# zhouxuguang/GNXRayTracer

Measured on AMD Instinct MI355X. Metric: Mrays/sec + wall-clock to 1024spp, dragon Cornell 1920×1080, higher is better.
Workload: dtype f32; 1 GPU; cfg3: Cornell + synthetic 100000-tri mesh (stand-in for absent dragon.3d), Glass+Metal, PathIntegrator maxDepth 8 rr 1 spatial, Halton(1024), 1920x1080; passes_in_flight=4, sub_passes=56, spp_rendered=1024, gather=n/a, world_size=1, backend=none, devices_visible=1

## Files before the change

### __graft_entry__.py

```python
import os
import shutil
import subprocess
import sys

ROOT = os.path.dirname(os.path.abspath(__file__))
CSRC = os.path.join(ROOT, "gnxraytracer_amd", "csrc")
LIB = os.path.join(ROOT, "gnxraytracer_amd", "libgnxr.so")
SOURCES = ["inst_whitted_tex.hip", "inst_whitted.hip", "inst_vol.hip", "inst_shade_query.hip", "inst_aov.hip", "api.hip", "scene_compile.cpp", "scene_builder.cpp"]
HIPCC_FLAGS = ["--offload-arch=gfx950", "-O3", "-std=c++17", "-fPIC", "-ffp-contract=off", "-fno-slp-vectorize", "-fno-unroll-loops", "-Wall",
               "-Wno-unused-variable", "-Wno-unused-function"]


def _newer(target, deps):
    if not os.path.exists(target):
        return False
    t = os.path.getmtime(target)
    return all(os.path.getmtime(d) <= t for d in deps)


def source_id():
    import hashlib
    h = hashlib.sha1()
    for f in sorted(os.listdir(CSRC)):
        if f.endswith((".h", ".hip", ".cpp")):
            h.update(f.encode()); h.update(open(os.path.join(CSRC, f), "rb").read())
    h.update(" ".join(HIPCC_FLAGS).encode())
    return h.hexdigest()[:12]


LIB_ID = LIB + ".source_id"


def library_source_id():
    try:
        return open(LIB_ID).read().strip()
    except OSError:
        return None


def build_lib(force=False):
    hipcc = shutil.which("hipcc") or "/opt/rocm/bin/hipcc"
    deps = [os.path.join(CSRC, f) for f in os.listdir(CSRC)] + [os.path.join(ROOT, "include", "gnxr.h")]
    if not force and _newer(LIB, deps) and library_source_id() == source_id():
        return LIB
    objdir = os.path.join(ROOT, "build")
    os.makedirs(objdir, exist_ok=True)
    objs = [os.path.join(objdir, os.path.splitext(s)[0] + ".o") for s in SOURCES]
    procs = [subprocess.Popen([hipcc] + HIPCC_FLAGS + ["-c", os.path.join(CSRC, s), "-o", o], cwd=CSRC) for s, o in zip(SOURCES, objs)]
    failed = [s for s, p in zip(SOURCES, procs) if p.wait() != 0]
    if failed:
        raise RuntimeError("hipcc failed for " + ", ".join(failed))
    sid = source_id()
    subprocess.check_call([hipcc, "--offload-arch=gfx950", "-shared", "-fPIC"] + objs + ["-o", LIB, "-lpthread"], cwd=CSRC)
    with open(LIB_ID, "w") as f:
        f.write(sid + "\n")
    return LIB


CLI = os.path.join(ROOT, "gnxraytracer_amd", "gnxr_cli")


def build_cli():
    src = os.path.join(ROOT, "tools", "gnxr_cli.c")
    if _newer(CLI, [src, LIB, os.path.join(ROOT, "include", "gnxr.h")]):
        return CLI
    subprocess.check_call(["gcc", "-std=c11", "-O2", "-Wall", src, "-o", CLI, "-L" + os.path.dirname(LIB), "-lgnxr", "-Wl,-rpath,$ORIGIN"])
    return CLI


def build_oracle():
    subprocess.check_call(["make", "-C", os.path.join(ROOT, "oracle"), "libgnx_oracle.so"])
    if os.path.isdir("/root/reference"):
        subprocess.check_call(["make", "-C", os.path.join(ROOT, "oracle"), "-j8", "ref"], stdout=subprocess.DEVNULL)


def build():
    build_lib()
    build_cli()
    build_oracle()
    sys.path.insert(0, ROOT)
    import gnxraytracer_amd as gx
    gx.lib()


def smoke():
    sys.path.insert(0, ROOT)
    sys.path.insert(0, os.path.join(ROOT, "tests"))
    import numpy as np

    import gnxraytracer_amd as gx
    import oracle_lib as ol
    import scenes

    if library_source_id() is not None and library_source_id() != source_id():
        raise RuntimeError("gnxraytracer_amd/libgnxr.so was built from other sources than gnxraytracer_amd/csrc (%s vs %s): run build()" % (library_source_id(), source_id()))
    gx.init(0)
    b = scenes.cornell()
    integ = gx.PathIntegrator(8, 1.0, "spatial")
    scene = gx.Scene(b)
    img, st = integ.Render(scene, 64, 64, 16)
    oimg, ost = ol.OracleScene(b).render(integ, 64, 64, 16)
    rmse = float(np.sqrt(np.mean((img[..., :3] - oimg[..., :3]) ** 2)))
    print(f"smoke: 64x64x16spp Cornell  rays gpu={st['rays_closest']}+{st['rays_any']} oracle={ost['rays_closest']}+{ost['rays_any']} rmse={rmse:.3e}")
    assert rmse < 1e-3, rmse
    assert abs(st["rays_closest"] - ost["rays_closest"]) <= 1e-3 * ost["rays_closest"]


if __name__ == "__main__":
    build()
    if len(sys.argv) > 1 and sys.argv[1] == "smoke":
        smoke()
```

### gnxraytracer_amd/csrc/api.hip

```cpp
#include <hip/hip_runtime.h>

#include <chrono>
#include <cstdio>
#include <cstdlib>
#include <memory>
#include <mutex>
#include <string>
#include <thread>
#include <vector>

#include "host_scene.h"
#include "kernels.hip.h"
#include "trace4_kernel.hip.h"
#include "hlbvh_build.hip.h"
#include "refit_kernel.hip.h"
#include "material_kernel.hip.h"
#include "rebuild_kernel.hip.h"
#include "li_kernel.hip.h"
#include "views_kernel.hip.h"
#include "shade_query_kernel.hip.h"
#include "aov_kernel.hip.h"
#include "kernel_instances.h"

using namespace gnxr;

#define X(M, L, S, T) extern template GX_WHITTED_SIGNATURE(M, L, S, T)
GX_WHITTED_INSTANCES(X)
#undef X
#define X(M, L, ST, T) extern template GX_VOL_SIGNATURE(M, L, ST, T)
GX_VOL_INSTANCES(X)
#undef X
extern template GX_BSDF_QUERY_SIGNATURE(LM_ALL)
extern template GX_LIGHT_SAMPLE_QUERY_SIGNATURE(LT_ALL)
extern template GX_LIGHT_LE_QUERY_SIGNATURE(LT_ALL)
extern template GX_TRACE_CLOSEST_CODE_SIGNATURE(32)
extern template GX_TRACE_CLOSEST_CODE_SIGNATURE(64)
#define X(M) extern template GX_AOV_RESOLVE_SIGNATURE(M)
GX_AOV_INSTANCES(X)
#undef X

#include "api_common.hip.h"
#include "api_scene.hip.h"
#include "api_hlbvh.hip.h"
#include "api_probes.hip.h"
#include "api_device_call.hip.h"
#include "api_render.hip.h"

extern "C" {

int gnxr_init(int device_id) {
    int n = 0;
    hipError_t e = hipGetDeviceCount(&n);
    if (e != hipSuccess || n <= 0) { set_error("no HIP device available; libgnxr has no CPU fallback"); return GNXR_ERR_NO_DEVICE; }
    if (device_id < 0 || device_id >= n) { set_error("device %d out of range (%d visible)", device_id, n); return GNXR_ERR_INVALID; }
    HIP_TRY(hipSetDevice(device_id));
    g_device = -1;
    g_devices.assign(1, device_id);
    g_peer_ok.assign(1, 1);
    return ensure_device();
}
int gnxr_init_devices(int32_t n_devices, const int32_t *device_ids) {
    if (n_devices <= 0 || n_devices > 64 || !device_ids) { set_error("bad device list"); return GNXR_ERR_INVALID; }
    int n = 0;
    hipError_t e = hipGetDeviceCount(&n);
    if (e != hipSuccess || n <= 0) { set_error("no HIP device available; libgnxr has no CPU fallback"); return GNXR_ERR_NO_DEVICE; }
    for (int i = 0; i < n_devices; ++i)
        if (device_ids[i] < 0 || device_ids[i] >= n) { set_error("device %d out of range (%d visible)", device_ids[i], n); return GNXR_ERR_INVALID; }
    int rc = gnxr_init(device_ids[0]);
    if (rc) return rc;
    g_devices.assign(device_ids, device_ids + n_devices);
    g_peer_ok.assign(n_devices, 1);
    for (int i = 1; i < n_devices; ++i) {
        if (device_ids[i] == device_ids[0]) continue;
        int can01 = 0, can10 = 0;
        bool ok = hipDeviceCanAccessPeer(&can01, device_ids[0], device_ids[i]) == hipSuccess && can01 &&
                  hipDeviceCanAccessPeer(&can10, device_ids[i], device_ids[0]) == hipSuccess && can10;
        if (ok) {
            hipError_t e0 = hipSetDevice(device_ids[0]) == hipSuccess ? hipDeviceEnablePeerAccess(device_ids[i], 0) : hipErrorInvalidDevice;
            hipError_t e1 = hipSetDevice(device_ids[i]) == hipSuccess ? hipDeviceEnablePeerAccess(device_ids[0], 0) : hipErrorInvalidDevice;
            ok = (e0 == hipSuccess || e0 == hipErrorPeerAccessAlreadyEnabled) && (e1 == hipSuccess || e1 == hipErrorPeerAccessAlreadyEnabled);
        }
        g_peer_ok[i] = ok ? 1 : 0;
        if (getenv("GNXR_VERBOSE")) fprintf(stderr, "[gnxr] device %d <-> %d: %s\n", device_ids[0], device_ids[i], ok ? "peer access" : "no peer access: rows are staged through the host");
    }
    (void)hipGetLastError();
    if (getenv("GNXR_NO_PEER")) for (int i = 1; i < n_devices; ++i) g_peer_ok[i] = 0;
    HIP_TRY(hipSetDevice(device_ids[0]));
    return GNXR_OK;
}
void gnxr_shutdown(void) { g_device = -1; g_devices.clear(); g_peer_ok.clear(); }
int gnxr_set_profiling(int flags) { g_profiling = flags; return GNXR_OK; }
#ifdef GX_SHADE_STATS
int gnxr_debug_shade_stats(unsigned long long *out16, int reset) {
    if (hipMemcpyFromSymbol(out16, HIP_SYMBOL(g_shade_stats), 16 * sizeof(unsigned long long)) != hipSuccess) return GNXR_ERR_INVALID;
    if (reset) { unsigned long long z[16] = {0}; (void)hipMemcpyToSymbol(HIP_SYMBOL(g_shade_stats), z, sizeof(z)); }
    return GNXR_OK;
}
#endif
#ifdef GX_TRACE_STATS
int gnxr_debug_trace_stats(unsigned long long *out16, int reset) {
    if (hipMemcpyFromSymbol(out16, HIP_SYMBOL(g_trace_stats), 24 * sizeof(unsigned long long)) != hipSuccess) return GNXR_ERR_INVALID;
    if (reset) { unsigned long long z[24] = {0}; (void)hipMemcpyToSymbol(HIP_SYMBOL(g_trace_stats), z, sizeof(z)); }
    return GNXR_OK;
}
#endif
#ifdef GX_TAIL_STAMP
int gnxr_debug_tail_stamp(unsigned long long *out12, int reset) {
    if (hipMemcpyFromSymbol(out12, HIP_SYMBOL(g_tail), 12 * sizeof(unsigned long long)) != hipSuccess) return GNXR_ERR_INVALID;
    if (reset) { unsigned long long z[12] = {~0ull, 0ull, ~0ull, 0ull}; (void)hipMemcpyToSymbol(HIP_SYMBOL(g_tail), z, sizeof(z)); }
    return GNXR_OK;
}
#endif

static int upload_scene(gnxr_scene *s, size_t) {
    const CompiledScene &cs = s->cs;
    int rc;
    if (cs.bvh_max_depth + 1 > 64) { set_error("BVH depth %d exceeds the 64-entry traversal stack (BVHAccel.cpp:661)", cs.bvh_max_depth); return GNXR_ERR_UNSUPPORTED; }
    s->set_traversal(std::any_of(cs.nodes.begin(), cs.nodes.end(), [](const DNode &n) { return (n.meta & 0xffffu) > 127; }));
#define UP(field) if ((rc = s->field.upload(cs.field)) != GNXR_OK) return rc;
    UP(nodes) UP(nodes4) UP(tris) UP(leaf_boxes) UP(tri_class) UP(lights) UP(perms) UP(primes) UP(prime_sums) UP(prime_magic)
    UP(dmedia) UP(grid_density) UP(tri_media) UP(spheres) UP(textures) UP(tex_texels) UP(ewa_lut) UP(tri_uv) UP(tri_n) UP(tri_s)
    UP(aov_albedo)
    UP(env_texels4) UP(env_cond_func) UP(env_cond_cdf) UP(env_cond_int) UP(env_marg_func) UP(env_marg_cdf) UP(env_marg_guide) UP(env_cond_guide)
#undef UP
    {
        const size_t worst = 2 * cs.desc_materials.size();
        if ((rc = s->material_authored.alloc(worst)) || (rc = s->materials.alloc(1 + worst)) || (rc = s->materials_single.alloc(1 + worst))) return rc;
        if ((rc = s->material_authored.upload(cs.material_authored)) != GNXR_OK) return rc;
        const DTexTables rec = s->tex_tables(s->tri_uv.p, s->tri_n.p, s->tri_s.p);
        for (int k = 0; k < 2; ++k) {
            const std::vector<DMaterial> &src = k == 0 ? cs.materials : cs.materials_single;
            std::vector<DMaterial> up(src.size() + 1);
            memset(&up[0], 0, sizeof(DMaterial));
            memcpy(&up[0], &rec, sizeof(rec));
            std::copy(src.begin(), src.end(), up.begin() + 1);
            if ((rc = (k == 0 ? s->materials : s->materials_single).upload(up)) != GNXR_OK) return rc;
        }
    }
    if ((rc = s->infinite.upload(cs.infinite_lights)) != GNXR_OK) return rc;
    if ((rc = s->counters.alloc(1)) != GNXR_OK) return rc;
    if (hipHostMalloc((void **)&s->h_counters, sizeof(Counters)) != hipSuccess) { set_error("hipHostMalloc failed"); return GNXR_ERR_OOM; }
    if (hipHostMalloc((void **)&s->h_ring, sizeof(Counters) * gnxr_scene::kRing) != hipSuccess) { set_error("hipHostMalloc failed"); return GNXR_ERR_OOM; }
    for (hipEvent_t &e : s->ring_ev) HIP_TRY(hipEventCreateWithFlags(&e, hipEventDisableTiming));
    for (hipStream_t &a : s->aux_stream) HIP_TRY(hipStreamCreateWithFlags(&a, hipStreamNonBlocking));
    HIP_TRY(hipEventCreateWithFlags(&s->ev_fork, hipEventDisableTiming));
    for (hipEvent_t &e : s->ev_join) HIP_TRY(hipEventCreateWithFlags(&e, hipEventDisableTiming));
    return GNXR_OK;
}

int gnxr_scene_create(const gnxr_scene_desc *desc, gnxr_scene **out) {
    if (!desc || !out) { set_error("null argument"); return GNXR_ERR_INVALID; }
    int rc = ensure_device();
    if (rc) return rc;
    gnxr_scene *s = new (std::nothrow) gnxr_scene(g_device);
    if (!s) return GNXR_ERR_OOM;
    if (!compile_scene(desc, &s->cs, device_hlbvh_build)) { delete s; return GNXR_ERR_INVALID; }
    for (size_t i = 1; i < g_devices.size(); ++i) s->replicas.push_back(std::make_unique<gnxr_scene>(g_devices[i], s->host));
    if ((rc = s->each_copy(upload_scene)) != GNXR_OK) { delete s; return rc; }
    const CompiledScene &cs = s->cs;
    if (getenv("GNXR_VERBOSE"))
        fprintf(stderr, "[gnxr] scene: %zu tris, %zu nodes (depth %d), %zu 4-wide nodes (stack %d), wide=%d, %zu device(s)\n", cs.tris.size(), cs.nodes.size(), cs.bvh_max_depth,
                cs.nodes4.size(), cs.stack4_need, (int)s->wide_ok, s->n_copies());
    *out = s;
    return GNXR_OK;
}
void gnxr_scene_destroy(gnxr_scene *s) { delete s; }

int gnxr_scene_info(const gnxr_scene *s, int32_t *n_nodes, int32_t *max_depth, int32_t *n_vox) {
    if (!s) return GNXR_ERR_INVALID;
    if (n_nodes) *n_nodes = (int32_t)s->cs.nodes.size();
    if (max_depth) *max_depth = s->cs.bvh_max_depth;
    if (n_vox) *n_vox = s->grid_strategy >= 0 ? s->grid.nvox[0] * s->grid.nvox[1] * s->grid.nvox[2] : 0;
    return GNXR_OK;
}

int gnxr_render_device(gnxr_scene *s, const gnxr_render_params *pin, void *d_rgba_out, void *hip_stream, gnxr_stats *stats) {
    return render_sharded(s, pin, d_rgba_out, hip_stream, stats);
}

int gnxr_render_reserve(gnxr_scene *s, const gnxr_render_params *pin) {
    if (!s || !pin) { set_error("null argument"); return GNXR_ERR_INVALID; }
    int dummy = 0;
    return render_sharded(s, pin, &dummy, nullptr, nullptr, true);
// ... 261 lines not shown
```

### gnxraytracer_amd/csrc/api_common.hip.h

```cpp
#pragma once

namespace { int hip_status(hipError_t e); }
#define HIP_TRY(expr)                                                                                   \
    do {                                                                                                \
        hipError_t e_ = (expr);                                                                         \
        if (e_ != hipSuccess) {                                                                         \
            set_error("%s failed: %s (%s:%d)", #expr, hipGetErrorString(e_), __FILE__, __LINE__);       \
            return hip_status(e_);                                                                      \
        }                                                                                               \
    } while (0)

namespace {

int hip_status(hipError_t e) {
    if (e == hipErrorOutOfMemory) return GNXR_ERR_OOM;
    if (e == hipErrorNoDevice || e == hipErrorInvalidDevice || e == hipErrorInsufficientDriver || e == hipErrorNotInitialized) return GNXR_ERR_NO_DEVICE;
    return GNXR_ERR_RUNTIME;
}

int g_device = -1;
std::vector<int> g_devices;
std::vector<char> g_peer_ok;
int g_num_cus = 256;
int g_profiling = 0;
int g_grid_bpc = 8;
int g_trace_blocks_per_cu = 5;

struct KernelTimer {
    std::vector<hipEvent_t> pool;
    struct Span { int kind; hipEvent_t a, b; };
    std::vector<Span> open;
    size_t used = 0;
    double seconds[3] = {0, 0, 0};
    unsigned launches[3] = {0, 0, 0};
    hipEvent_t get() {
        if (used == pool.size()) { hipEvent_t e; if (hipEventCreate(&e) != hipSuccess) return nullptr; pool.push_back(e); }
        return pool[used++];
    }
    void begin(int kind, hipStream_t st) { Span s{kind, get(), get()}; if (s.a && s.b) { (void)hipEventRecord(s.a, st); open.push_back(s); } }
    void end(hipStream_t st) { if (!open.empty()) (void)hipEventRecord(open.back().b, st); }
    void collect() {
        for (auto &s : open) { float ms = 0; if (hipEventElapsedTime(&ms, s.a, s.b) == hipSuccess) { seconds[s.kind] += ms * 1e-3; launches[s.kind]++; } }
        open.clear();
        used = 0;
    }
    ~KernelTimer() { for (auto e : pool) (void)hipEventDestroy(e); }
};

struct Knobs {
    static int env_int(const char *name, int unset) { const char *e = getenv(name); return e ? atoi(e) : unset; }
    static bool env_set(const char *name) { return getenv(name) != nullptr; }
#define GX_ONCE(type, expr) do { static const type v = (expr); return v; } while (0)
    static int trace_blocks_per_cu() { const int v = env_int("GNXR_TRACE_BLOCKS_PER_CU", 0); return v >= 1 && v <= 8 ? v : 0; }
    static int grid_blocks_per_cu() { const int v = env_int("GNXR_GRID_BLOCKS_PER_CU", 0); return v >= 1 && v <= 4096 ? v : 0; }
    static int trace_lds_levels() { GX_ONCE(int, env_set("GNXR_TRACE_LDS_LEVELS") ? std::max(2, env_int("GNXR_TRACE_LDS_LEVELS", 0)) : 64); }
    static int trace_chunk() { GX_ONCE(int, env_set("GNXR_TRACE_CHUNK") ? std::max(64, env_int("GNXR_TRACE_CHUNK", 0) / 64 * 64) : kTraceChunk); }
    static bool leaf_box_table() { GX_ONCE(bool, env_set("GNXR_LEAF_BOX_TABLE")); }
    static int regions() { GX_ONCE(int, env_int("GNXR_REGIONS", 0)); }
    static bool pipeline() { GX_ONCE(bool, env_int("GNXR_PIPELINE", 1) != 0); }
    static int pipe_cut() { GX_ONCE(int, env_int("GNXR_PIPE_CUT", -1)); }
    static int loop_lag() { GX_ONCE(int, env_int("GNXR_LOOP_LAG", -1)); }
    static int shade_blocks_per_cu() { GX_ONCE(int, env_set("GNXR_SHADE_BLOCKS_PER_CU") ? std::max(1, env_int("GNXR_SHADE_BLOCKS_PER_CU", 0)) : 32); }
    static int shade_lds_dims() { GX_ONCE(int, env_set("GNXR_SHADE_LDS_DIMS") ? std::max(0, std::min(128, env_int("GNXR_SHADE_LDS_DIMS", 0))) : 64); }
    static bool shade_lds_tables() { GX_ONCE(bool, env_int("GNXR_SHADE_LDS_TABLES", 1) != 0); }
    static int shade_streams() { GX_ONCE(int, env_int("GNXR_SHADE_STREAMS", -1)); }
    static bool vol_pack() { GX_ONCE(bool, env_int("GNXR_VOL_PACK", 1) != 0); }
#undef GX_ONCE
    static int volmedia_step_cap() { return env_set("GNXR_VOLMEDIA_STEP_CAP") ? std::max(0, env_int("GNXR_VOLMEDIA_STEP_CAP", 0)) : 64; }
    static bool no_escape_queue() { return env_set("GNXR_NO_ESCAPE_QUEUE"); }
    static bool host_light_grid() { return env_set("GNXR_HOST_LIGHT_GRID"); }
    static bool binary_bvh() { return env_set("GNXR_BINARY_BVH"); }
};

int ensure_device() {
    if (g_device >= 0) { HIP_TRY(hipSetDevice(g_device)); return GNXR_OK; }
    int n = 0;
    hipError_t e = hipGetDeviceCount(&n);
    if (e != hipSuccess || n <= 0) {
        set_error("no HIP device available (%s); libgnxr has no CPU fallback", e != hipSuccess ? hipGetErrorString(e) : "0 devices");
        return GNXR_ERR_NO_DEVICE;
    }
    int dev = 0;
    HIP_TRY(hipGetDevice(&dev));
    hipDeviceProp_t prop;
    HIP_TRY(hipGetDeviceProperties(&prop, dev));
    g_num_cus = prop.multiProcessorCount > 0 ? prop.multiProcessorCount : 256;
    g_device = dev;
    if (const int v = Knobs::trace_blocks_per_cu()) g_trace_blocks_per_cu = v;
    if (const int v = Knobs::grid_blocks_per_cu()) g_grid_bpc = v;
    return GNXR_OK;
}

template <typename T>
struct DevBuf {
    T *p = nullptr;
    size_t n = 0;
    ~DevBuf() { release(); }
    void release() { if (p) { (void)hipFree(p); p = nullptr; n = 0; } }
    int alloc(size_t count) {
        if (count <= n && p) return GNXR_OK;
        release();
        if (count == 0) count = 1;
        HIP_TRY(hipMalloc((void **)&p, count * sizeof(T)));
        n = count;
        return GNXR_OK;
    }
    int upload(const T *src, size_t count) {
        int rc = alloc(count);
        if (rc) return rc;
        if (count) HIP_TRY(hipMemcpy(p, src, count * sizeof(T), hipMemcpyHostToDevice));
        return GNXR_OK;
    }
    template <typename V> int upload(const V &v) { return upload(v.data(), v.size()); }
};

int grid_for(long long n, int blocks_per_cu = 0) {
    if (blocks_per_cu <= 0) blocks_per_cu = g_grid_bpc;
    long long need = (n + kBlock - 1) / kBlock;
    long long cap = (long long)g_num_cus * blocks_per_cu;
    return (int)std::max<long long>(1, std::min(need, cap));
}

}
```

### gnxraytracer_amd/csrc/api_render.hip.h

```cpp
#pragma once

struct TraceLaunch {
    int entries;
    int lds_entries;
    bool spill_needed;
    size_t lds;
    int n_top;
    int blocks;
};
static TraceLaunch trace_launch(const gnxr_scene *s, bool wide, bool spheres, long long total) {
    TraceLaunch t;
    t.entries = wide ? s->cs.stack4_need + 1 : s->cs.bvh_max_depth + 2;
    const int per_cu = g_trace_blocks_per_cu;
    const size_t fixed_b = wide ? (size_t)(kRayRecDwords + (spheres ? 1 : 0)) * kRqStride * sizeof(int) + (size_t)kTopCache * 128 + 128 : 0;
    t.lds_entries = std::min(std::min(t.entries, Knobs::trace_lds_levels()), std::max(2, (int)(((160 * 1024) / per_cu - 1024 - fixed_b) / (kBlock * sizeof(int)))));
    t.spill_needed = t.entries > t.lds_entries;
    t.lds = (size_t)t.lds_entries * kBlock * sizeof(int) + fixed_b;
    t.n_top = (int)std::min<size_t>(kTopCache, s->cs.root4 >= 0 ? s->cs.nodes4.size() : 0);
    t.blocks = (int)std::min<long long>((long long)g_num_cus * per_cu, (total + kBlock - 1) / kBlock);
    return t;
}

static int count_local_rows(const gnxr_render_params *p) {
    int rows = 0;
    for (int y = 0; y < p->height; ++y)
        if ((y / p->shard_rows) % p->shard_count == p->shard_index) ++rows;
    return rows;
}

struct RaySource {
    const gnxr_ray *rays;
    const gnxr_li_sample *samples;
    float *L;
    long long n;
};

struct ViewSource {
    const gnxr_camera *cameras;
    const int32_t *media;
    int n_views;
};

struct RenderPlan {
    gnxr_render_params p;
    bool direct, volpath, whitted;
    int wmode;
    int n_records, max_light_samples;
    bool textured_scene;
    int class_mask;
    bool area_only, area_env_only;
    bool escape_queue;
    bool caller_rays;
    int n_views;
    int local_rows, npix;
    long long unit, unit_begin, unit_end;
    int spill_entries;
    int k, in_flight;
    size_t half, cap, nrec;

    bool path_int() const { return !whitted && !volpath; }
    int nsamples() const { return p.spp_end - p.spp_begin; }
    int size_passes(size_t slots_held, bool have_mem, size_t free_b);
};

static const long long kSubPassPaths = 64ll << 20;
static const unsigned long long kSlotBytesEstimate = 238;
static const double kStateFreeFraction = 0.45;
static const unsigned long long kStateCapBytes = 150ull * 1000 * 1000 * 1000;

static int plan_render(const CompiledScene &cs, const gnxr_render_params *pin, const RaySource *src, const ViewSource *views, RenderPlan *out) {
    RenderPlan &pl = *out;
    gnxr_render_params &p = pl.p;
    p = *pin;
    if (p.shard_count <= 0) p.shard_count = 1;
    if (p.shard_rows <= 0) p.shard_rows = 1;
    if (p.spp_end <= 0) p.spp_end = p.spp;
    if (!image_and_samples_ok(p) || p.shard_index < 0 || p.shard_index >= p.shard_count || p.max_depth < 0 || p.max_depth > 250) return invalid_render_params();
    if (p.integrator != GNXR_INTEGRATOR_PATH && p.integrator != GNXR_INTEGRATOR_VOLPATH && p.integrator != GNXR_INTEGRATOR_WHITTED &&
        p.integrator != GNXR_INTEGRATOR_DIRECT) {
        set_error("unknown integrator %d", p.integrator);
        return GNXR_ERR_UNSUPPORTED;
    }
    pl.direct = p.integrator == GNXR_INTEGRATOR_DIRECT;
    if (pl.direct && p.direct_strategy != GNXR_DIRECT_SAMPLE_ALL && p.direct_strategy != GNXR_DIRECT_SAMPLE_ONE) {
        set_error("unknown direct-lighting strategy %d", p.direct_strategy);
        return GNXR_ERR_INVALID;
    }
    pl.volpath = p.integrator == GNXR_INTEGRATOR_VOLPATH;
    pl.whitted = p.integrator == GNXR_INTEGRATOR_WHITTED || pl.direct;
    pl.wmode = !pl.direct ? WM_WHITTED : (p.direct_strategy == GNXR_DIRECT_SAMPLE_ONE ? WM_DIRECT_ONE : WM_DIRECT_ALL);
    pl.n_records = (int)cs.desc_lights.size();
    pl.max_light_samples = 1;
    if (pl.wmode == WM_DIRECT_ONE) pl.n_records = 1;
    if (pl.wmode == WM_DIRECT_ALL) {
        pl.n_records = 0;
        for (const gnxr_light &l : cs.desc_lights) { pl.n_records += std::max(1, l.n_samples); pl.max_light_samples = std::max(pl.max_light_samples, l.n_samples); }
        pl.n_records = std::max(1, pl.n_records);
    }
    if (pl.whitted && (pl.n_records > 256 || p.max_depth > 32)) {
        set_error("Whitted / DirectLighting on the device: at most 256 light samples per vertex (every light is sampled at every vertex), depth 32");
        return GNXR_ERR_UNSUPPORTED;
    }
    pl.class_mask = 0;
    for (const DMaterial &m : cs.materials) pl.class_mask |= 1 << m.shade_class;
    pl.textured_scene = (pl.class_mask & 8) != 0;
    if (src && pl.textured_scene && (pl.whitted || pl.volpath)) {
        set_error("Li for caller rays: Whitted, DirectLighting and VolPath need camera ray differentials on scenes with image textures");
        return GNXR_ERR_UNSUPPORTED;
    }
    if (views && pl.textured_scene && pl.volpath) {
        set_error("views: VolPath on a scene with image textures recomputes the camera's ray differentials inside its shade kernels; render its views one by one");
        return GNXR_ERR_UNSUPPORTED;
    }
    pl.area_only = pl.area_env_only = true;
    for (const gnxr_light &l : cs.desc_lights) {
        if (l.type != GNXR_LIGHT_AREA_TRI) pl.area_only = false;
        if (l.type != GNXR_LIGHT_AREA_TRI && l.type != GNXR_LIGHT_INFINITE) pl.area_env_only = false;
    }
    pl.escape_queue = pl.path_int() && !pl.textured_scene && !cs.infinite_lights.empty() && !Knobs::no_escape_queue();
    pl.caller_rays = src != nullptr;
    pl.n_views = views ? views->n_views : 0;
    pl.local_rows = count_local_rows(&p);
    pl.npix = views ? views->n_views * p.width * p.height : pl.local_rows * p.width;
    pl.unit = src ? 1 : pl.npix;
    pl.unit_begin = src ? 0 : p.spp_begin;
    pl.unit_end = src ? src->n : p.spp_end;
    pl.spill_entries = std::max(cs.stack4_need + 1, cs.bvh_max_depth + 2);
    pl.k = pl.in_flight = 0;
    pl.half = pl.cap = pl.nrec = 0;
    return GNXR_OK;
}

int RenderPlan::size_passes(size_t slots_held, bool have_mem, size_t free_b) {
    const long long n_units = unit_end - unit_begin;
    k = p.samples_per_pass;
    if (k <= 0) {
        long long target = 32ll << 20;
        if (have_mem) target = std::max<long long>(target, std::min<long long>(256ll << 20, (long long)(free_b / 4 / 230)));
        if (volpath) target = std::min<long long>(target, 64ll << 20);
        if (whitted) target = (4ll << 20) / std::max(1, n_records / 4);
        if (path_int()) target = kSubPassPaths;
        k = (int)std::max<long long>(1, std::min<long long>(n_units, target / unit));
    }
    k = (int)std::min<long long>(k, n_units);
    half = (size_t)unit * k;
    in_flight = 1;
    if (path_int() && Knobs::pipeline()) {
        const int n_subs = (int)std::min<long long>(kMaxRegions, (n_units + k - 1) / k);
        in_flight = p.passes_in_flight > 0 ? p.passes_in_flight : (Knobs::regions() > 0 ? Knobs::regions() : 4);
        in_flight = std::max(1, std::min(std::min(in_flight, kMaxRegions), n_subs));
        for (; in_flight > 1; --in_flight) {
            const unsigned long long want = (unsigned long long)in_flight * half, held = (unsigned long long)slots_held;
            const bool idx_ok = want < (1ull << 31) && want * 3ull < (1ull << 32);
            bool mem_ok = true;
            if (want > held && have_mem) mem_ok = (want - held) * kSlotBytesEstimate < (unsigned long long)(kStateFreeFraction * (double)free_b);
            if (want * kSlotBytesEstimate > kStateCapBytes) mem_ok = false;
            if (idx_ok && mem_ok) break;
        }
    }
    cap = (size_t)in_flight * half;
    nrec = whitted ? (size_t)std::max(1, n_records) : 1;
    const unsigned long long recs = nrec;
    if (cap >= (1ull << 31) || (unsigned long long)cap * recs >= (1ull << 31) || (unsigned long long)cap * (1ull + 2ull * recs) >= (1ull << 32)) {
        set_error("pass too large: %zu paths x %llu NEE records per vertex overflow the 32-bit work indices; lower samples_per_pass", cap, recs);
        return GNXR_ERR_INVALID;
    }
    return GNXR_OK;
}

int RenderState::reserve(const RenderPlan &pl) {
    const size_t cap = pl.cap, nrec = pl.nrec;
    int rc;
#define AL(f) if ((rc = f.alloc(cap)) != GNXR_OK) return rc;
    for (int i = 0; i < kRecGroups; ++i) {
        const size_t per_slot = i < 2 ? 1 : (i < 4 ? nrec : (pl.direct ? nrec : 1));
        if ((rc = rec[i].alloc(cap * per_slot * kRS)) != GNXR_OK) return rc;
    }
    if ((rc = mis_Y.alloc(cap * (pl.direct ? nrec : 1))) != GNXR_OK) return rc;
    AL(L) AL(hit) AL(queue_a) AL(queue_b) AL(queue_nee) AL(queue_c0) AL(queue_c1) AL(queue_c2) AL(queue_c3) AL(pflags) AL(pclass) AL(nee_vis)
    if (pl.whitted) {
        const size_t nl = (size_t)std::max(1, pl.n_records), md = (size_t)std::max(1, pl.p.max_depth);
        if ((rc = wh_rec.alloc(cap * nl)) ||
            (rc = wh_o.alloc(cap * md)) || (rc = wh_d.alloc(cap * md)) || (rc = wh_L.alloc(cap * md)) || (rc = wh_w.alloc(cap * md)) ||
            (rc = wh_pdf.alloc(cap * md)) || (rc = vol_vs.alloc(cap)))
            return rc;
        if (pl.textured_scene && ((rc = wh_rxo.alloc(cap * (md + 1))) || (rc = wh_rxd.alloc(cap * (md + 1))) || (rc = wh_ryo.alloc(cap * (md + 1))) || (rc = wh_ryd.alloc(cap * (md + 1)))))
            return rc;
    }
    if (pl.volpath) {
        AL(vol_n1) AL(vol_f) AL(vol_Li) AL(vol_Tr) AL(vol_Ld) AL(vol_mres) AL(vol_vs) AL(vol_state)
        AL(vol_Lout) AL(vol_alt_state) AL(vol_orig) AL(vol_alt_orig) AL(vol_newslot)
        for (int i = 0; i < kVolPackF4; ++i) AL(vol_alt[i])
        for (int i = 0; i < kRecGroups; ++i) if ((rc = vol_alt_rec[i].alloc(cap * kRS)) != GNXR_OK) return rc;
    }
#undef AL
    if ((rc = trace_spill.alloc((size_t)g_num_cus * g_trace_blocks_per_cu * kBlock * (size_t)pl.spill_entries)) != GNXR_OK) return rc;
    if (!pl.caller_rays && (rc = accum.alloc(pl.npix)) != GNXR_OK) return rc;
    const size_t max_tiles = (cap + kCompactTile - 1) / kCompactTile;
    if (tile_desc.n < kCompactMaxOut * max_tiles || !tile_desc.p) {
        if ((rc = tile_desc.alloc(kCompactMaxOut * max_tiles)) != GNXR_OK) return rc;
        HIP_TRY(hipMemset(tile_desc.p, 0, tile_desc.n * sizeof(unsigned long long)));
        HIP_TRY(hipDeviceSynchronize());
        compact_seq = 0;
    }
    if ((rc = compact_ticket.alloc(2)) != GNXR_OK) return rc;
    if (pl.n_views > 0 && (rc = view_cams.alloc((size_t)pl.n_views)) != GNXR_OK) return rc;
    return GNXR_OK;
}

unsigned long long RenderState::state_bytes(const RenderPlan &pl) {
    const unsigned long long per_slot = (2ull * kRecGroups + 2) * sizeof(float4) + 8ull * sizeof(int) + 2 + sizeof(unsigned int);
    const unsigned long long tiles = ((unsigned long long)pl.cap + kCompactTile - 1) / kCompactTile;
    return (unsigned long long)pl.cap * per_slot + tiles * kCompactMaxOut * sizeof(unsigned long long) +
           (pl.volpath ? (unsigned long long)pl.cap * (6ull * sizeof(float4) + sizeof(int4) + 1) : 0ull);
}

PathArrays RenderState::path_arrays() {
    PathArrays pa;
    float4 *rec_primary[kRecGroups];
    record_ptrs(rec, rec_primary);
    pa.bind_records(rec_primary);
    pa.mis_Y = mis_Y.p;
    pa.L = L.p; pa.hit = hit.p; pa.pflags = pflags.p; pa.pclass = pclass.p; pa.nee_vis = nee_vis.p;
    return pa;
}
VolArrays RenderState::vol_arrays() {
    VolArrays va;
    float4 *rec_primary[kRecGroups];
    record_ptrs(rec, rec_primary);
    va.bind_records(rec_primary);
    va.mis_Y = mis_Y.p;
    va.vs = vol_vs.p; va.n1 = vol_n1.p; va.f = vol_f.p;
    va.Li = vol_Li.p; va.Tr = vol_Tr.p; va.Ld = vol_Ld.p; va.mres = vol_mres.p; va.state = vol_state.p;
    va.orig = vol_orig.p; va.Lout = vol_Lout.p;
    return va;
}
WhittedArrays RenderState::whitted_arrays(const RenderPlan &pl, int n_lights) {
    WhittedArrays wa;
    wa.ws = vol_vs.p; wa.fr_o = wh_o.p; wa.fr_d = wh_d.p; wa.fr_L = wh_L.p; wa.fr_w = wh_w.p; wa.fr_pdf = wh_pdf.p;
    wa.fr_rxo = wh_rxo.p; wa.fr_rxd = wh_rxd.p; wa.fr_ryo = wh_ryo.p; wa.fr_ryd = wh_ryd.p;
    wa.cap = (int)pl.cap; wa.n_lights = n_lights; wa.n_records = pl.n_records;
    wa.start_dim = pl.wmode == WM_DIRECT_ALL ? 5 + 2 * (pl.p.max_depth * n_lights * 2) : 5;
    return wa;
}
VolPackSet RenderState::pack_set(bool alt) {
    VolPackSet ps;
    if (!alt) {
        float4 *a[kVolPackF4] = {L.p, reinterpret_cast<float4 *>(vol_vs.p), vol_n1.p, vol_f.p, vol_Li.p, vol_Tr.p, vol_Ld.p, mis_Y.p, vol_mres.p};
        for (int i = 0; i < kVolPackF4; ++i) ps.f4[i] = a[i];
        record_ptrs(rec, ps.rec);
        ps.state = vol_state.p; ps.orig = vol_orig.p;
    } else {
        for (int i = 0; i < kVolPackF4; ++i) ps.f4[i] = vol_alt[i].p;
        record_ptrs(vol_alt_rec, ps.rec);
        ps.state = vol_alt_state.p; ps.orig = vol_alt_orig.p;
    }
    return ps;
}

struct RenderRun {
    gnxr_scene *s;
    RenderState &st;
    hipStream_t stream;
    const RenderPlan &pl;
    const RaySource *src;
    const ViewSource *views;
    DScene sc;
    DRender r;
    PathArrays pa;
    VolArrays va;
    WhittedArrays wa;
    DMediaTables mt;
    Counters *dctr;
    KernelTimer timer;
    const bool timing = (g_profiling & 1) != 0, count_wide = (g_profiling & 4) != 0, counting = (g_profiling & 2) != 0 && !count_wide;
    bool spheres;
    bool list_media = false;
    int n_lights, n_scene_media;
    unsigned long long rays_closest = 0, rays_any = 0, rays_mis = 0, media_segments = 0;
    unsigned long long new_paths = 0;
    unsigned int launches = 0, passes = 0, loop_iterations = 0;

    RenderRun(gnxr_scene *scene, hipStream_t stream_, const RenderPlan &plan, const RaySource *src_, const ViewSource *views_, const DScene &sc_, const DRender &r_)
        : s(scene), st(scene->st), stream(stream_), pl(plan), src(src_), views(views_), sc(sc_), r(r_), pa(st.path_arrays()), va(st.vol_arrays()),
          wa(st.whitted_arrays(plan, (int)scene->cs.desc_lights.size())), mt(scene->media_tables()), dctr(scene->counters.p), spheres(scene->cs.n_spheres > 0),
          n_lights((int)scene->cs.desc_lights.size()), n_scene_media((int)scene->cs.media.size()) {}

    void launch_trace(TraceWork w, int n_sh, int n_mis, bool count_rays = true);
    void compact(int mode, const int *qin, int nin, const unsigned char *keys, int nout, int nscatter, unsigned int *totals, int *o0, int *o1, int *o2, int *o3 = nullptr, int split = 0,
                 const unsigned *n_dev = nullptr);
    int shade_stage(const int *q_in, int n, int *q_out, const unsigned *n_dev);
    void raygen(const PathArrays &at, long long u0, int kk, unsigned char *medium_keys);
    void resolve(const PathArrays &at, long long u0, int kk);
    void bind_set(const VolPackSet &ps);
};

void RenderRun::launch_trace(TraceWork w, int n_sh, int n_mis, bool count_rays) {
    long long total = (long long)w.n_closest + w.n_nee;
    if (total <= 0) return;
    w.order = nullptr;
    (void)hipMemsetAsync(&dctr->cursor, 0, sizeof(unsigned int), stream);
    const bool wide = s->wide_ok && !counting;
    const TraceLaunch tl = trace_launch(s, wide, spheres, total);
    if (timing) timer.begin(0, stream);
    const int chunk = Knobs::trace_chunk();
#define GX_TRACE(C, W, S) hipLaunchKernelGGL((k_trace<C, W, S>), dim3(tl.blocks), dim3(kBlock), tl.lds, stream, sc, pa, w, &dctr->cursor, dctr, tl.lds_entries, st.trace_spill.p, chunk)
#define GX_TRACE4(C, S, P) hipLaunchKernelGGL((k_trace4<C, S, P>), dim3(tl.blocks), dim3(kBlock), tl.lds, stream, sc, pa, w, &dctr->cursor, dctr, tl.lds_entries, st.trace_spill.p, chunk, tl.n_top)
#define GX_TRACE4_CS(C, S) do { if (tl.spill_needed) GX_TRACE4(C, S, true); else GX_TRACE4(C, S, false); } while (0)
    if (wide) {
        if (spheres) { if (count_wide) GX_TRACE4_CS(true, true); else GX_TRACE4_CS(false, true); }
        else { if (count_wide) GX_TRACE4_CS(true, false); else GX_TRACE4_CS(false, false); }
    } else {
        const bool cnt = counting || count_wide;
        if (spheres) { if (cnt) GX_TRACE(true, false, true); else GX_TRACE(false, false, true); }
        else { if (cnt) GX_TRACE(true, false, false); else GX_TRACE(false, false, false); }
    }
#undef GX_TRACE4_CS
#undef GX_TRACE4
#undef GX_TRACE
    if (timing) timer.end(stream);
    if (count_rays) {
        rays_closest += (unsigned long long)w.n_closest + (unsigned long long)n_mis;
        rays_any += (unsigned long long)n_sh;
        rays_mis += (unsigned long long)n_mis;
    }
    ++launches;
}

void RenderRun::compact(int mode, const int *qin, int nin, const unsigned char *keys, int nout, int nscatter, unsigned int *totals, int *o0, int *o1, int *o2, int *o3, int split,
                        const unsigned *n_dev) {
    const int tiles = (nin + kCompactTile - 1) / kCompactTile;
    const int g = std::max(1, std::min(tiles, g_num_cus * kCompactBlocksPerCu));
    if (st.compact_seq >= (1u << 30) - 1u) {
        (void)hipMemsetAsync(st.tile_desc.p, 0, st.tile_desc.n * sizeof(unsigned long long), stream);
        st.compact_seq = 0;
    }
    const unsigned seq = ++st.compact_seq;
    const CompactScratch cs{st.tile_desc.p, tiles, st.compact_ticket.p + (seq & 1u), st.compact_ticket.p + ((seq + 1u) & 1u), seq};
    const bool hitclass = mode == COMPACT_HITCLASS;
    const int *hit = hitclass ? (const int *)st.hit.p : nullptr;
    const unsigned char *cls = hitclass ? (const unsigned char *)s->tri_class.p : nullptr;
#define GX_COMPACT(M, N, NS) hipLaunchKernelGGL((k_compact<M, N, NS>), dim3(g), dim3(kCompactBlock), 0, stream, qin, nin, keys, cs, totals, o0, o1, o2, o3, hit, cls, split, n_dev, dctr)
    if (mode == COMPACT_FLAGS) {
        if (nout == 5) { if (nscatter == 3) GX_COMPACT(COMPACT_FLAGS, 5, 3); else GX_COMPACT(COMPACT_FLAGS, 5, 2); }
        else { if (nscatter == 3) GX_COMPACT(COMPACT_FLAGS, 4, 3); else GX_COMPACT(COMPACT_FLAGS, 4, 2); }
    } else if (hitclass) { if (nout == 4) GX_COMPACT(COMPACT_HITCLASS, 4, 4); else GX_COMPACT(COMPACT_HITCLASS, 3, 3); }
    else if (nout == 4) GX_COMPACT(COMPACT_CLASS, 4, 4);
    else GX_COMPACT(COMPACT_CLASS, 3, 3);
#undef GX_COMPACT
    launches += 1;
}
static int compact_stalled(const Counters &c) {
    if (!c.compact_stall) return GNXR_OK;
    set_error("queue compaction: a tile waited for its predecessors beyond the poll limit (k_compact); the render was abandoned");
    return GNXR_ERR_RUNTIME;
}

int RenderRun::shade_stage(const int *q_in, int n, int *q_out, const unsigned *n_dev) {
    if (timing) timer.begin(2, stream);
    const int class_mask = pl.class_mask;
    const bool escape_queue = pl.escape_queue;
    const int n_classes = ((class_mask & 8) || escape_queue) ? 4 : 3;
    compact(COMPACT_HITCLASS, q_in, n, st.pclass.p, n_classes, n_classes, &dctr->q_class[0], st.queue_c0.p, st.queue_c1.p, st.queue_c2.p, st.queue_c3.p, 0, n_dev);
    int *qc[4] = {st.queue_c0.p, st.queue_c1.p, st.queue_c2.p, st.queue_c3.p};
    dim3 g(grid_for(n, Knobs::shade_blocks_per_cu())), b(kBlock);
    const int sdims = std::min<int>(Knobs::shade_lds_dims(), (int)s->cs.prime_sums.size() - 1);
    const int snperm = sdims > 0 ? s->cs.prime_sums[sdims] : 0;
    const bool shade_lds_tabs = Knobs::shade_lds_tables();
    const int lmats = (shade_lds_tabs && s->cs.materials.size() <= 12) ? (int)s->cs.materials.size() : 0;
    const int llights = (shade_lds_tabs && n_lights > 0 && n_lights <= 16) ? n_lights : 0;
    const size_t slds = (sdims > 0 ? ((((size_t)snperm * 2 + 15) & ~(size_t)15) + (size_t)sdims * 32) : 0) + (size_t)lmats * sizeof(DMaterial) + (size_t)llights * sizeof(DLight);
    const int shade_streams = Knobs::shade_streams();
    const int n_class_kernels = 1 + ((class_mask & 2) ? 1 : 0) + ((class_mask & 4) ? 1 : 0) + (((class_mask & 8) || escape_queue) ? 1 : 0);
    const bool fork = (shade_streams < 0 ? n_class_kernels >= 3 : (shade_streams != 0 && n_class_kernels >= 2)) && s->aux_stream[0] && s->aux_stream[1];
    hipStream_t cst[4] = {stream, stream, stream, stream};
    if (fork) {
        HIP_TRY(hipEventRecord(s->ev_fork, stream));
        HIP_TRY(hipStreamWaitEvent(s->aux_stream[0], s->ev_fork, 0));
        HIP_TRY(hipStreamWaitEvent(s->aux_stream[1], s->ev_fork, 0));
        cst[1] = s->aux_stream[0]; cst[2] = s->aux_stream[1]; cst[3] = s->aux_stream[1];
    }
    const bool area_only = pl.area_only, area_env_only = pl.area_env_only;
#define GX_SHADE_K(K, C) hipLaunchKernelGGL(K, g, b, slds, cst[C], sc, r, pa, (const int *)qc[C], (const unsigned int *)&dctr->q_class[C], sdims, snperm, lmats, llights)
#define GX_SHADE(LMV, LTV, C) do { if (spheres) GX_SHADE_K((k_shade<LMV, LTV, true>), C); else GX_SHADE_K((k_shade<LMV, LTV, false>), C); } while (0)
#define GX_SHADE_TEX(LTV) do { if (spheres) GX_SHADE_K((k_shade<LM_ALL, LTV, true, true>), 3); else GX_SHADE_K((k_shade<LM_ALL, LTV, false, true>), 3); } while (0)
    if (area_only) {
        GX_SHADE(LM_DIFFUSE, LT_AREA, 0);
        if (class_mask & 2) GX_SHADE(LM_GLOSSY, LT_AREA, 1);
        if (class_mask & 4) GX_SHADE(LM_ALL, LT_AREA, 2);
        if (class_mask & 8) GX_SHADE_TEX(LT_AREA);
    } else if (area_env_only && !spheres && !(class_mask & 8)) {
#define GX_SHADE_AE(LMV, C) GX_SHADE_K((k_shade<LMV, LT_AREA | LT_ENV, false>), C)
        GX_SHADE_AE(LM_DIFFUSE, 0);
        if (class_mask & 2) GX_SHADE_AE(LM_GLOSSY, 1);
        if (class_mask & 4) GX_SHADE_AE(LM_ALL, 2);
#undef GX_SHADE_AE
    } else {
        GX_SHADE(LM_DIFFUSE, LT_ALL, 0);
        if (class_mask & 2) GX_SHADE(LM_GLOSSY, LT_ALL, 1);
        if (class_mask & 4) GX_SHADE(LM_ALL, LT_ALL, 2);
        if (class_mask & 8) GX_SHADE_TEX(LT_ALL);
    }
#undef GX_SHADE_TEX
#undef GX_SHADE
#undef GX_SHADE_K
    if (escape_queue) {
        if (area_env_only) hipLaunchKernelGGL((k_shade_escape<LT_AREA | LT_ENV>), g, b, 0, cst[3], sc, pa, (const int *)qc[3], (const unsigned int *)&dctr->q_class[3]);
        else hipLaunchKernelGGL((k_shade_escape<LT_ALL>), g, b, 0, cst[3], sc, pa, (const int *)qc[3], (const unsigned int *)&dctr->q_class[3]);
        ++launches;
    }
    if (fork) {
        HIP_TRY(hipEventRecord(s->ev_join[0], s->aux_stream[0]));
        HIP_TRY(hipEventRecord(s->ev_join[1], s->aux_stream[1]));
        HIP_TRY(hipStreamWaitEvent(stream, s->ev_join[0], 0));
        HIP_TRY(hipStreamWaitEvent(stream, s->ev_join[1], 0));
    }
    launches += 1 + ((class_mask & 2) ? 1 : 0) + ((class_mask & 4) ? 1 : 0) + ((class_mask & 8) ? 1 : 0);
    compact(COMPACT_FLAGS, q_in, n, st.pflags.p, 4, 2, &dctr->q_next, q_out, st.queue_nee.p, nullptr, nullptr, 0, n_dev);
    if (timing) timer.end(stream);
    return GNXR_OK;
}

void RenderRun::raygen(const PathArrays &at, long long u0, int kk, unsigned char *medium_keys) {
    const int n_new = (int)(pl.unit * kk);
    if (views) hipLaunchKernelGGL(k_raygen_views, dim3(grid_for(n_new)), dim3(kBlock), 0, stream, sc, r, (const DCamera *)st.view_cams.p, at, n_new, (int)u0, medium_keys);
    else if (!src) hipLaunchKernelGGL(k_raygen, dim3(grid_for(n_new)), dim3(kBlock), 0, stream, sc, r, at, n_new, (int)u0);
    else hipLaunchKernelGGL(k_raygen_rays, dim3(grid_for(n_new)), dim3(kBlock), 0, stream, sc, r, at, reinterpret_cast<const float4 *>(src->rays + u0),
                            reinterpret_cast<const int4 *>(src->samples + u0), n_new, n_scene_media, medium_keys, dctr, u0);
}
void RenderRun::resolve(const PathArrays &at, long long u0, int kk) {
    if (!src) hipLaunchKernelGGL(k_resolve, dim3(grid_for(r.npix)), dim3(kBlock), 0, stream, at, st.accum.p, r.npix, kk);
    else hipLaunchKernelGGL(k_store_li, dim3(grid_for(kk)), dim3(kBlock), 0, stream, (const float4 *)at.L, reinterpret_cast<const int4 *>(src->samples + u0), r,
                            n_scene_media, kk, reinterpret_cast<float4 *>(src->L) + u0);
}
void RenderRun::bind_set(const VolPackSet &ps) {
    pa.bind_records(ps.rec); va.bind_records(ps.rec);
    pa.L = ps.f4[0]; va.vs = reinterpret_cast<int4 *>(ps.f4[1]); va.n1 = ps.f4[2]; va.f = ps.f4[3]; va.Li = ps.f4[4]; va.Tr = ps.f4[5]; va.Ld = ps.f4[6]; pa.mis_Y = va.mis_Y = ps.f4[7]; va.mres = ps.f4[8];
    va.state = ps.state; va.orig = ps.orig;
}

#define GX_CHECK_LAUNCHES(where)                                                                                    \
    do {                                                                                                            \
        const hipError_t le_ = hipGetLastError();                                                                   \
        if (le_ != hipSuccess) { set_error("HIP runtime error in " where ": %s", hipGetErrorString(le_)); return hip_status(le_); } \
    } while (0)

static int run_path_loop(RenderRun &run) {
    gnxr_scene *s = run.s;
    RenderState &st = run.st;
    const RenderPlan &pl = run.pl;
    hipStream_t stream = run.stream;
    Counters *dctr = run.dctr;
    const size_t half = pl.half;
    struct Sub { long long u0; int kk; };
    std::vector<Sub> subs;
    for (long long u0 = pl.unit_begin; u0 < pl.unit_end; u0 += pl.k) subs.push_back(Sub{u0, (int)std::min<long long>(pl.k, pl.unit_end - u0)});
    const int R = pl.in_flight;
    struct Region { int sub = -1, started = -1; long long paths = 0; } reg[kMaxRegions];
    const int lag = std::max(1, std::min(gnxr_scene::kRing - 2, Knobs::loop_lag() >= 0 ? Knobs::loop_lag() : 2));
    const int stagger = Knobs::pipe_cut() >= 0 ? Knobs::pipe_cut() : std::max(1, (pl.p.max_depth + 2 + lag + R - 1) / R);
    int *qbuf[2] = {st.queue_a.p, st.queue_b.p};
    int in_idx = 0;
    const unsigned *cnt_ptr = &dctr->n_queue;
    size_t next_sub = 0, done_subs = 0;
    int iter = 0, last_start = -(1 << 20), newest_seen = -1;
    int ring_iter[gnxr_scene::kRing];
    for (int &v : ring_iter) v = -1;
    Counters seen;
    memset(&seen, 0, sizeof(seen));
    long long guard = 0;
    while (done_subs < subs.size()) {
        {
            int oldest_needed = iter - 1 - lag;
            for (int j = newest_seen + 1; j <= oldest_needed; ++j) {
                const int slot = j % gnxr_scene::kRing;
                if (j >= 0 && ring_iter[slot] == j) HIP_TRY(hipEventSynchronize(s->ring_ev[slot]));
            }
            for (int j = iter - 1; j > newest_seen; --j) {
                const int slot = ((j % gnxr_scene::kRing) + gnxr_scene::kRing) % gnxr_scene::kRing;
                if (j < 0 || ring_iter[slot] != j) continue;
                const hipError_t q = hipEventQuery(s->ring_ev[slot]);
                if (q == hipSuccess) { seen = s->h_ring[slot]; newest_seen = j; if (int rc = compact_stalled(seen)) return rc; break; }
                if (q != hipErrorNotReady) { set_error("HIP runtime error in the path loop: hipEventQuery: %s", hipGetErrorString(q)); return hip_status(q); }
                (void)hipGetLastError();
            }
        }
        for (bool progress = true; progress;) {
            progress = false;
            for (int rg = 0; rg < R; ++rg) {
                Region &g = reg[rg];
                if (g.sub >= 0 && (run.src || g.sub == (int)done_subs) && newest_seen > g.started && seen.region_alive[rg] == 0) {
                    run.resolve(run.pa.at((size_t)rg * half), subs[g.sub].u0, subs[g.sub].kk);
                    ++run.launches; ++run.passes; ++done_subs;
                    g.sub = -1;
                    progress = true;
                }
            }
        }
        if (done_subs == subs.size()) break;
        bool any_active = false;
        long long n_upper = 0;
        for (int rg = 0; rg < R; ++rg) {
            const Region &g = reg[rg];
            if (g.sub < 0) continue;
            any_active = true;
            n_upper += newest_seen > g.started ? std::min<long long>(g.paths, seen.region_alive[rg]) : g.paths;
        }
        const int out_idx = 1 - in_idx;
        if (any_active) {
            if (int rc = run.shade_stage(qbuf[in_idx], (int)n_upper, qbuf[out_idx], cnt_ptr)) return rc;
            hipLaunchKernelGGL(k_loop_tail, dim3(1), dim3(64), 0, stream, (const int *)qbuf[out_idx], dctr, R, (int)half, (unsigned)iter);
            ++run.launches;
            const int slot = iter % gnxr_scene::kRing;
            HIP_TRY(hipMemcpyAsync(&s->h_ring[slot], dctr, sizeof(Counters), hipMemcpyDeviceToHost, stream));
            HIP_TRY(hipEventRecord(s->ring_ev[slot], stream));
            ring_iter[slot] = iter;
        }
        int trace_idx = out_idx;
        long long n_trace_upper = n_upper;
        int free_rg = -1;
        for (int rg = 0; rg < R && free_rg < 0; ++rg) if (reg[rg].sub < 0) free_rg = rg;
        const bool start = next_sub < subs.size() && free_rg >= 0 && (!any_active || iter - last_start >= stagger);
        if (start) {
            const Sub &nw = subs[next_sub];
            const int n_new = (int)(pl.unit * nw.kk);
            const size_t base = (size_t)free_rg * half;
            run.raygen(run.pa.at(base), nw.u0, nw.kk, nullptr);
            hipLaunchKernelGGL(k_queue_merge, dim3(grid_for(n_upper + n_new)), dim3(kBlock), 0, stream, (const int *)qbuf[out_idx], dctr, any_active ? 0 : 1, free_rg, (int)base, n_new, qbuf[in_idx]);
            run.launches += 2;
            trace_idx = in_idx; n_trace_upper = n_upper + n_new;
            run.new_paths += (unsigned long long)n_new;
            reg[free_rg].sub = (int)next_sub; reg[free_rg].started = iter; reg[free_rg].paths = n_new;
            last_start = iter;
            ++next_sub;
        }
        if (any_active || start) {
            TraceWork tw{qbuf[trace_idx], (int)n_trace_upper, st.queue_nee.p, any_active ? (int)n_upper : 0, nullptr, reinterpret_cast<unsigned char *>(st.nee_vis.p), cnt_ptr,
                         any_active ? (const unsigned *)&dctr->q_nee : nullptr};
            run.launch_trace(tw, 0, 0, false);
            if (any_active) {
                if (run.timing) run.timer.begin(1, stream);
                hipLaunchKernelGGL(k_nee_combine, dim3(grid_for(n_upper)), dim3(kBlock), 0, stream, run.pa, (const int *)st.queue_nee.p, (int)n_upper, reinterpret_cast<const unsigned char *>(st.nee_vis.p),
                                   (const unsigned *)&dctr->q_nee);
                if (run.timing) run.timer.end(stream);
                ++run.launches;
            }
            in_idx = trace_idx;
        }
        GX_CHECK_LAUNCHES("the path loop");
        ++iter; ++run.loop_iterations;
        if (++guard > (1ll << 24)) { set_error("path loop did not terminate"); return GNXR_ERR_INVALID; }
    }
    return GNXR_OK;
}

static int run_whitted_pass(RenderRun &run, long long u0, int kk) {
    RenderState &st = run.st;
    const RenderPlan &pl = run.pl;
    hipStream_t stream = run.stream;
    Counters *dctr = run.dctr;
    const DScene &sc = run.sc;
    const DRender &r = run.r;
    const PathArrays &pa = run.pa;
    const WhittedArrays &wa = run.wa;
    const int n_paths = (int)(pl.unit * kk), n_records = pl.n_records;
    const bool textured = pl.textured_scene;
    hipLaunchKernelGGL(k_whitted_init, dim3(grid_for(n_paths)), dim3(kBlock), 0, stream, pa, wa, n_paths);
    ++run.launches;
    if (textured) {
        if (run.views) hipLaunchKernelGGL(k_whitted_init_diff_views, dim3(grid_for(n_paths)), dim3(kBlock), 0, stream, sc, r, (const DCamera *)st.view_cams.p, pa, wa, n_paths);
// ... 338 lines not shown
```

### gnxraytracer_amd/csrc/compact_kernel.hip.h

```cpp
#pragma once
#include "device_math.h"

namespace gnxr {

constexpr int kCompactBlock = 512;
enum CompactMode { COMPACT_FLAGS = 0, COMPACT_CLASS = 1, COMPACT_HITCLASS = 2 };

template <int MODE>
GX_DEV bool compact_pred(unsigned key, int o) { return MODE == COMPACT_FLAGS ? ((key >> o) & 1u) != 0 : key == (unsigned)o; }

constexpr int kCompactChunks = 32;
constexpr int kCompactTile = kCompactBlock * kCompactChunks;
constexpr int kCompactWaves = kCompactBlock / 64;
constexpr int kCompactSpan = 64 * kCompactChunks;
constexpr int kCompactBlocksPerCu = 2;
constexpr int kCompactGather = 8;
constexpr unsigned kCompactPollCap = 1u << 21;
constexpr int kCompactMaxOut = 5;
static_assert(kCompactChunks <= 32 && kCompactChunks % kCompactGather == 0, "predicate masks are 32-bit");
static_assert(kCompactMaxOut <= kCompactWaves, "one wave per predicate looks back");

enum : unsigned { COMPACT_DESC_COUNT = 1u, COMPACT_DESC_PREFIX = 2u };
GX_DEV unsigned long long compact_desc(unsigned tag, unsigned value) { return ((unsigned long long)tag << 32) | value; }

struct CompactScratch {
    unsigned long long *desc;
    int stride;
    unsigned *ticket;
    unsigned *ticket_next;
    unsigned seq;
};

template <int MODE, int NOUT, int NSCATTER>
__global__ void __launch_bounds__(kCompactBlock) k_compact(const int *__restrict__ q_in, int n, const unsigned char *__restrict__ keys, CompactScratch cs,
                                                           unsigned int *totals, int *out0, int *out1, int *out2, int *out3, const int *__restrict__ hit,
                                                           const unsigned char *__restrict__ tri_class, int split, const unsigned *n_dev, Counters *ctr) {
    __shared__ unsigned int wtot[NOUT][kCompactWaves];
    __shared__ unsigned int s_excl[NOUT];
    __shared__ unsigned int s_ticket;
    __shared__ int s_stop;
    const int tid = threadIdx.x, lane = tid & 63, wave = tid >> 6;
    int *outs[4] = {out0, out1, out2, out3};
    if (n_dev) n = (int)min(*n_dev, (unsigned)n);
    const int tilesUsed = (n + kCompactTile - 1) / kCompactTile;
    if (blockIdx.x == 0 && tid == 0) *cs.ticket_next = 0u;
    if (tilesUsed == 0) {
        if (blockIdx.x == 0 && tid < NOUT) totals[tid] = 0u;
        return;
    }
    if (tid == 0) s_stop = 0;
    const unsigned tag_count = (cs.seq << 2) | COMPACT_DESC_COUNT, tag_prefix = (cs.seq << 2) | COMPACT_DESC_PREFIX;
    for (;;) {
        __syncthreads();
        if (tid == 0) s_ticket = atomicAdd(cs.ticket, 1u);
        __syncthreads();
        const unsigned tile = s_ticket;
        if (tile >= (unsigned)tilesUsed) break;
        const long long base = (long long)tile * kCompactTile + wave * kCompactSpan + lane;
        const int *q = q_in ? q_in + base : nullptr;
        const int left = (int)min((long long)n - base, (long long)kCompactSpan);
        int path[kCompactChunks];
#pragma unroll
        for (int c = 0; c < kCompactChunks; ++c) path[c] = c * 64 < left ? (q ? q[c * 64] : (int)base + c * 64) : -1;
        unsigned m[NSCATTER];
#pragma unroll
        for (int o = 0; o < NSCATTER; ++o) m[o] = 0u;
        unsigned acc[NOUT];
#pragma unroll
        for (int o = 0; o < NOUT; ++o) acc[o] = 0u;
#pragma unroll
        for (int c0 = 0; c0 < kCompactChunks; c0 += kCompactGather) {
            unsigned key[kCompactGather];
            if (MODE == COMPACT_HITCLASS) {
                int h[kCompactGather];
#pragma unroll
                for (int j = 0; j < kCompactGather; ++j) h[j] = path[c0 + j] >= 0 ? hit[path[c0 + j]] : -1;
#pragma unroll
                for (int j = 0; j < kCompactGather; ++j) key[j] = path[c0 + j] < 0 ? 0xffu : (h[j] >= 0 ? (unsigned)tri_class[h[j]] : (unsigned)keys[path[c0 + j]]);
            } else {
#pragma unroll
                for (int j = 0; j < kCompactGather; ++j) key[j] = path[c0 + j] >= 0 ? (unsigned)keys[path[c0 + j]] : 0xffu;
            }
#pragma unroll
            for (int j = 0; j < kCompactGather; ++j) {
                const int c = c0 + j;
                const bool valid = path[c] >= 0;
#pragma unroll
                for (int o = 0; o < NOUT; ++o) {
                    const bool pr = valid && ((MODE == COMPACT_FLAGS && o == 4) ? ((key[j] & 1u) != 0 && path[c] < split) : compact_pred<MODE>(key[j], o));
                    if (o < NSCATTER) m[o < NSCATTER ? o : 0] |= (pr ? 1u : 0u) << c;
                    acc[o] += (unsigned)__popcll(__ballot(pr));
                }
            }
        }
#pragma unroll
        for (int o = 0; o < NSCATTER; ++o) m[o] = (unsigned)__shfl((int)m[o], lane);
#pragma unroll
        for (int o = 0; o < NOUT; ++o) if (lane == 0) wtot[o][wave] = acc[o];
        __syncthreads();
        if (wave < NOUT) {
            const int o = wave;
            unsigned agg = 0;
            for (int w = 0; w < kCompactWaves; ++w) agg += wtot[o][w];
            unsigned long long *d = cs.desc + (size_t)o * cs.stride;
            if (lane == 0) __hip_atomic_store(&d[tile], compact_desc(tile == 0 ? tag_prefix : tag_count, agg), __ATOMIC_RELAXED, __HIP_MEMORY_SCOPE_AGENT);
            unsigned excl = 0, polls = 0;
            bool stalled = false;
            long long j = (long long)tile - 1;
            while (j >= 0) {
                const long long idx = j - lane;
                const unsigned long long w = idx >= 0 ? __hip_atomic_load(&d[idx], __ATOMIC_RELAXED, __HIP_MEMORY_SCOPE_AGENT) : compact_desc(tag_prefix, 0u);
                const unsigned tag = (unsigned)(w >> 32);
                const unsigned long long has_prefix = __ballot(tag == tag_prefix), not_ready = __ballot(tag != tag_prefix && tag != tag_count);
                const int first = has_prefix ? __ffsll((long long)has_prefix) - 1 : 63;
                const unsigned long long needed = first >= 63 ? ~0ull : ((2ull << first) - 1ull);
                if (not_ready & needed) {
                    if (++polls > kCompactPollCap) { stalled = true; break; }
                    __builtin_amdgcn_s_sleep(2);
                    continue;
                }
                unsigned sum = lane <= first ? (unsigned)w : 0u;
#pragma unroll
                for (int off = 32; off > 0; off >>= 1) sum += __shfl_xor(sum, off);
                excl += sum;
                if (has_prefix) break;
                j -= 64;
            }
            if (lane == 0) {
                if (stalled) {
                    s_stop = 1;
                    atomicOr(&ctr->compact_stall, 1u);
                    __hip_atomic_store(cs.ticket, 0x80000000u, __ATOMIC_RELAXED, __HIP_MEMORY_SCOPE_AGENT);
                } else {
                    s_excl[o] = excl;
                    if (tile > 0) __hip_atomic_store(&d[tile], compact_desc(tag_prefix, excl + agg), __ATOMIC_RELAXED, __HIP_MEMORY_SCOPE_AGENT);
                    if (tile == (unsigned)tilesUsed - 1u) totals[o] = excl + agg;
                }
            }
        }
        __syncthreads();
        if (s_stop) return;
        unsigned run[NSCATTER];
#pragma unroll
        for (int o = 0; o < NSCATTER; ++o) {
            run[o] = s_excl[o];
            for (int w = 0; w < wave; ++w) run[o] += wtot[o][w];
        }
#pragma unroll
        for (int c = 0; c < kCompactChunks; ++c) {
#pragma unroll
            for (int o = 0; o < NSCATTER; ++o) {
                const bool pr = ((m[o] >> c) & 1u) != 0;
                const unsigned long long b = __ballot(pr);
                const unsigned rank = __builtin_amdgcn_mbcnt_hi((unsigned)(b >> 32), __builtin_amdgcn_mbcnt_lo((unsigned)b, 0u));
                if (pr) outs[o][run[o] + rank] = path[c];
                run[o] += (unsigned)__popcll(b);
            }
        }
    }
}

}
```

### gnxraytracer_amd/csrc/device_bsdf.h

```cpp
#pragma once
#include "device_sampler.h"

namespace gnxr {

GX_DEV float cos_theta(V3 w) { return w.z; }
GX_DEV float cos2_theta(V3 w) { return w.z * w.z; }
GX_DEV float abs_cos_theta(V3 w) { return fabsf(w.z); }
GX_DEV float sin2_theta(V3 w) { return fmaxf(0.f, 1.f - cos2_theta(w)); }
GX_DEV float sin_theta(V3 w) { return gx_sqrt(sin2_theta(w)); }
GX_DEV float tan_theta(V3 w) { return sin_theta(w) / cos_theta(w); }
GX_DEV float tan2_theta(V3 w) { return sin2_theta(w) / cos2_theta(w); }
GX_DEV float cos_phi(V3 w) { float s = sin_theta(w); return (s == 0) ? 1 : clampf(w.x / s, -1, 1); }
GX_DEV float sin_phi(V3 w) { float s = sin_theta(w); return (s == 0) ? 0 : clampf(w.y / s, -1, 1); }
GX_DEV float cos2_phi(V3 w) { return cos_phi(w) * cos_phi(w); }
GX_DEV float sin2_phi(V3 w) { return sin_phi(w) * sin_phi(w); }
GX_DEV bool same_hemisphere(V3 w, V3 wp) { return w.z * wp.z > 0; }
GX_DEV V3 reflect(V3 wo, V3 n) { return -wo + 2 * dot(wo, n) * n; }
GX_DEV bool refract(V3 wi, V3 n, float eta, V3 *wt) {
    float cosThetaI = dot(n, wi);
    float sin2ThetaI = fmaxf(0.f, 1 - cosThetaI * cosThetaI);
    float sin2ThetaT = eta * eta * sin2ThetaI;
    if (sin2ThetaT >= 1) return false;
    float cosThetaT = gx_sqrt(1 - sin2ThetaT);
    *wt = eta * -wi + (eta * cosThetaI - cosThetaT) * n;
    return true;
}

GX_DEV float fr_dielectric(float cosThetaI, float etaI, float etaT) {
    cosThetaI = clampf(cosThetaI, -1, 1);
    bool entering = cosThetaI > 0.f;
    if (!entering) { float t = etaI; etaI = etaT; etaT = t; cosThetaI = fabsf(cosThetaI); }
    float sinThetaI = gx_sqrt(fmaxf(0.f, 1 - cosThetaI * cosThetaI));
    float sinThetaT = etaI / etaT * sinThetaI;
    if (sinThetaT >= 1) return 1;
    float cosThetaT = gx_sqrt(fmaxf(0.f, 1 - sinThetaT * sinThetaT));
    float Rparl = ((etaT * cosThetaI) - (etaI * cosThetaT)) / ((etaT * cosThetaI) + (etaI * cosThetaT));
    float Rperp = ((etaI * cosThetaI) - (etaT * cosThetaT)) / ((etaI * cosThetaI) + (etaT * cosThetaT));
    return (Rparl * Rparl + Rperp * Rperp) / 2;
}
GX_DEV Spec fr_conductor(float cosThetaI, Spec etat, Spec k) {
    cosThetaI = clampf(cosThetaI, -1, 1);
    Spec etai(1.f);
    Spec eta = etat / etai;
    Spec etak = k / etai;
    float cosThetaI2 = cosThetaI * cosThetaI;
    float sinThetaI2 = (float)(1. - (double)cosThetaI2);
    Spec eta2 = eta * eta;
    Spec etak2 = etak * etak;
    Spec t0 = eta2 - etak2 - Spec(sinThetaI2);
    Spec a2plusb2 = ssqrt(t0 * t0 + 4 * eta2 * etak2);
    Spec t1 = a2plusb2 + Spec(cosThetaI2);
    Spec a = ssqrt(0.5f * (a2plusb2 + t0));
    Spec t2 = 2.f * cosThetaI * a;
    Spec Rs = (t1 - t2) / (t1 + t2);
    Spec t3 = cosThetaI2 * a2plusb2 + Spec(sinThetaI2 * sinThetaI2);
    Spec t4 = t2 * sinThetaI2;
    Spec Rp = Rs * (t3 - t4) / (t3 + t4);
    return 0.5f * (Rp + Rs);
}
GX_DEV float schlick_weight(float cosTheta) { float m = clampf(1 - cosTheta, 0, 1); return (m * m) * (m * m) * m; }
GX_DEV float fr_schlick(float R0, float cosTheta) { return lerpf(schlick_weight(cosTheta), R0, 1); }
GX_DEV Spec fr_schlick_spec(Spec R0, float cosTheta) { return slerp(schlick_weight(cosTheta), R0, Spec(1.f)); }
GX_DEV float gtr1(float cosTheta, float alpha) {
    float alpha2 = alpha * alpha;
    return (alpha2 - 1) / (GX_PI * gx_log(alpha2) * (1 + (alpha2 - 1) * cosTheta * cosTheta));
}
GX_DEV float smith_g_ggx(float cosTheta, float alpha) {
    float alpha2 = alpha * alpha;
    float cosTheta2 = cosTheta * cosTheta;
    return (float)(1 / ((double)cosTheta + sqrt((double)(alpha2 + cosTheta2 - alpha2 * cosTheta2))));
}

#define GX_HAS_LOBE(K) ((LM >> (K)) & 1u)
#define GX_HAS_FRESNEL(K) ((LM >> (16 + (K))) & 1u)
constexpr uint32_t lobe_bit(int k) { return 1u << k; }
constexpr uint32_t fresnel_bit(int k) { return 1u << (16 + k); }
constexpr uint32_t LM_DIFFUSE = lobe_bit(LOBE_LAMBERT) | lobe_bit(LOBE_OREN);
constexpr uint32_t LM_GLOSSY = LM_DIFFUSE | lobe_bit(LOBE_SPEC_REFL) | lobe_bit(LOBE_SPEC_TRANS) | lobe_bit(LOBE_FRESNEL_SPEC) | lobe_bit(LOBE_MICRO_REFL) |
                               lobe_bit(LOBE_MICRO_TRANS) | fresnel_bit(FRESNEL_NOOP) | fresnel_bit(FRESNEL_DIELECTRIC) | fresnel_bit(FRESNEL_CONDUCTOR);
constexpr uint32_t LM_ALL = 0xffffffffu;

template <uint32_t LM>
GX_DEV Spec fresnel_eval(const DLobe &l, float cosI) {
    if (GX_HAS_FRESNEL(FRESNEL_DIELECTRIC) && l.fresnel == FRESNEL_DIELECTRIC) return Spec(fr_dielectric(cosI, l.f_etaI, l.f_etaT));
    if (GX_HAS_FRESNEL(FRESNEL_CONDUCTOR) && l.fresnel == FRESNEL_CONDUCTOR) return fr_conductor(fabsf(cosI), spec3(l.f_cEtaT), spec3(l.f_cK));
    if (GX_HAS_FRESNEL(FRESNEL_DISNEY) && l.fresnel == FRESNEL_DISNEY)
        return slerp(l.f_metallic, Spec(fr_dielectric(cosI, 1, l.f_eta)), fr_schlick_spec(spec3(l.f_R0), cosI));
    return Spec(1.f);
}

GX_DEV float tr_D(float ax, float ay, V3 wh) {
    float tan2Theta = tan2_theta(wh);
    if (isinf(tan2Theta)) return 0.f;
    const float cos4Theta = cos2_theta(wh) * cos2_theta(wh);
    float e = (cos2_phi(wh) / (ax * ax) + sin2_phi(wh) / (ay * ay)) * tan2Theta;
    return 1 / (GX_PI * ax * ay * cos4Theta * (1 + e) * (1 + e));
}
GX_DEV float tr_lambda(float ax, float ay, V3 w) {
    float absTanTheta = fabsf(tan_theta(w));
    if (isinf(absTanTheta)) return 0.f;
    float alpha = gx_sqrt(cos2_phi(w) * ax * ax + sin2_phi(w) * ay * ay);
    float alpha2Tan2Theta = (alpha * absTanTheta) * (alpha * absTanTheta);
    return (-1 + gx_sqrt(1.f + alpha2Tan2Theta)) / 2;
}
GX_DEV float tr_G1(float ax, float ay, V3 w) { return 1 / (1 + tr_lambda(ax, ay, w)); }
GX_DEV float tr_G(const DLobe &l, V3 wo, V3 wi) {
    if (l.disney_g) return tr_G1(l.alphax, l.alphay, wo) * tr_G1(l.alphax, l.alphay, wi);
    return 1 / (1 + tr_lambda(l.alphax, l.alphay, wo) + tr_lambda(l.alphax, l.alphay, wi));
}
GX_DEV float tr_pdf(float ax, float ay, V3 wo, V3 wh) {
    return tr_D(ax, ay, wh) * tr_G1(ax, ay, wo) * absdot(wo, wh) / abs_cos_theta(wo);
}
GX_DEV void tr_sample11(float cosTheta, float U1, float U2, float *slope_x, float *slope_y) {
    if (cosTheta > .9999) {
        float r = (float)sqrt((double)(U1 / (1 - U1)));
        float phi = (float)(6.28318530718 * (double)U2);
        const double sphi = gx_sin_d((double)phi), cphi = gx_cos_d((double)phi);
        *slope_x = (float)((double)r * cphi);
        *slope_y = (float)((double)r * sphi);
        return;
    }
    float sinTheta = gx_sqrt(fmaxf(0.f, 1.f - cosTheta * cosTheta));
    float tanTheta = sinTheta / cosTheta;
    float a = 1 / tanTheta;
    float G1 = 2 / (1 + gx_sqrt(1.f + 1.f / (a * a)));
    float A = 2 * U1 / G1 - 1;
    float tmp = 1.f / (A * A - 1.f);
    if (tmp > 1e10f) tmp = 1e10f;
    float B = tanTheta;
    float D = gx_sqrt(fmaxf(B * B * tmp * tmp - (A * A - B * B) * tmp, 0.f));
    float slope_x_1 = B * tmp - D;
    float slope_x_2 = B * tmp + D;
    *slope_x = (A < 0 || slope_x_2 > 1.f / tanTheta) ? slope_x_1 : slope_x_2;
    float S;
    if (U2 > 0.5f) { S = 1.f; U2 = 2.f * (U2 - .5f); }
    else { S = -1.f; U2 = 2.f * (.5f - U2); }
    float z = (U2 * (U2 * (U2 * 0.27385f - 0.73369f) + 0.46341f)) / (U2 * (U2 * (U2 * 0.093073f + 0.309420f) - 1.000000f) + 0.597999f);
    *slope_y = S * z * gx_sqrt(1.f + *slope_x * *slope_x);
}
GX_DEV V3 tr_sample_wh(float ax, float ay, V3 wo, float u0, float u1) {
    bool flip = wo.z < 0;
    V3 wi = flip ? -wo : wo;
    V3 wiStretched = normalize(V3(ax * wi.x, ay * wi.y, wi.z));
    float slope_x, slope_y;
    tr_sample11(cos_theta(wiStretched), u0, u1, &slope_x, &slope_y);
    float tmp = cos_phi(wiStretched) * slope_x - sin_phi(wiStretched) * slope_y;
    slope_y = sin_phi(wiStretched) * slope_x + cos_phi(wiStretched) * slope_y;
    slope_x = tmp;
    slope_x = ax * slope_x;
    slope_y = ay * slope_y;
    V3 wh = normalize(V3(-slope_x, -slope_y, 1.f));
    if (flip) wh = -wh;
    return wh;
}

template <uint32_t LM>
GX_DEV Spec lobe_f(const DLobe &l, V3 wo, V3 wi) {
    switch (l.kind) {
    case LOBE_LAMBERT: if (GX_HAS_LOBE(LOBE_LAMBERT)) return spec3(l.R) * GX_INV_PI; break;
    case LOBE_LAMBERT_TRANS: if (GX_HAS_LOBE(LOBE_LAMBERT_TRANS)) return spec3(l.T) * GX_INV_PI; break;
    case LOBE_OREN: if (GX_HAS_LOBE(LOBE_OREN)) {
        float sinThetaI = sin_theta(wi), sinThetaO = sin_theta(wo);
        float maxCos = 0;
        if (sinThetaI > 1e-4 && sinThetaO > 1e-4) {
            float sinPhiI = sin_phi(wi), cosPhiI = cos_phi(wi);
            float sinPhiO = sin_phi(wo), cosPhiO = cos_phi(wo);
            float dCos = cosPhiI * cosPhiO + sinPhiI * sinPhiO;
            maxCos = fmaxf(0.f, dCos);
        }
        const bool iBig = abs_cos_theta(wi) > abs_cos_theta(wo);
        const float sinAlpha = iBig ? sinThetaO : sinThetaI;
        const float tanBeta = (iBig ? sinThetaI : sinThetaO) / (iBig ? abs_cos_theta(wi) : abs_cos_theta(wo));
        return spec3(l.R) * GX_INV_PI * (l.A + l.B * maxCos * sinAlpha * tanBeta);
    }
    break;
    case LOBE_MICRO_REFL: case LOBE_MICRO_TRANS: if (GX_HAS_LOBE(LOBE_MICRO_REFL) || GX_HAS_LOBE(LOBE_MICRO_TRANS)) {
        const bool refl = l.kind == LOBE_MICRO_REFL;
        float cosThetaO, cosThetaI, eta = 1, cosArg;
        V3 wh;
        if (refl) {
            cosThetaO = abs_cos_theta(wo); cosThetaI = abs_cos_theta(wi);
            wh = wi + wo;
            if (cosThetaI == 0 || cosThetaO == 0) return Spec(0.f);
            if (wh.x == 0 && wh.y == 0 && wh.z == 0) return Spec(0.f);
            wh = normalize(wh);
            cosArg = dot(wi, faceforward(wh, V3(0, 0, 1)));
        } else {
            if (same_hemisphere(wo, wi)) return Spec(0.f);
            cosThetaO = cos_theta(wo); cosThetaI = cos_theta(wi);
            if (cosThetaI == 0 || cosThetaO == 0) return Spec(0.f);
            { const bool up = cos_theta(wo) > 0; eta = (up ? l.etaB : l.etaA) / (up ? l.etaA : l.etaB); }
            wh = normalize(wo + wi * eta);
            if (wh.z < 0) wh = -wh;
            if (dot(wo, wh) * dot(wi, wh) > 0) return Spec(0.f);
            cosArg = dot(wo, wh);
        }
        const Spec F = fresnel_eval<LM>(l, cosArg);
        const float D = tr_D(l.alphax, l.alphay, wh), G = tr_G(l, wo, wi);
        if (refl) return spec3(l.R) * D * G * F / (4 * cosThetaI * cosThetaO);
        float sqrtDenom = dot(wo, wh) + eta * dot(wi, wh);
        float factor = (1 / eta);
        return (Spec(1.f) - F) * spec3(l.T) *
               fabsf(D * G * eta * eta * absdot(wi, wh) * absdot(wo, wh) * factor * factor / (cosThetaI * cosThetaO * sqrtDenom * sqrtDenom));
    }
    break;
    case LOBE_DISNEY_DIFFUSE: if (GX_HAS_LOBE(LOBE_DISNEY_DIFFUSE)) {
        float Fo = schlick_weight(abs_cos_theta(wo)), Fi = schlick_weight(abs_cos_theta(wi));
        return spec3(l.R) * GX_INV_PI * (1 - Fo / 2) * (1 - Fi / 2);
    }
    break;
    case LOBE_DISNEY_FAKESS: if (GX_HAS_LOBE(LOBE_DISNEY_FAKESS)) {
        V3 wh = wi + wo;
        if (wh.x == 0 && wh.y == 0 && wh.z == 0) return Spec(0.f);
        wh = normalize(wh);
        float cosThetaD = dot(wi, wh);
        float Fss90 = cosThetaD * cosThetaD * l.roughness;
        float Fo = schlick_weight(abs_cos_theta(wo)), Fi = schlick_weight(abs_cos_theta(wi));
        float Fss = lerpf(Fo, 1.0f, Fss90) * lerpf(Fi, 1.0f, Fss90);
        float ss = 1.25f * (Fss * (1 / (abs_cos_theta(wo) + abs_cos_theta(wi)) - .5f) + .5f);
        return spec3(l.R) * GX_INV_PI * ss;
    }
    break;
    case LOBE_DISNEY_RETRO: if (GX_HAS_LOBE(LOBE_DISNEY_RETRO)) {
        V3 wh = wi + wo;
        if (wh.x == 0 && wh.y == 0 && wh.z == 0) return Spec(0.f);
        wh = normalize(wh);
        float cosThetaD = dot(wi, wh);
        float Fo = schlick_weight(abs_cos_theta(wo)), Fi = schlick_weight(abs_cos_theta(wi));
        float Rr = 2 * l.roughness * cosThetaD * cosThetaD;
        return spec3(l.R) * GX_INV_PI * Rr * (Fo + Fi + Fo * Fi * (Rr - 1));
    }
    break;
    case LOBE_DISNEY_SHEEN: if (GX_HAS_LOBE(LOBE_DISNEY_SHEEN)) {
        V3 wh = wi + wo;
        if (wh.x == 0 && wh.y == 0 && wh.z == 0) return Spec(0.f);
        wh = normalize(wh);
        return spec3(l.R) * schlick_weight(dot(wi, wh));
    }
    break;
    case LOBE_DISNEY_CLEARCOAT: if (GX_HAS_LOBE(LOBE_DISNEY_CLEARCOAT)) {
        V3 wh = wi + wo;
        if (wh.x == 0 && wh.y == 0 && wh.z == 0) return Spec(0.f);
        wh = normalize(wh);
        float Dr = gtr1(abs_cos_theta(wh), l.gloss);
        float Fr = fr_schlick(.04f, dot(wo, wh));
        float Gr = smith_g_ggx(abs_cos_theta(wo), .25f) * smith_g_ggx(abs_cos_theta(wi), .25f);
        return Spec(l.weight * Gr * Fr * Dr / 4);
    }
    break;
    default: break;
    }
    return Spec(0.f);
}

template <uint32_t LM>
GX_DEV float lobe_pdf(const DLobe &l, V3 wo, V3 wi) {
    switch (l.kind) {
    case LOBE_SPEC_REFL: case LOBE_SPEC_TRANS: case LOBE_FRESNEL_SPEC: return 0.f;
    case LOBE_LAMBERT_TRANS: if (GX_HAS_LOBE(LOBE_LAMBERT_TRANS)) return !same_hemisphere(wo, wi) ? abs_cos_theta(wi) * GX_INV_PI : 0.f; break;
    case LOBE_MICRO_REFL: case LOBE_MICRO_TRANS: if (GX_HAS_LOBE(LOBE_MICRO_REFL) || GX_HAS_LOBE(LOBE_MICRO_TRANS)) {
        const bool refl = l.kind == LOBE_MICRO_REFL;
        V3 wh;
        float scale;
        if (refl) {
            if (!same_hemisphere(wo, wi)) return 0.f;
            wh = normalize(wo + wi);
            scale = 4 * dot(wo, wh);
        } else {
            if (same_hemisphere(wo, wi)) return 0.f;
            const bool up = cos_theta(wo) > 0;
            float eta = (up ? l.etaB : l.etaA) / (up ? l.etaA : l.etaB);
            wh = normalize(wo + wi * eta);
            if (dot(wo, wh) * dot(wi, wh) > 0) return 0.f;
            float sqrtDenom = dot(wo, wh) + eta * dot(wi, wh);
            scale = fabsf((eta * eta * dot(wi, wh)) / (sqrtDenom * sqrtDenom));
        }
        const float p = tr_pdf(l.alphax, l.alphay, wo, wh);
        return refl ? p / scale : p * scale;
    }
    break;
    case LOBE_DISNEY_CLEARCOAT: if (GX_HAS_LOBE(LOBE_DISNEY_CLEARCOAT)) {
        if (!same_hemisphere(wo, wi)) return 0.f;
        V3 wh = wi + wo;
        if (wh.x == 0 && wh.y == 0 && wh.z == 0) return 0.f;
        wh = normalize(wh);
        float Dr = gtr1(abs_cos_theta(wh), l.gloss);
        return Dr * abs_cos_theta(wh) / (4 * dot(wo, wh));
    }
    break;
    default: break;
    }
    return same_hemisphere(wo, wi) ? abs_cos_theta(wi) * GX_INV_PI : 0.f;
}

template <uint32_t LM>
GX_DEV Spec lobe_sample(const DLobe &l, V3 wo, V3 *wi, float u0, float u1, float *pdf, int *sampledType, bool need_f = true) {
    switch (l.kind) {
    case LOBE_SPEC_REFL: if (GX_HAS_LOBE(LOBE_SPEC_REFL)) {
        *wi = V3(-wo.x, -wo.y, wo.z);
        *pdf = 1;
        return fresnel_eval<LM>(l, cos_theta(*wi)) * spec3(l.R) / abs_cos_theta(*wi);
    }
    break;
    case LOBE_SPEC_TRANS: if (GX_HAS_LOBE(LOBE_SPEC_TRANS)) {
        bool entering = cos_theta(wo) > 0;
        float etaI = entering ? l.etaA : l.etaB, etaT = entering ? l.etaB : l.etaA;
        if (!refract(wo, faceforward(V3(0, 0, 1), wo), etaI / etaT, wi)) return Spec(0.f);
        *pdf = 1;
        Spec ft = spec3(l.T) * (Spec(1.f) - fresnel_eval<LM>(l, cos_theta(*wi)));
        ft = ft * ((etaI * etaI) / (etaT * etaT));
        return ft / abs_cos_theta(*wi);
    }
    break;
    case LOBE_FRESNEL_SPEC: if (GX_HAS_LOBE(LOBE_FRESNEL_SPEC)) {
        float F = fr_dielectric(cos_theta(wo), l.etaA, l.etaB);
        if (u0 < F) {
            *wi = V3(-wo.x, -wo.y, wo.z);
            *sampledType = BSDF_SPECULAR | BSDF_REFLECTION;
            *pdf = F;
            return F * spec3(l.R) / abs_cos_theta(*wi);
        } else {
            bool entering = cos_theta(wo) > 0;
            float etaI = entering ? l.etaA : l.etaB, etaT = entering ? l.etaB : l.etaA;
            if (!refract(wo, faceforward(V3(0, 0, 1), wo), etaI / etaT, wi)) return Spec(0.f);
            Spec ft = spec3(l.T) * (1 - F);
            ft = ft * ((etaI * etaI) / (etaT * etaT));
            *sampledType = BSDF_SPECULAR | BSDF_TRANSMISSION;
            *pdf = 1 - F;
            return ft / abs_cos_theta(*wi);
        }
    }
    break;
    case LOBE_MICRO_REFL: case LOBE_MICRO_TRANS: if (GX_HAS_LOBE(LOBE_MICRO_REFL) || GX_HAS_LOBE(LOBE_MICRO_TRANS)) {
        if (wo.z == 0) return Spec(0.f);
        V3 wh = tr_sample_wh(l.alphax, l.alphay, wo, u0, u1);
        if (dot(wo, wh) < 0) return Spec(0.f);
        if (l.kind == LOBE_MICRO_REFL) {
            *wi = reflect(wo, wh);
            if (!same_hemisphere(wo, *wi)) return Spec(0.f);
            *pdf = tr_pdf(l.alphax, l.alphay, wo, wh) / (4 * dot(wo, wh));
        } else {
            const bool up = cos_theta(wo) > 0;
            float eta = (up ? l.etaA : l.etaB) / (up ? l.etaB : l.etaA);
            if (!refract(wo, wh, eta, wi)) return Spec(0.f);
            *pdf = lobe_pdf<LM>(l, wo, *wi);
        }
        return need_f ? lobe_f<LM>(l, wo, *wi) : Spec(0.f);
    }
    break;
    case LOBE_LAMBERT_TRANS: if (GX_HAS_LOBE(LOBE_LAMBERT_TRANS)) {
        *wi = cosine_sample_hemisphere(u0, u1);
        if (wo.z > 0) wi->z *= -1;
        *pdf = lobe_pdf<LM>(l, wo, *wi);
        return need_f ? lobe_f<LM>(l, wo, *wi) : Spec(0.f);
    }
    break;
    case LOBE_DISNEY_CLEARCOAT: if (GX_HAS_LOBE(LOBE_DISNEY_CLEARCOAT)) {
        if (wo.z == 0) return Spec(0.f);
        float alpha2 = l.gloss * l.gloss;
        float cosTheta = gx_sqrt(fmaxf(0.f, (1 - gx_pow(alpha2, 1 - u0)) / (1 - alpha2)));
        float sinTheta = gx_sqrt(fmaxf(0.f, 1 - cosTheta * cosTheta));
        float phi = 2 * GX_PI * u1;
        float sinPhi, cosPhi;
        gx_sincos(phi, &sinPhi, &cosPhi);
        V3 wh(sinTheta * cosPhi, sinTheta * sinPhi, cosTheta);
        if (!same_hemisphere(wo, wh)) wh = -wh;
        *wi = reflect(wo, wh);
        if (!same_hemisphere(wo, *wi)) return Spec(0.f);
        *pdf = lobe_pdf<LM>(l, wo, *wi);
        return need_f ? lobe_f<LM>(l, wo, *wi) : Spec(0.f);
    }
    break;
    default: break;
    }
    *wi = cosine_sample_hemisphere(u0, u1);
    if (wo.z < 0) wi->z *= -1;
    *pdf = lobe_pdf<LM>(l, wo, *wi);
    return need_f ? lobe_f<LM>(l, wo, *wi) : Spec(0.f);
}

template <uint32_t LM>
struct Bsdf {
    const DMaterial *mat;
    V3 ns, ng, ss, ts;
    GX_DEV V3 to_local(V3 v) const { return V3(dot(v, ss), dot(v, ts), dot(v, ns)); }
    GX_DEV V3 to_world(V3 v) const {
        return V3(ss.x * v.x + ts.x * v.y + ns.x * v.z, ss.y * v.x + ts.y * v.y + ns.y * v.z, ss.z * v.x + ts.z * v.y + ns.z * v.z);
    }
    GX_DEV static bool matches(int type, int flags) { return (type & flags) == type; }
    GX_DEV int num_components(int flags) const {
        int n = 0;
        for (int i = 0; i < mat->n_lobes; ++i) if (matches(mat->lobes[i].type, flags)) ++n;
        return n;
    }
    static constexpr bool kSingle = (LM == LM_DIFFUSE);
    static constexpr int kSingleType = BSDF_REFLECTION | BSDF_DIFFUSE;
    GX_DEV Spec f(V3 woW, V3 wiW, int flags) const {
        V3 wi = to_local(wiW), wo = to_local(woW);
        if (wo.z == 0) return Spec(0.f);
        bool refl = dot(wiW, ng) * dot(woW, ng) > 0;
        if (kSingle) return (mat->n_lobes > 0 && refl && matches(kSingleType, flags)) ? lobe_f<LM>(mat->lobes[0], wo, wi) : Spec(0.f);
        return sum_f(wo, wi, flags, refl);
    }
    GX_DEV Spec sum_f(V3 wo, V3 wi, int flags, bool refl) const {
        Spec f(0.f);
        const int n = mat->n_lobes;
        int i = 0;
        while (true) {
            while (i < n) {
                const int t = mat->lobes[i].type;
                if (matches(t, flags) && ((refl && (t & BSDF_REFLECTION)) || (!refl && (t & BSDF_TRANSMISSION)))) break;
                ++i;
            }
            if (i >= n) break;
            f = f + lobe_f<LM>(mat->lobes[i], wo, wi);
            ++i;
        }
        return f;
    }
    GX_DEV float pdf(V3 woW, V3 wiW, int flags) const {
        if (mat->n_lobes == 0) return 0.f;
        V3 wo = to_local(woW), wi = to_local(wiW);
        if (wo.z == 0) return 0.f;
        if (kSingle) return matches(kSingleType, flags) ? 0.f + lobe_pdf<LM>(mat->lobes[0], wo, wi) : 0.f;
        float p = 0.f;
        int matching = 0;
        for (int i = 0; i < mat->n_lobes; ++i) {
            const DLobe &l = mat->lobes[i];
            if (matches(l.type, flags)) { ++matching; p += lobe_pdf<LM>(l, wo, wi); }
        }
        return matching > 0 ? p / matching : 0.f;
    }
    GX_DEV Spec sample_f(V3 woW, V3 *wiW, float u0, float u1, float *pdf, int flags, int *sampledType) const {
        if (kSingle) {
            *sampledType = 0;
            if (mat->n_lobes == 0 || !matches(kSingleType, flags)) { *pdf = 0; return Spec(0.f); }
            const DLobe &bx = mat->lobes[0];
            const float ur0 = fminf(u0 * 1 - 0, GX_ONE_MINUS_EPS);
            V3 wi, wo = to_local(woW);
            *pdf = 0;
            if (wo.z == 0) return Spec(0.f);
            *sampledType = kSingleType;
            (void)lobe_sample<LM>(bx, wo, &wi, ur0, u1, pdf, sampledType, false);
            if (*pdf == 0) { *sampledType = 0; return Spec(0.f); }
            *wiW = to_world(wi);
            const bool refl = dot(*wiW, ng) * dot(woW, ng) > 0;
            return refl ? lobe_f<LM>(bx, wo, wi) : Spec(0.f);
        }
        int matching = num_components(flags);
        *sampledType = 0;
        if (matching == 0) { *pdf = 0; return Spec(0.f); }
        int comp = min((int)floorf(u0 * matching), matching - 1);
        int which = -1, count = comp;
        for (int i = 0; i < mat->n_lobes; ++i)
            if (matches(mat->lobes[i].type, flags) && count-- == 0) { which = i; break; }
        const DLobe &bx = mat->lobes[which];
        float ur0 = fminf(u0 * matching - comp, GX_ONE_MINUS_EPS);
        V3 wi, wo = to_local(woW);
        *pdf = 0;
        if (wo.z == 0) return Spec(0.f);
        *sampledType = bx.type;
        Spec f = lobe_sample<LM>(bx, wo, &wi, ur0, u1, pdf, sampledType, (bx.type & BSDF_SPECULAR) != 0);
        if (*pdf == 0) { *sampledType = 0; return Spec(0.f); }
        *wiW = to_world(wi);
        if (!(bx.type & BSDF_SPECULAR) && matching > 1) {
            const int n = mat->n_lobes;
            int i = 0;
            while (true) {
                while (i < n && !(i != which && matches(mat->lobes[i].type, flags))) ++i;
                if (i >= n) break;
                *pdf += lobe_pdf<LM>(mat->lobes[i], wo, wi);
                ++i;
            }
        }
        if (matching > 1) *pdf /= matching;
        if (!(bx.type & BSDF_SPECULAR)) {
            bool refl = dot(*wiW, ng) * dot(woW, ng) > 0;
            f = sum_f(wo, wi, flags, refl);
        }
        return f;
    }
};

}
```

### gnxraytracer_amd/csrc/gnxr_device_types.h

```cpp
#pragma once
#include <stdint.h>

namespace gnxr {

struct DNode {
    float lo[3];
    float hi0;
    float hi1, hi2;
    int32_t offset;
    uint32_t meta;
};
static_assert(sizeof(DNode) == 32, "DNode must be 32 bytes");

struct DNode4 {
    float lox[4], loy[4], loz[4], hix[4], hiy[4], hiz[4];
    int32_t child[4];
    uint32_t order_lo, order_hi;
    int32_t axes;
    int32_t _pad;
};
static_assert(sizeof(DNode4) == 128, "DNode4 must be 128 bytes");
constexpr int32_t kNode4Empty = 0x7ffffffe;
constexpr int kTopNodesMax = 1024;
constexpr int32_t kRefDone = 0x7fffffff;

struct DTri {
    float p0[3]; int32_t prim;
    float p1[3]; int32_t material;
    float p2[3]; int32_t light;
};
static_assert(sizeof(DTri) == 48, "DTri must be 48 bytes");

struct DSphere {
    float c[3]; float r;
    int32_t material, med_in, med_out, prim;
};
static_assert(sizeof(DSphere) == 32, "DSphere must be 32 bytes");

enum LobeKind : int32_t {
    LOBE_LAMBERT = 0, LOBE_OREN, LOBE_SPEC_REFL, LOBE_SPEC_TRANS, LOBE_FRESNEL_SPEC, LOBE_MICRO_REFL, LOBE_MICRO_TRANS,
    LOBE_LAMBERT_TRANS, LOBE_DISNEY_DIFFUSE, LOBE_DISNEY_FAKESS, LOBE_DISNEY_RETRO, LOBE_DISNEY_SHEEN, LOBE_DISNEY_CLEARCOAT
};
enum FresnelKind : int32_t { FRESNEL_NOOP = 0, FRESNEL_DIELECTRIC, FRESNEL_CONDUCTOR, FRESNEL_DISNEY };
enum : int32_t {
    BSDF_REFLECTION = 1, BSDF_TRANSMISSION = 2, BSDF_DIFFUSE = 4, BSDF_GLOSSY = 8, BSDF_SPECULAR = 16, BSDF_ALL = 31
};

struct DLobe {
    int32_t kind, type, fresnel, disney_g;
    float R[3]; float A;
    float T[3]; float B;
    float etaA, etaB, alphax, alphay;
    float f_etaI, f_etaT, f_metallic, f_eta;
    float f_cEtaT[3]; float roughness;
    float f_cK[3]; float weight;
    float f_R0[3]; float gloss;
};
static_assert(sizeof(DLobe) == 128, "DLobe must be 128 bytes");

struct DMaterial {
    int32_t n_lobes;
    int32_t has_bump;
    int32_t n_nonspecular;
    float eta;
    int32_t shade_class;
    int32_t kd_tex, ks_tex;
    int32_t has_attr;
    DLobe lobes[8];
};

struct DTexture {
    int32_t n_levels, w0, h0, wrap;
    int32_t trilinear; float max_aniso;
    float su, sv, du, dv;
    int32_t level_offset[16];
    int32_t _pad[2];
};
struct DLight {
    int32_t type;
    int32_t tri_leaf;
    int32_t two_sided;
    int32_t env;
    float le[3]; float area;
    float p0[3]; float inv_area;
    float p1[3]; float radius;
    float p2[3]; int32_t n_samples;
    float n[3]; float _pad2;
    float center[3]; float _pad3;
};

struct DHalton {
    int32_t base_scale[2], base_exp[2];
    int32_t stride, mult_inv[2];
    int32_t base32_max;
};

struct DCamera {
    float r2c[16];
    float c2w[16];
    float lens_radius, focal_distance;
    int32_t medium;
    int32_t ortho;
};

constexpr int kEnvGuideMarg = 1024, kEnvGuideCond = 512;
struct DEnv {
    int32_t w, h;
    int32_t dw, dh;
    float l2w[16], w2l[16];
    float world_center[3]; float world_radius;
    float marg_func_int;
};

struct DMedium {
    int32_t type;
    int32_t nx, ny, nz;
    float sigma_a[3]; float g;
    float sigma_s[3]; float sigma_t;
    float w2m[16];
    float inv_max_density;
    int32_t density_offset;
    int32_t _pad[2];
};

struct DLightGrid {
    int32_t nvox[3];
    int32_t n_lights;
    int32_t stride;
    int32_t spatial;
    float lo[3], hi[3];
};

}
```

### gnxraytracer_amd/csrc/host_scene.h

```cpp
#pragma once
#include <string>
#include <vector>

#include "../../include/gnxr.h"
#include "gnxr_device_types.h"
#include "host_math.h"

namespace gnxr {

void set_error(const char *fmt, ...);
const char *get_error();

struct Builder {
    std::vector<float> vertices;
    std::vector<int32_t> indices, tri_material, tri_light, tri_med_in, tri_med_out;
    std::vector<gnxr_material> materials;
    std::vector<gnxr_light> lights;
    std::vector<gnxr_medium> media;
    std::vector<gnxr_sphere> spheres;
    std::vector<float> grid_density;
    std::vector<gnxr_texture> textures;
    std::vector<float> texels;
    std::vector<float> tri_uv;
    std::vector<float> tri_n;
    std::vector<float> tri_s;
    std::vector<float> env_rgb;
    int env_w = 0, env_h = 0;
    gnxr_camera camera;
    int camera_medium = -1;
    int bvh_split_method = 0;
    Builder();
    int add_mesh(const float *verts, int nv, const int32_t *idx, int nt, const Xf &o2w, int material, int med_in, int med_out);
    void fill_desc(gnxr_scene_desc *d) const;
};

bool read_model_3d(const char *path, std::vector<float> *verts, std::vector<int32_t> *idx);
bool write_synthetic_3d(const char *path, int target_tris, uint32_t seed);
bool read_rgbe(const char *path, std::vector<float> *rgb, int *w, int *h);

struct CompiledScene {
    std::vector<DNode> nodes;
    std::vector<DNode4> nodes4;
    int32_t root4 = 0;
    int stack4_need = 1;
    std::vector<DTri> tris;
    std::vector<float> leaf_boxes;
    int leaf1_from_verts = 0;
    std::vector<uint8_t> tri_class;
    std::vector<int32_t> leaf_of_prim;
    int bvh_max_depth = 0;
    Box3 world_bound;
    int n_vertices = 0;
    std::vector<int32_t> corner_vertex;
    std::vector<int32_t> node_parent;
    std::vector<int32_t> node4_src;
    std::vector<DMaterial> materials;
    std::vector<DMaterial> materials_single;
    std::vector<DTexture> textures;
    std::vector<float> tex_texels;
    std::vector<float> ewa_lut;
    std::vector<float> tri_uv;
    std::vector<float> tri_n;
    std::vector<float> tri_s;
    std::vector<float> aov_albedo;
    std::vector<int32_t> material_authored;
    std::vector<gnxr_material> desc_materials;
    std::vector<int32_t> tri_material;
    std::vector<uint8_t> tri_own_attr;
    std::vector<int32_t> sphere_material;
    std::vector<int32_t> mat_map;
    std::vector<DLight> lights;
    std::vector<int32_t> infinite_lights;
    std::vector<uint16_t> perms;
    std::vector<int32_t> primes, prime_sums;
    std::vector<uint32_t> prime_magic;
    bool has_env = false;
    DEnv env;
    std::vector<float> env_texels;
    std::vector<float> env_texels4;
    float env_power_lookup[3] = {0, 0, 0};
    std::vector<float> env_cond_func, env_cond_cdf, env_cond_int;
    std::vector<float> env_marg_func, env_marg_cdf;
    std::vector<uint16_t> env_marg_guide, env_cond_guide;
    std::vector<gnxr_medium> media;
    std::vector<DMedium> dmedia;
    std::vector<float> grid_density;
    std::vector<DSphere> spheres;
    int n_spheres = 0;
    std::vector<int32_t> tri_media;
    gnxr_camera camera;
    int camera_medium = -1;
    std::vector<gnxr_light> desc_lights;
};

struct HlbvhNode { float b[6]; int32_t child[2]; int32_t axis, first, n; };
typedef bool (*HlbvhBuildFn)(const float *prim_bounds6, const float *centroids3, int n, const float lo[3], const float hi[3],
                             std::vector<HlbvhNode> *nodes, int *root, uint32_t *prims_sorted);
bool compile_scene(const gnxr_scene_desc *d, CompiledScene *out, HlbvhBuildFn hlbvh_build = nullptr);
struct MaterialTables {
    std::vector<DMaterial> materials, materials_single;
    std::vector<float> aov_albedo;
    std::vector<int32_t> material_authored, mat_map;
    void move_to(CompiledScene *cs);
};
bool compile_materials(const gnxr_material *mats, int n_materials, int n_textures, const std::vector<int32_t> &sphere_material, const int32_t *tri_material,
                       const uint8_t *tri_own_attr, int n_triangles, const int32_t *visit, MaterialTables *mt);
void triangle_material(const int32_t *mat_map, int32_t authored, uint8_t own_attr, int32_t *material, uint8_t *shade_class);
void refit_world_bound(CompiledScene *cs, const float root6[6]);
bool compile_light(const gnxr_light &l, int index, const Vec3 corners[3], int tri_leaf, const Box3 &world_bound, DLight *out);
DCamera make_camera(const gnxr_camera &c, int W, int H, int medium);
DHalton make_halton(int W, int H);
void build_light_grid(const CompiledScene &cs, int strategy, DLightGrid *grid, std::vector<float> *table, bool layout_only = false);
void light_grid_probes(const CompiledScene &cs, float *ri );

float host_radical_inverse(const CompiledScene &cs, int baseIndex, uint64_t a);

}
```

### gnxraytracer_amd/csrc/kernel_instances.h

```cpp
#pragma once
#include <hip/hip_runtime.h>

#include "host_scene.h"
#include "kernels.hip.h"
#include "vol_kernel.hip.h"
#include "whitted_kernel.hip.h"

#define GX_WH_SPH(X, M, L, T) X(M, L, false, T) X(M, L, true, T)
#define GX_WH_LT(X, M, T) GX_WH_SPH(X, M, LT_AREA, T) GX_WH_SPH(X, M, LT_ALL, T)
#define GX_WHITTED_INSTANCES_TEX(X, T) GX_WH_LT(X, WM_WHITTED, T) GX_WH_LT(X, WM_DIRECT_ONE, T) GX_WH_LT(X, WM_DIRECT_ALL, T)
#define GX_WHITTED_INSTANCES(X) GX_WHITTED_INSTANCES_TEX(X, false) GX_WHITTED_INSTANCES_TEX(X, true)

#define GX_VS_ST(X, M, L, T) X(M, L, VS_MAIN, T) X(M, L, VS_SHADOW, T) X(M, L, VS_MIS, T)
#define GX_VS_LT(X, M, T) GX_VS_ST(X, M, LT_AREA, T) GX_VS_ST(X, M, LT_ALL, T)
#define GX_VOL_INSTANCES(X) GX_VS_LT(X, LM_DIFFUSE, false) GX_VS_LT(X, LM_GLOSSY, false) GX_VS_LT(X, LM_ALL, false) GX_VS_LT(X, LM_ALL, true)

#define GX_WHITTED_SIGNATURE(M, L, S, T) \
    __global__ void gnxr::k_whitted_step<M, L, S, T>(gnxr::DScene, gnxr::DRender, gnxr::PathArrays, gnxr::WhittedArrays, const int *, int, unsigned long long *);
#define GX_VOL_SIGNATURE(M, L, ST, T) \
    __global__ void gnxr::k_vol_step<M, L, ST, T>(gnxr::DScene, gnxr::DMediaTables, gnxr::DRender, gnxr::PathArrays, gnxr::VolArrays, const int *, const unsigned int *, int, int);
```

### gnxraytracer_amd/csrc/kernels.hip.h

```cpp
#pragma once
#include "device_bsdf.h"
#include "device_lights.h"
#include "device_texture.h"

namespace gnxr {

constexpr int kBlock = 256;

constexpr int kRS = 2;
constexpr int kRSm = 2 * kRS;
constexpr int kRecGroups = 5;
struct PathArrays {
    float4 *ray_o;
    float4 *ray_d;
    float4 *beta;
    uint2 *meta;
    float4 *L;
    int *hit;
    unsigned char *pflags;
    unsigned char *pclass;
    float4 *sh_o;
    float4 *sh_d;
    float4 *sh_X;
    float4 *nbeta;
// ... 194 lines not shown
        V3 o, d;
        float tMax;
        int dim;
        camera_ray(r.cam, sc.st, px, py, index, &o, &d, &tMax, &dim);
        pa.ray_o[(size_t)slot * kRS] = make_float4(o.x, o.y, o.z, tMax);
        pa.ray_d[(size_t)slot * kRS] = make_float4(d.x, d.y, d.z, __int_as_float(r.cam.medium));
        pa.beta[(size_t)slot * kRS] = make_float4(1.f, 1.f, 1.f, 1.f);
        pa.L[slot] = make_float4(0.f, 0.f, 0.f, 0.f);
        pa.store_meta(slot, index, (uint32_t)dim);
    }
}

template <uint32_t LM, int LT>
GX_DEV int estimate_direct_record(const DScene &sc, const Bsdf<LM> &bsdf, const SurfacePoint &sp, V3 woN, int lightNum, float ul0, float ul1, float us0,
                                  float us1, const PathArrays &pa, size_t rec, float xw) {
    const int bsdfFlags = BSDF_ALL & ~BSDF_SPECULAR;
    int nflags = 0;
    V3 so, sd, mo, wi2;
    Spec X(0.f), Y(0.f);
    int expect = -1;
    LightSample ls = light_sample<LT>(sc.lt, lightNum, sp.p, ul0, ul1);
    float scatteringPdf = 0;
    if (ls.pdf > 0 && !ls.Li.is_black()) {
        Spec f = bsdf.f(woN, ls.wi, bsdfFlags) * absdot(ls.wi, sp.ns);
        scatteringPdf = bsdf.pdf(woN, ls.wi, bsdfFlags);
        if (!f.is_black()) {
            spawn_ray_to(sp.p, sp.pError, sp.n, ls.p1, ls.p1Error, ls.n1, &so, &sd);
            float weight = light_is_delta<LT>(sc.lt.lights[lightNum]) ? 1.f : power_heuristic(ls.pdf, scatteringPdf);
            X = f * ls.Li * weight / ls.pdf;
            nflags |= 1;
        }
    }
    if (!light_is_delta<LT>(sc.lt.lights[lightNum])) {
        int sampledType;
        Spec f = bsdf.sample_f(woN, &wi2, us0, us1, &scatteringPdf, bsdfFlags, &sampledType);
        f = f * absdot(wi2, sp.ns);
        bool sampledSpecular = (sampledType & BSDF_SPECULAR) != 0;
        if (!f.is_black() && scatteringPdf > 0) {
            float weight = 1;
            bool skip = false;
            if (!sampledSpecular) {
                float lightPdf = light_pdf<LT>(sc.lt, lightNum, sp.p, sp.pError, sp.n, wi2);
                if (lightPdf == 0) skip = true;
                else weight = power_heuristic(scatteringPdf, lightPdf);
            }
            if (!skip) {
                const DLight &lt = sc.lt.lights[lightNum];
                mo = offset_ray_origin(sp.p, sp.pError, sp.n, wi2);
                Spec Li2;
                if (LT == LT_AREA || lt.type == GNXR_LIGHT_AREA_TRI) {
                    V3 lp0(lt.p0[0], lt.p0[1], lt.p0[2]), lp1(lt.p1[0], lt.p1[1], lt.p1[2]), lp2(lt.p2[0], lt.p2[1], lt.p2[2]);
                    V3 ln = normalize(cross(lp0 - lp2, lp1 - lp2));
                    Li2 = area_L(lt, ln, -wi2);
                    expect = lt.tri_leaf;
                } else {
                    Li2 = light_Le<LT>(sc.lt, lightNum, mo, wi2);
                    expect = -1;
                }
                if (!Li2.is_black()) Y = f * Li2 * Spec(1.f) * weight / scatteringPdf;
                nflags |= 2;
            }
        }
    }
    if (nflags) {
        pa.sh_o[(size_t)rec * kRS] = make_float4(so.x, so.y, so.z, 1 - GX_SHADOW_EPS);
        pa.sh_d[(size_t)rec * kRS] = make_float4(sd.x, sd.y, sd.z, __int_as_float(nflags));
        pa.sh_X[(size_t)rec * kRS] = make_float4(X.r, X.g, X.b, xw);
        if (nflags & 2) {
            pa.mis_o[(size_t)rec * kRS] = make_float4(mo.x, mo.y, mo.z, __int_as_float(expect));
            pa.mis_d[(size_t)rec * kRS] = make_float4(wi2.x, wi2.y, wi2.z, 0.f);
            pa.mis_Y[rec] = make_float4(Y.r, Y.g, Y.b, 0.f);
        }
    }
    return nflags;
}
GX_DEV Spec nee_record_Ld(const PathArrays &pa, size_t rec, float *xw) {
    float4 sd4 = pa.sh_d[(size_t)rec * kRS], X4 = pa.sh_X[(size_t)rec * kRS];
    int flags = __float_as_int(sd4.w);
    Spec Ld(0.f);
    if ((flags & 1) && pa.sh_o[(size_t)rec * kRS].w == 1.f) Ld = Ld + Spec(X4.x, X4.y, X4.z);
    if (flags & 2) {
        float4 Y4 = pa.mis_Y[rec];
        Spec Y(Y4.x, Y4.y, Y4.z);
        if (pa.mis_o[(size_t)rec * kRS].w == 1.f && !Y.is_black()) Ld = Ld + Y;
    }
    *xw = X4.w;
    return Ld;
}

template <bool SPH, bool TEX, bool UV = false>
GX_DEV bool shade_hit_rebuild(const DScene &sc, const DMaterial *mats, int leaf, V3 ro, V3 rd, float tMax, V3 *p0, V3 *p1, V3 *p2, TriHit *h, int *triMat, int *triLight,
                              SurfacePoint *sp, V3 *sdpdu, V3 *sdpdv) {
    bool found = leaf != -1;
    if (SPH && leaf < -1) {
        const DSphere &sph = sc.spheres[-2 - leaf];
        *triMat = sph.material;
        float tH;
        found = sphere_test(sph, ro, rd, tMax, &tH);
        if (found) *sp = sphere_surface_point_uv<UV>(sph, ro, rd, tH, *triMat >= 0 ? mats[*triMat].has_bump != 0 : false, sdpdu, sdpdv);
    } else if (found) {
        const float4 *q = reinterpret_cast<const float4 *>(sc.tris + leaf);
        float4 a = q[0], b = q[1], c = q[2];
        *p0 = V3(a.x, a.y, a.z); *p1 = V3(b.x, b.y, b.z); *p2 = V3(c.x, c.y, c.z);
        *triMat = __float_as_int(b.w); *triLight = __float_as_int(c.w);
        tri_hit_recompute(*p0, *p1, *p2, ro, rd, h);
        *sp = surface_point(*p0, *p1, *p2, *h, *triMat >= 0 ? mats[*triMat].has_bump != 0 : false);
        if (TEX) {
            V3 dndu, dndv;
            *sp = surface_point_tables(tex_tables(sc.materials), leaf, *p0, *p1, *p2, *h, *triMat >= 0 ? mats[*triMat].has_bump != 0 : false, &dndu, &dndv);
        }
        found = sp->valid;
    }
    return found;
}
template <bool TEX>
GX_DEV const DMaterial *shade_material(const DScene &sc, const DMaterial *mat, int leaf, V3 p0, V3 p1, V3 p2, const TriHit &h, const SurfacePoint &sp, const RayDiff &rdf,
                                       DMaterial *tm) {
    if (TEX && leaf >= 0 && (mat->kd_tex | mat->ks_tex)) {
        float tu, tv;
        V3 dpdu, dpdv;
        tri_uv_frame(p0, p1, p2, h, tri_uvs(tex_tables(sc.materials), leaf), &tu, &tv, &dpdu, &dpdv);
        textured_material(tex_tables(sc.materials), *mat, tu, tv, compute_differentials(rdf, sp.p, sp.n, dpdu, dpdv), tm);
        mat = tm;
    }
    return mat;
}

#ifndef GX_SHADE_MINWAVES
#define GX_SHADE_MINWAVES 2
#endif
#ifdef GX_SHADE_WAVES
#define GX_SHADE_ATTR __attribute__((amdgpu_waves_per_eu(GX_SHADE_WAVES, GX_SHADE_WAVES)))
#else
#define GX_SHADE_ATTR __attribute__((amdgpu_waves_per_eu(GX_SHADE_MINWAVES)))
#endif
#ifdef GX_SHADE_STATS
static __device__ unsigned long long g_shade_stats[16];
#define GX_STICK(i) do { const unsigned long long t_ = __builtin_amdgcn_s_memtime(); if ((threadIdx.x & 63) == 0) sst_[i] += t_ - stick_; stick_ = t_; } while (0)
#else
#define GX_STICK(i) do {} while (0)
#endif
#ifndef GX_SHADE_W_DIFFUSE
#define GX_SHADE_W_DIFFUSE 3
#endif
#ifndef GX_SHADE_W_GLOSSY
#define GX_SHADE_W_GLOSSY 3
#endif
#ifndef GX_SHADE_W_ALL
#define GX_SHADE_W_ALL GX_SHADE_MINWAVES
#endif
#ifndef GX_SHADE_W_TEX
#define GX_SHADE_W_TEX 3
#endif
template <uint32_t LM> constexpr int shade_min_waves() { return LM == LM_DIFFUSE ? GX_SHADE_W_DIFFUSE : (LM == LM_GLOSSY ? GX_SHADE_W_GLOSSY : GX_SHADE_W_ALL); }
template <uint32_t LM, int LT, bool SPH, bool TEX = false>
__global__ void __launch_bounds__(kBlock, (TEX ? GX_SHADE_W_TEX : shade_min_waves<LM>())) k_shade(DScene sc, DRender r, PathArrays pa, const int *__restrict__ queue, const unsigned int *n_dev, int lds_dims, int lds_nperm, int lds_mats, int lds_lights) {
    extern __shared__ int shade_smem[];
    const int n = (int)*n_dev;
    if (blockIdx.x * blockDim.x >= (unsigned)n) return;
    const LdsSampler lsam = lds_sampler_fill(sc.st, lds_dims, lds_nperm, shade_smem, threadIdx.x, kBlock);
    const DMaterial *mats = sc.materials;
    DLightTables ltab = sc.lt;
    {
        int *dst = shade_smem + (lds_sampler_bytes(lds_nperm, lds_dims) >> 2);
        if (!TEX && lds_mats > 0) {
            const int *src = reinterpret_cast<const int *>(sc.materials);
            const int nd = lds_mats * (int)(sizeof(DMaterial) / 4);
            for (int k = threadIdx.x; k < nd; k += kBlock) dst[k] = src[k];
            mats = reinterpret_cast<const DMaterial *>(dst);
            dst += nd;
        }
        if (lds_lights > 0) {
            const int *src = reinterpret_cast<const int *>(sc.lt.lights);
            const int nd = lds_lights * (int)(sizeof(DLight) / 4);
            for (int k = threadIdx.x; k < nd; k += kBlock) dst[k] = src[k];
            ltab.lights = reinterpret_cast<const DLight *>(dst);
        }
    }
    __syncthreads();
#ifdef GX_SHADE_STATS
    unsigned long long sst_[16] = {0};
    unsigned long long stick_ = __builtin_amdgcn_s_memtime();
#endif
    const int stride_ = (int)(gridDim.x * blockDim.x);
    int i = (int)(blockIdx.x * blockDim.x + threadIdx.x);
    int pathCur_ = i < n ? queue[i] : -1;
    int leafCur_ = pathCur_ >= 0 ? pa.hit[pathCur_] : -1;
    int pathNext_ = (long long)i + stride_ < n ? queue[i + stride_] : -1;
    for (; i < n; i += stride_) {
        bool survive = false, wantNee = false, wantShadow = false, wantMis = false;
        int path = -1;
        GX_STICK(9);
        const int leafNext_ = pathNext_ >= 0 ? pa.hit[pathNext_] : -1;
        const int pathNext2_ = (long long)i + 2ll * stride_ < n ? queue[i + 2 * stride_] : -1;
        {
            path = pathCur_;
            uint2 m = pa.meta[(size_t)path * kRSm];
            uint32_t index = m.x;
            int dim = (int)(m.y & 0xffffu), bounces = (int)((m.y >> 16) & 0xffu);
            bool specularBounce = (m.y >> 31) != 0;
            float4 o4 = pa.ray_o[(size_t)path * kRS], d4 = pa.ray_d[(size_t)path * kRS], b4 = pa.beta[(size_t)path * kRS];
            V3 ro(o4.x, o4.y, o4.z), rd(d4.x, d4.y, d4.z);
            Spec beta(b4.x, b4.y, b4.z);
            float etaScale = b4.w;
            int leaf = leafCur_;
            bool found = leaf != -1;
            V3 p0, p1, p2;
            int triMat = -1, triLight = -1;
            TriHit h;
            SurfacePoint sp;
            sp.valid = false;
            found = shade_hit_rebuild<SPH, TEX>(sc, mats, leaf, ro, rd, o4.w, &p0, &p1, &p2, &h, &triMat, &triLight, &sp, nullptr, nullptr);
            GX_STICK(0);
            if ((bounces == 0 || specularBounce) && (found ? triLight >= 0 : ltab.n_infinite > 0)) {
                const float4 L4 = pa.L[path];
                Spec L(L4.x, L4.y, L4.z);
                if (found) L = L + beta * area_L(ltab.lights[triLight], sp.n, -rd);
                else for (int k = 0; k < ltab.n_infinite; ++k) L = L + beta * light_Le<LT>(ltab, ltab.infinite[k], ro, rd);
                pa.L[path] = make_float4(L.r, L.g, L.b, 0.f);
            }
            GX_STICK(1);
            if (found && bounces < r.max_depth) {
                if (triMat < 0) {
                    V3 o2 = offset_ray_origin(sp.p, sp.pError, sp.n, rd);
                    pa.ray_o[(size_t)path * kRS] = make_float4(o2.x, o2.y, o2.z, GX_INF);
                    survive = true;
                } else {
                    DMaterial tm;
                    RayDiff none;
                    none.has = false;
                    const DMaterial *mat = shade_material<TEX>(sc, mats + triMat, leaf, p0, p1, p2, h, sp, none, &tm);
                    Bsdf<LM> bsdf;
                    bsdf.mat = mat; bsdf.ns = sp.ns; bsdf.ng = sp.n; bsdf.ss = sp.ss; bsdf.ts = sp.ts;
                    SampleStream ss(sc.st, index, dim, lsam);
                    V3 woN = normalize(-rd);
                    if (mat->n_nonspecular > 0 && ltab.n_lights > 0) {
                        float lightPdfSel;
                        int lightNum = light_select(ltab, sp.p, ss.get1d(), &lightPdfSel);
                        GX_STICK(2);
                        if (lightPdfSel != 0) {
                            float ul0, ul1, us0, us1;
                            ss.get2d(&ul0, &ul1);
                            ss.get2d(&us0, &us1);
                            GX_STICK(3);
                            const int bsdfFlags = BSDF_ALL & ~BSDF_SPECULAR;
                            int nflags = 0;
                            V3 so, sd, mo, wi2;
                            Spec X(0.f), Y(0.f);
                            int expect = -1;
                            LightSample ls = light_sample<LT>(ltab, lightNum, sp.p, ul0, ul1);
                            GX_STICK(4);
                            float scatteringPdf = 0;
                            if (ls.pdf > 0 && !ls.Li.is_black()) {
                                Spec f = bsdf.f(woN, ls.wi, bsdfFlags) * absdot(ls.wi, sp.ns);
                                scatteringPdf = bsdf.pdf(woN, ls.wi, bsdfFlags);
                                if (!f.is_black()) {
                                    spawn_ray_to(sp.p, sp.pError, sp.n, ls.p1, ls.p1Error, ls.n1, &so, &sd);
                                    float weight = light_is_delta<LT>(ltab.lights[lightNum]) ? 1.f : power_heuristic(ls.pdf, scatteringPdf);
                                    X = f * ls.Li * weight / ls.pdf;
                                    nflags |= 1;
                                }
                            }
                            GX_STICK(5);
                            if (!light_is_delta<LT>(ltab.lights[lightNum])) {
                                int sampledType;
                                Spec f = bsdf.sample_f(woN, &wi2, us0, us1, &scatteringPdf, bsdfFlags, &sampledType);
                                f = f * absdot(wi2, sp.ns);
                                bool sampledSpecular = (sampledType & BSDF_SPECULAR) != 0;
                                GX_STICK(6);
                                if (!f.is_black() && scatteringPdf > 0) {
                                    float weight = 1;
                                    bool skip = false;
                                    if (!sampledSpecular) {
                                        float lightPdf = light_pdf<LT>(ltab, lightNum, sp.p, sp.pError, sp.n, wi2);
                                        if (lightPdf == 0) skip = true;
                                        else weight = power_heuristic(scatteringPdf, lightPdf);
                                    }
                                    if (!skip) {
                                        const DLight &lt = ltab.lights[lightNum];
                                        mo = offset_ray_origin(sp.p, sp.pError, sp.n, wi2);
                                        Spec Li2;
                                        if (LT == LT_AREA || lt.type == GNXR_LIGHT_AREA_TRI) {
                                            V3 lp0(lt.p0[0], lt.p0[1], lt.p0[2]), lp1(lt.p1[0], lt.p1[1], lt.p1[2]), lp2(lt.p2[0], lt.p2[1], lt.p2[2]);
                                            V3 ln = normalize(cross(lp0 - lp2, lp1 - lp2));
                                            Li2 = area_L(lt, ln, -wi2);
                                            expect = lt.tri_leaf;
                                        } else {
                                            Li2 = light_Le<LT>(ltab, lightNum, mo, wi2);
                                            expect = -1;
                                        }
                                        if (!Li2.is_black()) Y = f * Li2 * Spec(1.f) * weight / scatteringPdf;
                                        nflags |= 2;
                                    }
                                }
                            }
                            GX_STICK(7);
                            if (nflags) {
                                pa.sh_o[(size_t)path * kRS] = make_float4(so.x, so.y, so.z, 1 - GX_SHADOW_EPS);
                                pa.sh_d[(size_t)path * kRS] = make_float4(sd.x, sd.y, sd.z, __int_as_float(nflags));
                                pa.sh_X[(size_t)path * kRS] = make_float4(X.r, X.g, X.b, lightPdfSel);
                                if (nflags & 2) {
                                    pa.mis_o[(size_t)path * kRS] = make_float4(mo.x, mo.y, mo.z, __int_as_float(expect));
                                    pa.mis_d[(size_t)path * kRS] = make_float4(wi2.x, wi2.y, wi2.z, 0.f);
                                    pa.mis_Y[path] = make_float4(Y.r, Y.g, Y.b, 0.f);
                                }
                                pa.nbeta[(size_t)path * kRS] = make_float4(beta.r, beta.g, beta.b, 0.f);
                                const bool betaFinite = __builtin_isfinite(beta.r) && __builtin_isfinite(beta.g) && __builtin_isfinite(beta.b);
// ... 320 lines not shown
```

### gnxraytracer_amd/csrc/material_kernel.hip.h

```cpp
#pragma once
#include <hip/hip_runtime.h>

#include "gnxr_device_types.h"
#include "refit_kernel.hip.h"

namespace gnxr {
namespace matedit {

static __global__ void __launch_bounds__(refit::kB) k_material_tris(DTri *__restrict__ tris, unsigned char *__restrict__ tri_class, int n_tris,
                                                                    const int *__restrict__ tri_material, const unsigned char *__restrict__ own_attr,
                                                                    const int4 *__restrict__ mat_map) {
    for (int li = blockIdx.x * blockDim.x + threadIdx.x; li < n_tris; li += gridDim.x * blockDim.x) {
        const int prim = tris[li].prim;
        if ((unsigned)prim >= (unsigned)n_tris) continue;
        const int authored = tri_material[prim];
        int material = authored, cls = 0;
        if (authored >= 0) {
            const int4 e = mat_map[authored];
            const bool own = own_attr[prim] != 0;
            material = e.x < 0 ? -1 : (own ? e.y : e.x);
            cls = e.x < 0 ? 0 : (own ? 3 : e.z);
        }
        tris[li].material = material;
        tri_class[li] = (unsigned char)cls;
    }
}

static __global__ void __launch_bounds__(refit::kB) k_material_gather(const DTri *__restrict__ tris, const unsigned char *__restrict__ tri_class, int n_tris,
                                                                      const int *__restrict__ authored, int *__restrict__ material_out,
                                                                      unsigned char *__restrict__ class_out) {
    for (int li = blockIdx.x * blockDim.x + threadIdx.x; li < n_tris; li += gridDim.x * blockDim.x) {
        const int prim = tris[li].prim;
        if ((unsigned)prim >= (unsigned)n_tris) continue;
        const int m = tris[li].material;
        material_out[prim] = m >= 0 ? authored[m] : -1;
        class_out[prim] = tri_class[li];
    }
}

}
}
```

### gnxraytracer_amd/csrc/scene_compile.cpp

```cpp
#include <cstdio>
#include <thread>

#include "host_scene.h"

namespace gnxr {

namespace {
struct PrimInfo { int prim; Box3 b; Vec3 c; };
struct BuildNode { Box3 b; int child[2]; int axis, first, n; };

struct BvhBuilder {
    std::vector<PrimInfo> info;
    std::vector<BuildNode> nodes;
    std::vector<int> ordered;
    int method = GNXR_BVH_SAH;

    int build(int start, int end) {
        int me = (int)nodes.size();
        nodes.push_back(BuildNode());
        Box3 bounds;
        for (int i = start; i < end; ++i) bounds.grow(info[i].b);
        int n = end - start;
        auto leaf = [&]() {
            nodes[me].b = bounds; nodes[me].first = (int)ordered.size(); nodes[me].n = n;
// ... 231 lines not shown
            }
        }
        break;
    }
    case GNXR_MAT_MIRROR: {
        RGB R = clamp0(m.kr);
        if (!black(R)) { DLobe l = blank_lobe(LOBE_SPEC_REFL, BSDF_REFLECTION | BSDF_SPECULAR); set_R(l, R); l.fresnel = FRESNEL_NOOP; add(l); }
        break;
    }
    case GNXR_MAT_GLASS: {
        float eta = m.eta[0], urough = m.urough, vrough = m.vrough;
        RGB R = clamp0(m.kr), T = clamp0(m.kt);
        out->eta = eta;
        if (black(R) && black(T)) break;
        bool isSpecular = urough == 0 && vrough == 0;
        if (isSpecular && allowMultipleLobes) {
            DLobe l = blank_lobe(LOBE_FRESNEL_SPEC, BSDF_REFLECTION | BSDF_TRANSMISSION | BSDF_SPECULAR);
            set_R(l, R); set_T(l, T); l.etaA = 1.f; l.etaB = eta;
            add(l);
        } else if (isSpecular) {
            if (!black(R)) {
                DLobe l = blank_lobe(LOBE_SPEC_REFL, BSDF_REFLECTION | BSDF_SPECULAR);
                set_R(l, R); l.fresnel = FRESNEL_DIELECTRIC; l.f_etaI = 1.f; l.f_etaT = eta;
                add(l);
            }
            if (!black(T)) {
                DLobe l = blank_lobe(LOBE_SPEC_TRANS, BSDF_TRANSMISSION | BSDF_SPECULAR);
                set_T(l, T); l.etaA = 1.f; l.etaB = eta; l.fresnel = FRESNEL_DIELECTRIC; l.f_etaI = 1.f; l.f_etaT = eta;
                add(l);
            }
        } else {
            if (m.remap_roughness) { urough = roughness_to_alpha(urough); vrough = roughness_to_alpha(vrough); }
            if (!black(R)) {
                DLobe l = blank_lobe(LOBE_MICRO_REFL, BSDF_REFLECTION | BSDF_GLOSSY);
                set_R(l, R); l.fresnel = FRESNEL_DIELECTRIC; l.f_etaI = 1.f; l.f_etaT = eta; set_alpha(l, urough, vrough);
                add(l);
            }
            if (!black(T)) {
                DLobe l = blank_lobe(LOBE_MICRO_TRANS, BSDF_TRANSMISSION | BSDF_GLOSSY);
                set_T(l, T); l.etaA = 1.f; l.etaB = eta; l.fresnel = FRESNEL_DIELECTRIC; l.f_etaI = 1.f; l.f_etaT = eta;
                set_alpha(l, urough, vrough);
                add(l);
            }
        }
        break;
    }
    case GNXR_MAT_METAL: {
        float ur = m.urough, vr = m.vrough;
        if (m.remap_roughness) { ur = roughness_to_alpha(ur); vr = roughness_to_alpha(vr); }
        DLobe l = blank_lobe(LOBE_MICRO_REFL, BSDF_REFLECTION | BSDF_GLOSSY);
        l.R[0] = l.R[1] = l.R[2] = 1.f;
        l.fresnel = FRESNEL_CONDUCTOR;
        memcpy(l.f_cEtaT, m.eta, 12); memcpy(l.f_cK, m.k, 12);
        set_alpha(l, ur, vr);
        add(l);
        break;
    }
    case GNXR_MAT_PLASTIC: {
        RGB kd = clamp0(m.kd), ks = clamp0(m.ks);
        if (!black(kd) || textured) { DLobe l = blank_lobe(LOBE_LAMBERT, BSDF_REFLECTION | BSDF_DIFFUSE); set_R(l, kd); add(l); }
        if (!black(ks) || textured) {
            DLobe l = blank_lobe(LOBE_MICRO_REFL, BSDF_REFLECTION | BSDF_GLOSSY);
            set_R(l, ks); l.fresnel = FRESNEL_DIELECTRIC; l.f_etaI = 1.5f; l.f_etaT = 1.f;
            float rough = m.urough;
            if (m.remap_roughness) rough = roughness_to_alpha(rough);
            set_alpha(l, rough, rough);
            add(l);
        }
        break;
    }
    case GNXR_MAT_DISNEY: {
        if (m.disney_scatter_distance[0] != 0 || m.disney_scatter_distance[1] != 0 || m.disney_scatter_distance[2] != 0) {
            set_error("Disney scatterDistance != 0 selects the BSSRDF branch, which no reference integrator consumes");
            return false;
        }
        RGB c = clamp0(m.kd);
        float metallicWeight = m.disney_metallic, e = m.eta[0], strans = m.disney_spec_trans;
        float diffuseWeight = (1 - metallicWeight) * (1 - strans);
        float dt = m.disney_diff_trans / 2;
        float rough = m.disney_roughness;
        float lum = 0.212671f * c.c[0] + 0.715160f * c.c[1] + 0.072169f * c.c[2];
        RGB Ctint = lum > 0 ? RGB{{c.c[0] / lum, c.c[1] / lum, c.c[2] / lum}} : RGB{{1, 1, 1}};
        float sheenWeight = m.disney_sheen;
        RGB Csheen = {{0, 0, 0}};
        if (sheenWeight > 0) for (int i = 0; i < 3; ++i) Csheen.c[i] = (1 - m.disney_sheen_tint) * 1.f + m.disney_sheen_tint * Ctint.c[i];
        bool thin = m.disney_thin != 0;
        if (diffuseWeight > 0) {
            if (thin) {
                float flat = m.disney_flatness;
                DLobe l = blank_lobe(LOBE_DISNEY_DIFFUSE, BSDF_REFLECTION | BSDF_DIFFUSE);
                set_R(l, scale_rgb(c, diffuseWeight * (1 - flat) * (1 - dt))); add(l);
                DLobe l2 = blank_lobe(LOBE_DISNEY_FAKESS, BSDF_REFLECTION | BSDF_DIFFUSE);
                set_R(l2, scale_rgb(c, diffuseWeight * flat * (1 - dt))); l2.roughness = rough; add(l2);
            } else {
                DLobe l = blank_lobe(LOBE_DISNEY_DIFFUSE, BSDF_REFLECTION | BSDF_DIFFUSE);
                set_R(l, scale_rgb(c, diffuseWeight)); add(l);
            }
            DLobe lr = blank_lobe(LOBE_DISNEY_RETRO, BSDF_REFLECTION | BSDF_DIFFUSE);
            set_R(lr, scale_rgb(c, diffuseWeight)); lr.roughness = rough; add(lr);
            if (sheenWeight > 0) {
                DLobe ls = blank_lobe(LOBE_DISNEY_SHEEN, BSDF_REFLECTION | BSDF_DIFFUSE);
                set_R(ls, scale_rgb(Csheen, diffuseWeight * sheenWeight)); add(ls);
            }
        }
        float aspect = (float)std::sqrt(1 - m.disney_anisotropic * .9);
        float ax = std::max(.001f, sqrf(rough) / aspect), ay = std::max(.001f, sqrf(rough) * aspect);
        float r0s = sqrf(e - 1) / sqrf(e + 1);
        RGB Cspec0;
        for (int i = 0; i < 3; ++i) {
            float tint = (1 - m.disney_spec_tint) * 1.f + m.disney_spec_tint * Ctint.c[i];
            Cspec0.c[i] = (1 - metallicWeight) * (r0s * tint) + metallicWeight * c.c[i];
        }
        {
            DLobe l = blank_lobe(LOBE_MICRO_REFL, BSDF_REFLECTION | BSDF_GLOSSY);
            l.R[0] = l.R[1] = l.R[2] = 1.f;
            l.fresnel = FRESNEL_DISNEY; memcpy(l.f_R0, Cspec0.c, 12); l.f_metallic = metallicWeight; l.f_eta = e;
            set_alpha(l, ax, ay); l.disney_g = 1;
            add(l);
        }
        if (m.disney_clearcoat > 0) {
            DLobe l = blank_lobe(LOBE_DISNEY_CLEARCOAT, BSDF_REFLECTION | BSDF_GLOSSY);
            l.weight = m.disney_clearcoat;
            l.gloss = lerpf(m.disney_clearcoat_gloss, (float).1, (float).001);
            add(l);
        }
        if (strans > 0) {
            RGB T = {{strans * std::sqrt(c.c[0]), strans * std::sqrt(c.c[1]), strans * std::sqrt(c.c[2])}};
            DLobe l = blank_lobe(LOBE_MICRO_TRANS, BSDF_TRANSMISSION | BSDF_GLOSSY);
            set_T(l, T); l.etaA = 1.f; l.etaB = e; l.fresnel = FRESNEL_DIELECTRIC; l.f_etaI = 1.f; l.f_etaT = e;
            if (thin) {
                float rscaled = (0.65f * e - 0.35f) * rough;
                set_alpha(l, std::max(.001f, sqrf(rscaled) / aspect), std::max(.001f, sqrf(rscaled) * aspect));
                l.disney_g = 0;
            } else { set_alpha(l, ax, ay); l.disney_g = 1; }
            add(l);
        }
        if (thin) { DLobe l = blank_lobe(LOBE_LAMBERT_TRANS, BSDF_TRANSMISSION | BSDF_DIFFUSE); set_T(l, scale_rgb(c, dt)); add(l); }
        break;
    }
    default: set_error("unknown material type %d", m.type); return false;
    }
    for (int i = 0; i < out->n_lobes; ++i) if (!(out->lobes[i].type & BSDF_SPECULAR)) out->n_nonspecular++;
    out->shade_class = 0;
    for (int i = 0; i < out->n_lobes; ++i) {
        int k = out->lobes[i].kind, f = out->lobes[i].fresnel;
        int c = (k == LOBE_LAMBERT || k == LOBE_OREN) ? 0
              : ((k == LOBE_SPEC_REFL || k == LOBE_SPEC_TRANS || k == LOBE_FRESNEL_SPEC || k == LOBE_MICRO_REFL || k == LOBE_MICRO_TRANS) && f != FRESNEL_DISNEY &&
                 !out->lobes[i].disney_g) ? 1 : 2;
        out->shade_class = std::max(out->shade_class, c);
    }
    if (out->shade_class == 0 && out->n_lobes > 1) out->shade_class = 1;
    if (textured) out->shade_class = 3;
    return true;
}

namespace {
struct Pcg32 {
    uint64_t state = 0x853c49e6748fea9bULL, inc = 0xda3e39cb94b95bdbULL;
    uint32_t next() {
        uint64_t old = state;
        state = old * 0x5851f42d4c957f2dULL + inc;
        uint32_t xs = (uint32_t)(((old >> 18u) ^ old) >> 27u), rot = (uint32_t)(old >> 59u);
        return (xs >> rot) | (xs << ((~rot + 1u) & 31));
    }
    uint32_t bounded(uint32_t b) {
        uint32_t threshold = (~b + 1u) % b;
        while (true) { uint32_t r = next(); if (r >= threshold) return r % b; }
    }
};
}

static void build_sampler_tables(CompiledScene *cs) {
    const int N = 1000;
    cs->primes.clear();
    for (int c = 2; (int)cs->primes.size() < N; ++c) {
        bool p = true;
        for (int d = 2; d * d <= c; ++d) if (c % d == 0) { p = false; break; }
        if (p) cs->primes.push_back(c);
    }
    cs->prime_sums.resize(N);
    int sum = 0;
    for (int i = 0; i < N; ++i) { cs->prime_sums[i] = sum; sum += cs->primes[i]; }
    cs->perms.resize(sum);
    Pcg32 rng;
    uint16_t *p = cs->perms.data();
    for (int i = 0; i < N; ++i) {
        int count = cs->primes[i];
        for (int j = 0; j < count; ++j) p[j] = (uint16_t)j;
        for (int j = 0; j < count; ++j) { int other = j + (int)rng.bounded(count - j); std::swap(p[j], p[other]); }
        p += count;
    }
    cs->prime_magic.resize(8 * (size_t)N);
    for (int i = 0; i < N; ++i) {
        uint32_t d = (uint32_t)cs->primes[i];
        int s = 0;
        while ((1ull << s) < d) ++s;
        uint64_t M = ((1ull << 32) * ((1ull << s) - d)) / d + 1;
        uint32_t *rec = &cs->prime_magic[8 * (size_t)i];
        rec[0] = (uint32_t)M;
        rec[1] = (uint32_t)s;
        rec[2] = d;
        rec[3] = (uint32_t)cs->prime_sums[i];
        const float invBase = 1.f / (float)d;
        const float tail = invBase * (float)(int)cs->perms[cs->prime_sums[i]] / (1 - invBase);
        memcpy(&rec[4], &invBase, 4);
        memcpy(&rec[5], &tail, 4);
        rec[6] = (uint32_t)((0x100000000ull + d - 1) / d);
        rec[7] = 0;
    }
}

float host_radical_inverse(const CompiledScene &cs, int baseIndex, uint64_t a) {
    if (baseIndex == 0) {
        uint32_t lo = (uint32_t)a, hi = (uint32_t)(a >> 32);
        auto rev = [](uint32_t n) {
            n = (n << 16) | (n >> 16);
            n = ((n & 0x00ff00ff) << 8) | ((n & 0xff00ff00) >> 8);
            n = ((n & 0x0f0f0f0f) << 4) | ((n & 0xf0f0f0f0) >> 4);
            n = ((n & 0x33333333) << 2) | ((n & 0xcccccccc) >> 2);
            n = ((n & 0x55555555) << 1) | ((n & 0xaaaaaaaa) >> 1);
            return n;
        };
        uint64_t r = ((uint64_t)rev(lo) << 32) | rev(hi);
        return (float)(r * 5.4210108624275222e-20);
    }
    int base = cs.primes[baseIndex];
    const float invBase = 1.f / (float)base;
    uint64_t reversedDigits = 0;
    float invBaseN = 1;
    while (a) {
        uint64_t next = a / base, digit = a - next * base;
        reversedDigits = reversedDigits * base + digit;
        invBaseN *= invBase;
        a = next;
    }
    return std::min(reversedDigits * invBaseN, 0x1.fffffep-1f);
}

DCamera make_camera(const gnxr_camera &c, int W, int H, int medium) {
    DCamera d;
    memset(&d, 0, sizeof(d));
    Xf lookat = look_at(Vec3(c.eye[0], c.eye[1], c.eye[2]), Vec3(c.look[0], c.look[1], c.look[2]), Vec3(c.up[0], c.up[1], c.up[2]));
    Mat4 c2w = lookat.inv;
    float frame = (float)W / (float)H;
    float sxmin, sxmax, symin, symax;
    if (frame > 1.f) { sxmin = -frame; sxmax = frame; symin = -1.f; symax = 1.f; }
    else { sxmin = -1.f; sxmax = 1.f; symin = -1.f / frame; symax = 1.f / frame; }
    if (c.orthographic) {
        const float ScreenScale = 2.0f;
        sxmin *= ScreenScale; sxmax *= ScreenScale; symin *= ScreenScale; symax *= ScreenScale;
    }
    Xf c2s = c.orthographic ? xmul(scale(1, 1, 1 / (10.f - 0.f)), translate(Vec3(0, 0, -0.f))) : perspective(c.fov_deg, 1e-2f, 1000.f);
    Xf s2r = xmul(xmul(scale((float)W, (float)H, 1), scale(1 / (sxmax - sxmin), 1 / (symin - symax), 1)), translate(Vec3(-sxmin, -symax, 0)));
    Xf r2c = xmul(xinverse(c2s), xinverse(s2r));
    memcpy(d.r2c, r2c.m.m, 64);
    memcpy(d.c2w, c2w.m, 64);
    d.lens_radius = c.lens_radius;
    d.focal_distance = c.focal_distance;
    d.medium = medium;
    d.ortho = c.orthographic ? 1 : 0;
    return d;
}

static int64_t mod64(int64_t a, int64_t b) { int64_t r = a - (a / b) * b; return r < 0 ? r + b : r; }
static void ext_gcd(uint64_t a, uint64_t b, int64_t *x, int64_t *y) {
    if (b == 0) { *x = 1; *y = 0; return; }
    int64_t d = a / b, xp, yp;
    ext_gcd(b, a % b, &xp, &yp);
    *x = yp; *y = xp - (d * yp);
}
DHalton make_halton(int W, int H) {
    DHalton h;
    memset(&h, 0, sizeof(h));
    int res[2] = {W, H};
    for (int i = 0; i < 2; ++i) {
        int base = (i == 0) ? 2 : 3, sc = 1, ex = 0;
        while (sc < std::min(res[i], 128)) { sc *= base; ++ex; }
        h.base_scale[i] = sc; h.base_exp[i] = ex;
    }
    h.stride = h.base_scale[0] * h.base_scale[1];
    int64_t x, y;
    ext_gcd(h.base_scale[1], h.base_scale[0], &x, &y); h.mult_inv[0] = (int)mod64(x, h.base_scale[0]);
    ext_gcd(h.base_scale[0], h.base_scale[1], &x, &y); h.mult_inv[1] = (int)mod64(x, h.base_scale[1]);
    return h;
}

static inline float lanczos(float x, float tau = 2) {
    x = std::abs(x);
    if (x < 1e-5f) return 1;
    if (x > 1.f) return 0;
    x *= kPi;
    float s = std::sin(x * tau) / (x * tau);
    float l = std::sin(x) / x;
    return s * l;
}
static inline int modi(int a, int b) { int r = a - (a / b) * b; return r < 0 ? r + b : r; }
static inline int round_up_pow2(int v) { v--; v |= v >> 1; v |= v >> 2; v |= v >> 4; v |= v >> 8; v |= v >> 16; return v + 1; }
struct RW { int first; float w[4]; };
static std::vector<RW> resample_weights(int oldRes, int newRes) {
    std::vector<RW> wt(newRes);
    float filterwidth = 2.f;
    for (int i = 0; i < newRes; ++i) {
        float center = (i + .5f) * oldRes / newRes;
        wt[i].first = (int)std::floor((center - filterwidth) + 0.5f);
        for (int j = 0; j < 4; ++j) { float pos = wt[i].first + j + .5f; wt[i].w[j] = lanczos((pos - center) / filterwidth); }
        float inv = 1 / (wt[i].w[0] + wt[i].w[1] + wt[i].w[2] + wt[i].w[3]);
// ... 178 lines not shown
        for (int u = 0; u < W2; ++u) {
            float up = (u + .5f) / (float)W2;
            float s = up * rx - 0.5f, t = vp * ry - 0.5f;
            int s0 = (int)std::floor(s), t0 = (int)std::floor(t);
            float ds = s - s0, dt = t - t0;
            float rgb[3];
            for (int c = 0; c < 3; ++c)
                rgb[c] = (1 - ds) * (1 - dt) * texel(s0, t0, c) + (1 - ds) * dt * texel(s0, t0 + 1, c) + ds * (1 - dt) * texel(s0 + 1, t0, c) +
                         ds * dt * texel(s0 + 1, t0 + 1, c);
            float y = 0.212671f * rgb[0] + 0.715160f * rgb[1] + 0.072169f * rgb[2];
            img[(size_t)u + (size_t)v * W2] = y;
            img[(size_t)u + (size_t)v * W2] *= sinTheta;
        }
    }
    cs->env_cond_func = img;
    cs->env_cond_cdf.resize((size_t)(W2 + 1) * H2);
    cs->env_cond_int.resize(H2);
    for (int v = 0; v < H2; ++v) dist1d(&img[(size_t)v * W2], W2, &cs->env_cond_cdf[(size_t)v * (W2 + 1)], &cs->env_cond_int[v]);
    cs->env_marg_func = cs->env_cond_int;
    cs->env_marg_cdf.resize(H2 + 1);
    dist1d(cs->env_marg_func.data(), H2, cs->env_marg_cdf.data(), &e.marg_func_int);
    auto upper = [](const float *cdf, int size, float u) { int n = 0, len = size; while (len > 0) { int half = len >> 1; if (cdf[n + half] <= u) { n += half + 1; len -= half + 1; } else len = half; } return n; };
    cs->env_marg_guide.resize(kEnvGuideMarg + 1);
    for (int b = 0; b <= kEnvGuideMarg; ++b) cs->env_marg_guide[b] = b == kEnvGuideMarg ? (uint16_t)(H2 + 1) : (uint16_t)upper(cs->env_marg_cdf.data(), H2 + 1, (float)b / kEnvGuideMarg);
    cs->env_cond_guide.resize((size_t)H2 * (kEnvGuideCond + 1));
    for (int v = 0; v < H2; ++v)
        for (int b = 0; b <= kEnvGuideCond; ++b)
            cs->env_cond_guide[(size_t)v * (kEnvGuideCond + 1) + b] = b == kEnvGuideCond ? (uint16_t)(W2 + 1) : (uint16_t)upper(&cs->env_cond_cdf[(size_t)v * (W2 + 1)], W2 + 1, (float)b / kEnvGuideCond);
    env_bounding_sphere(cs);
    cs->has_env = true;
}

static float inverse_gamma_correct(float value) {
    if (value <= 0.04045f) return value * 1.f / 12.92f;
    return std::pow((value + 0.055f) * 1.f / 1.055f, (float)2.4f);
}
static bool build_textures(const gnxr_scene_desc *d, CompiledScene *cs) {
    cs->textures.clear(); cs->tex_texels.clear(); cs->ewa_lut.clear();
    if (d->n_textures <= 0) return true;
    if (!d->textures || !d->texels) { set_error("textures without texel data"); return false; }
    cs->ewa_lut.resize(128);
    for (int i = 0; i < 128; ++i) {
        float alpha = 2;
        float r2 = float(i) / float(128 - 1);
        cs->ewa_lut[i] = std::exp(-alpha * r2) - std::exp(-alpha);
    }
    for (int ti = 0; ti < d->n_textures; ++ti) {
        const gnxr_texture &t = d->textures[ti];
        if (t.width <= 0 || t.height <= 0 || t.texel_offset < 0 || t.wrap < GNXR_WRAP_REPEAT || t.wrap > GNXR_WRAP_CLAMP) { set_error("texture %d: bad description", ti); return false; }
        const float *src = d->texels + t.texel_offset;
        int rx = t.width, ry = t.height;
        std::vector<float> tex((size_t)rx * ry * 3);
        for (int y = 0; y < ry; ++y)
            for (int x = 0; x < rx; ++x)
                for (int c = 0; c < 3; ++c) {
                    float v = src[((size_t)(ry - 1 - y) * rx + x) * 3 + c];
                    tex[((size_t)y * rx + x) * 3 + c] = t.scale * (t.gamma ? inverse_gamma_correct(v) : v);
                }
        auto wrap = [&](int v, int res) { return t.wrap == GNXR_WRAP_REPEAT ? modi(v, res) : (t.wrap == GNXR_WRAP_CLAMP ? std::min(std::max(v, 0), res - 1) : v); };
        if ((rx & (rx - 1)) || (ry & (ry - 1))) {
            int px = round_up_pow2(rx), py = round_up_pow2(ry);
            std::vector<RW> sw = resample_weights(rx, px);
            std::vector<float> res((size_t)px * py * 3, 0.f);
            for (int tt = 0; tt < ry; ++tt)
                for (int s_ = 0; s_ < px; ++s_)
                    for (int c = 0; c < 3; ++c) {
                        float acc = 0.f;
                        for (int j = 0; j < 4; ++j) {
                            int o = wrap(sw[s_].first + j, rx);
                            if (o >= 0 && o < rx) acc += sw[s_].w[j] * tex[((size_t)tt * rx + o) * 3 + c];
                        }
                        res[((size_t)tt * px + s_) * 3 + c] = acc;
                    }
            std::vector<RW> tw = resample_weights(ry, py);
            std::vector<float> work((size_t)py * 3);
            for (int s_ = 0; s_ < px; ++s_) {
                for (int tt = 0; tt < py; ++tt)
                    for (int c = 0; c < 3; ++c) {
                        float acc = 0.f;
                        for (int j = 0; j < 4; ++j) {
                            int o = wrap(tw[tt].first + j, ry);
                            if (o >= 0 && o < ry) acc += tw[tt].w[j] * res[((size_t)o * px + s_) * 3 + c];
                        }
                        work[(size_t)tt * 3 + c] = acc;
                    }
                for (int tt = 0; tt < py; ++tt)
                    for (int c = 0; c < 3; ++c) res[((size_t)tt * px + s_) * 3 + c] = clampf(work[(size_t)tt * 3 + c], 0.f, INFINITY);
            }
            tex.swap(res);
            rx = px; ry = py;
        }
        DTexture dt;
        memset(&dt, 0, sizeof(dt));
        dt.w0 = rx; dt.h0 = ry; dt.wrap = t.wrap; dt.trilinear = t.trilinear; dt.max_aniso = t.max_aniso;
        dt.su = t.su; dt.sv = t.sv; dt.du = t.du; dt.dv = t.dv;
        int nLevels = 1;
        for (int m = std::max(rx, ry); m > 1; m >>= 1) ++nLevels;
        if (nLevels > 16) { set_error("texture %d: more than 16 MIP levels", ti); return false; }
        dt.n_levels = nLevels;
        std::vector<float> prev = tex, cur;
        int pw = rx, ph = ry;
        auto push_level = [&](const std::vector<float> &lvl, int level, int w, int h) {
            dt.level_offset[level] = (int32_t)(cs->tex_texels.size() / 4);
            for (size_t i = 0; i < (size_t)w * h; ++i) { cs->tex_texels.push_back(lvl[3 * i]); cs->tex_texels.push_back(lvl[3 * i + 1]); cs->tex_texels.push_back(lvl[3 * i + 2]); cs->tex_texels.push_back(0.f); }
        };
        push_level(prev, 0, pw, ph);
        for (int i = 1; i < nLevels; ++i) {
            int sRes = std::max(1, pw / 2), tRes = std::max(1, ph / 2);
            cur.assign((size_t)sRes * tRes * 3, 0.f);
            auto tx = [&](int s_, int t_, int c) -> float {
                if (t.wrap == GNXR_WRAP_BLACK && (s_ < 0 || s_ >= pw || t_ < 0 || t_ >= ph)) return 0.f;
                return prev[((size_t)wrap(t_, ph) * pw + wrap(s_, pw)) * 3 + c];
            };
            for (int tt = 0; tt < tRes; ++tt)
                for (int s_ = 0; s_ < sRes; ++s_)
                    for (int c = 0; c < 3; ++c)
                        cur[((size_t)tt * sRes + s_) * 3 + c] = .25f * (tx(2 * s_, 2 * tt, c) + tx(2 * s_ + 1, 2 * tt, c) + tx(2 * s_, 2 * tt + 1, c) + tx(2 * s_ + 1, 2 * tt + 1, c));
            push_level(cur, i, sRes, tRes);
            prev.swap(cur); pw = sRes; ph = tRes;
        }
        cs->textures.push_back(dt);
    }
    return true;
}

static bool material_textures_ok(const gnxr_material &m, int index, int n_textures) {
    if (m.kd_texture > n_textures || m.ks_texture > n_textures || m.kd_texture < 0 || m.ks_texture < 0) { set_error("material %d: texture reference out of range", index); return false; }
    return true;
}
static bool sphere_material_ok(const gnxr_material *mats, int n_materials, int m, int sphere) {
    if (m >= 0 && m < n_materials && (mats[m].kd_texture || mats[m].ks_texture)) { set_error("sphere %d: image-textured materials are supported on triangles only", sphere); return false; }
    return true;
}

void MaterialTables::move_to(CompiledScene *cs) {
    cs->materials = std::move(materials); cs->materials_single = std::move(materials_single);
    cs->aov_albedo = std::move(aov_albedo); cs->material_authored = std::move(material_authored); cs->mat_map = std::move(mat_map);
}

bool compile_materials(const gnxr_material *mats, int n_materials, int n_textures, const std::vector<int32_t> &sphere_material, const int32_t *tri_material,
                       const uint8_t *tri_own_attr, int n_triangles, const int32_t *visit, MaterialTables *mt) {
    for (int i = 0; i < n_materials; ++i) if (!material_textures_ok(mats[i], i, n_textures)) return false;
    for (size_t i = 0; i < sphere_material.size(); ++i) if (!sphere_material_ok(mats, n_materials, sphere_material[i], (int)i)) return false;
    mt->materials.resize(std::max(1, n_materials));
    memset(mt->materials.data(), 0, sizeof(DMaterial) * mt->materials.size());
    for (int i = 0; i < n_materials; ++i) if (!compile_material(mats[i], &mt->materials[i])) return false;
    mt->materials_single = mt->materials;
    for (int i = 0; i < n_materials; ++i) if (!compile_material(mats[i], &mt->materials_single[i], false)) return false;
    mt->mat_map.assign(4 * (size_t)std::max(1, n_materials), 0);
    for (int i = 0; i < n_materials; ++i) {
        mt->mat_map[4 * (size_t)i] = mats[i].type == GNXR_MAT_NONE ? -1 : i;
        mt->mat_map[4 * (size_t)i + 1] = -1;
        mt->mat_map[4 * (size_t)i + 2] = mt->materials[i].shade_class;
    }
    for (int k = 0; k < n_triangles; ++k) {
        const int prim = visit ? visit[k] : k, m = tri_material[prim];
        if (m < 0 || !tri_own_attr[prim] || mt->mat_map[4 * (size_t)m] < 0 || mt->mat_map[4 * (size_t)m + 1] >= 0) continue;
        mt->mat_map[4 * (size_t)m + 1] = (int32_t)mt->materials.size();
        DMaterial c = mt->materials[m], cs_ = mt->materials_single[m];
        c.shade_class = cs_.shade_class = 3;
        c.has_attr = cs_.has_attr = 1;
        mt->materials.push_back(c);
        mt->materials_single.push_back(cs_);
    }
    mt->aov_albedo.assign((size_t)std::max(1, n_materials) * 4, 0.f);
    for (int i = 0; i < n_materials; ++i) {
        if (!material_albedo(mats[i], &mt->aov_albedo[(size_t)i * 4])) { set_error("unknown material type %d", mats[i].type); return false; }
        memcpy(&mt->aov_albedo[(size_t)i * 4 + 3], &mats[i].kd_texture, 4);
    }
    mt->material_authored.assign(mt->materials.size(), 0);
    for (int i = 0; i < n_materials; ++i) {
        mt->material_authored[i] = i;
        if (mt->mat_map[4 * (size_t)i + 1] >= 0) mt->material_authored[mt->mat_map[4 * (size_t)i + 1]] = i;
    }
    return true;
}

void triangle_material(const int32_t *mat_map, int32_t authored, uint8_t own_attr, int32_t *material, uint8_t *shade_class) {
    *material = authored; *shade_class = 0;
    if (authored < 0) return;
    const int32_t *e = mat_map + 4 * (size_t)authored;
    if (e[0] < 0) { *material = -1; return; }
    *material = own_attr ? e[1] : e[0];
    *shade_class = (uint8_t)(own_attr ? 3 : e[2]);
}

bool compile_scene(const gnxr_scene_desc *d, CompiledScene *cs, HlbvhBuildFn hlbvh_build) {
    if (!d || d->abi_version != GNXR_ABI_VERSION) { set_error("scene description ABI version mismatch"); return false; }
    if (d->n_triangles <= 0 || d->n_vertices <= 0 || !d->vertices || !d->indices || !d->tri_material || !d->tri_light) {
        set_error("scene description has no geometry");
        return false;
    }
    if (d->n_materials < 0 || d->n_lights < 0 || d->n_media < 0 || d->n_spheres < 0 || d->n_textures < 0 || (d->n_materials > 0 && !d->materials) ||
        (d->n_lights > 0 && !d->lights) || (d->n_media > 0 && !d->media) || (d->n_spheres > 0 && !d->spheres) || (d->n_textures > 0 && (!d->textures || !d->texels))) {
        set_error("scene description: a table has a count but no data");
        return false;
    }
    for (int i = 0; i < d->n_materials; ++i) if (!material_textures_ok(d->materials[i], i, d->n_textures)) return false;
    if (!build_textures(d, cs)) return false;
    for (int i = 0; i < d->n_spheres; ++i) if (!sphere_material_ok(d->materials, d->n_materials, d->spheres[i].material, i)) return false;
    for (int i = 0; i < 3 * d->n_triangles; ++i)
        if (d->indices[i] < 0 || d->indices[i] >= d->n_vertices) { set_error("triangle index out of range"); return false; }
    for (int i = 0; i < d->n_triangles; ++i) {
        if (d->tri_material[i] >= d->n_materials) { set_error("material index out of range"); return false; }
        if (d->tri_light[i] >= d->n_lights) { set_error("light index out of range"); return false; }
    }
    auto vert = [&](int i) { return Vec3(d->vertices[3 * i], d->vertices[3 * i + 1], d->vertices[3 * i + 2]); };
    BvhBuilder bb;
    bb.info.resize(d->n_triangles);
    for (int i = 0; i < d->n_triangles; ++i) {
        Box3 b;
        b.grow(vert(d->indices[3 * i])); b.grow(vert(d->indices[3 * i + 1])); b.grow(vert(d->indices[3 * i + 2]));
        bb.info[i].prim = i; bb.info[i].b = b;
        bb.info[i].c = .5f * b.lo + .5f * b.hi;
    }
    bb.nodes.reserve(2 * (size_t)d->n_triangles);
    bb.ordered.reserve(d->n_triangles);
    if (d->bvh_split_method < GNXR_BVH_SAH || d->bvh_split_method > GNXR_BVH_EQUAL_COUNTS) { set_error("unknown BVH split method %d", d->bvh_split_method); return false; }
    bb.method = d->bvh_split_method;
    int root = d->bvh_split_method == GNXR_BVH_HLBVH ? bb.build_hlbvh(hlbvh_build) : bb.build(0, d->n_triangles);
    if (root < 0) return false;
    cs->nodes.clear();
    cs->nodes.reserve(bb.nodes.size());
    cs->bvh_max_depth = 0;
    flatten(bb.nodes, root, cs->nodes, 0, &cs->bvh_max_depth);
    cs->nodes4.clear();
    cs->node4_src.clear();
    cs->stack4_need = 1;
    cs->root4 = collapse(cs->nodes, 0, cs->nodes4, cs->node4_src, 0, &cs->stack4_need);
    if (cs->nodes4.empty()) { cs->nodes4.push_back(DNode4()); cs->node4_src.assign(4, -1); }
    else if (cs->root4 >= 0) {
        const size_t n = cs->nodes4.size();
        std::vector<int32_t> order;
        order.reserve(n);
        std::vector<char> placed(n, 0);
        std::vector<int32_t> frontier{cs->root4};
        for (size_t head = 0; head < frontier.size() && order.size() < (size_t)kTopNodesMax; ++head) {
            const int32_t o = frontier[head];
            order.push_back(o); placed[o] = 1;
            for (int k = 0; k < 4; ++k) if (cs->nodes4[o].child[k] >= 0 && cs->nodes4[o].child[k] != kNode4Empty) frontier.push_back(cs->nodes4[o].child[k]);
        }
        for (size_t o = 0; o < n; ++o) if (!placed[o]) order.push_back((int32_t)o);
        std::vector<int32_t> new_of(n);
        for (size_t i = 0; i < n; ++i) new_of[order[i]] = (int32_t)i;
        std::vector<DNode4> re(n);
        std::vector<int32_t> re_src(4 * n);
        for (size_t i = 0; i < n; ++i) {
            re[i] = cs->nodes4[order[i]];
            for (int k = 0; k < 4; ++k) if (re[i].child[k] >= 0 && re[i].child[k] != kNode4Empty) re[i].child[k] = new_of[re[i].child[k]];
            for (int k = 0; k < 4; ++k) re_src[4 * i + k] = cs->node4_src[4 * (size_t)order[i] + k];
        }
        cs->nodes4.swap(re);
        cs->node4_src.swap(re_src);
        cs->root4 = new_of[cs->root4];
    }
    cs->leaf_boxes.assign((size_t)d->n_triangles * 8, 0.f);
    for (const DNode &n : cs->nodes)
        if ((n.meta & 0xffffu) != 0) {
            float *lb = &cs->leaf_boxes[(size_t)n.offset * 8];
            lb[0] = n.lo[0]; lb[1] = n.lo[1]; lb[2] = n.lo[2]; lb[3] = n.hi0; lb[4] = n.hi1; lb[5] = n.hi2;
        }
    cs->node_parent.assign(cs->nodes.size(), -1);
    for (size_t i = 0; i < cs->nodes.size(); ++i)
        if ((cs->nodes[i].meta & 0xffffu) == 0) { cs->node_parent[i + 1] = (int32_t)i; cs->node_parent[cs->nodes[i].offset] = (int32_t)i; }
    cs->world_bound.lo = Vec3(cs->nodes[0].lo[0], cs->nodes[0].lo[1], cs->nodes[0].lo[2]);
    cs->world_bound.hi = Vec3(cs->nodes[0].hi0, cs->nodes[0].hi1, cs->nodes[0].hi2);
    cs->spheres.assign(std::max(1, d->n_spheres), DSphere());
    cs->sphere_material.assign(d->n_spheres, -1);
    for (int i = 0; i < d->n_spheres; ++i) {
        const gnxr_sphere &sp = d->spheres[i];
        DSphere &ds = cs->spheres[i];
        if (!(sp.radius > 0) || sp.material >= d->n_materials || sp.medium_inside >= d->n_media || sp.medium_outside >= d->n_media) {
            set_error("sphere %d: bad radius / material / medium", i);
            return false;
        }
        memcpy(ds.c, sp.center, 12);
        ds.r = sp.radius;
        ds.material = (sp.material >= 0 && d->materials[sp.material].type == GNXR_MAT_NONE) ? -1 : sp.material;
        cs->sphere_material[i] = sp.material;
        ds.med_in = sp.medium_inside; ds.med_out = sp.medium_outside;
        ds.prim = d->n_triangles + i;
    }
    cs->n_spheres = d->n_spheres;
    grow_by_spheres(cs);
    cs->tris.resize(d->n_triangles);
    cs->leaf_of_prim.assign(d->n_triangles, -1);
    cs->n_vertices = d->n_vertices;
    cs->corner_vertex.resize(3 * (size_t)d->n_triangles);
    for (int li = 0; li < d->n_triangles; ++li) {
        int prim = bb.ordered[li];
        cs->leaf_of_prim[prim] = li;
        for (int c = 0; c < 3; ++c) cs->corner_vertex[3 * (size_t)li + c] = d->indices[3 * prim + c];
        DTri &t = cs->tris[li];
        Vec3 p0 = vert(d->indices[3 * prim]), p1 = vert(d->indices[3 * prim + 1]), p2 = vert(d->indices[3 * prim + 2]);
        t.p0[0] = p0.x; t.p0[1] = p0.y; t.p0[2] = p0.z; t.prim = prim;
        t.p1[0] = p1.x; t.p1[1] = p1.y; t.p1[2] = p1.z; t.material = d->tri_material[prim];
        if (t.material >= 0 && d->materials[t.material].type == GNXR_MAT_NONE) t.material = -1;
        t.p2[0] = p2.x; t.p2[1] = p2.y; t.p2[2] = p2.z; t.light = d->tri_light[prim];
    }
    cs->leaf1_from_verts = 1;
    for (const DNode &n : cs->nodes)
        if ((n.meta & 0xffffu) == 1 && (size_t)n.offset < cs->tris.size()) {
            const DTri &t = cs->tris[n.offset];
            const float hi[3] = {n.hi0, n.hi1, n.hi2};
            for (int a = 0; a < 3; ++a) {
                const float lo_v = std::min(std::min(t.p0[a], t.p1[a]), t.p2[a]), hi_v = std::max(std::max(t.p0[a], t.p1[a]), t.p2[a]);
                if (!(lo_v == n.lo[a]) || !(hi_v == hi[a])) cs->leaf1_from_verts = 0;
            }
        }
    cs->tri_uv.clear();
    cs->tri_n.clear();
    cs->tri_s.clear();
    cs->tri_own_attr.assign(d->n_triangles, 0);
    if (d->tri_uv || d->tri_n || d->tri_s) {
        if (d->tri_uv) cs->tri_uv.assign((size_t)d->n_triangles * 8, 0.f);
        if (d->tri_n) cs->tri_n.assign((size_t)d->n_triangles * 12, 0.f);
        if (d->tri_s) cs->tri_s.assign((size_t)d->n_triangles * 12, 0.f);
        const float def[6] = {0, 0, 1, 0, 1, 1}, zero9[9] = {0, 0, 0, 0, 0, 0, 0, 0, 0};
        for (int li = 0; li < d->n_triangles; ++li) {
            const int prim = cs->tris[li].prim;
            bool custom = false;
            if (d->tri_uv) {
                const float *uv = d->tri_uv + 6 * (size_t)prim;
                memcpy(&cs->tri_uv[(size_t)li * 8], uv, 24);
                custom = custom || memcmp(uv, def, 24) != 0;
            }
            if (d->tri_n) {
                const float *nn = d->tri_n + 9 * (size_t)prim;
                memcpy(&cs->tri_n[(size_t)li * 12], nn, 36);
                const bool hasN = memcmp(nn, zero9, 36) != 0;
                if (hasN && d->tri_light[prim] >= 0) { set_error("triangle %d: per-vertex normals on an emissive triangle are not supported", prim); return false; }
                custom = custom || hasN;
            }
            if (d->tri_s) {
                const float *sv = d->tri_s + 9 * (size_t)prim;
                memcpy(&cs->tri_s[(size_t)li * 12], sv, 36);
                const bool hasS = memcmp(sv, zero9, 36) != 0;
// ... 303 lines not shown
```

Before: 5043 Mrays/s.

## Sort glossy hits into per-material-kind queues with narrow conductor/dielectric shade kernels

```diff
diff --git a/__graft_entry__.py b/__graft_entry__.py
--- a/__graft_entry__.py
+++ b/__graft_entry__.py
@@ -6,7 +6,7 @@
 ROOT = os.path.dirname(os.path.abspath(__file__))
 CSRC = os.path.join(ROOT, "gnxraytracer_amd", "csrc")
 LIB = os.path.join(ROOT, "gnxraytracer_amd", "libgnxr.so")
-SOURCES = ["inst_whitted_tex.hip", "inst_whitted.hip", "inst_vol.hip", "inst_shade_query.hip", "inst_aov.hip", "api.hip", "scene_compile.cpp", "scene_builder.cpp"]
+SOURCES = ["inst_whitted_tex.hip", "inst_whitted.hip", "inst_vol.hip", "inst_shade_query.hip", "inst_shade_kinds.hip", "inst_aov.hip", "api.hip", "scene_compile.cpp", "scene_builder.cpp"]
 HIPCC_FLAGS = ["--offload-arch=gfx950", "-O3", "-std=c++17", "-fPIC", "-ffp-contract=off", "-fno-slp-vectorize", "-fno-unroll-loops", "-Wall",
                "-Wno-unused-variable", "-Wno-unused-function"]
 
diff --git a/gnxraytracer_amd/csrc/api.hip b/gnxraytracer_amd/csrc/api.hip
--- a/gnxraytracer_amd/csrc/api.hip
+++ b/gnxraytracer_amd/csrc/api.hip
@@ -29,6 +29,9 @@
 #undef X
 #define X(M, L, ST, T) extern template GX_VOL_SIGNATURE(M, L, ST, T)
 GX_VOL_INSTANCES(X)
+#undef X
+#define X(M, L) extern template GX_SHADE_KIND_SIGNATURE(M, L)
+GX_SHADE_KIND_INSTANCES(X)
 #undef X
 extern template GX_BSDF_QUERY_SIGNATURE(LM_ALL)
 extern template GX_LIGHT_SAMPLE_QUERY_SIGNATURE(LT_ALL)
diff --git a/gnxraytracer_amd/csrc/api_common.hip.h b/gnxraytracer_amd/csrc/api_common.hip.h
--- a/gnxraytracer_amd/csrc/api_common.hip.h
+++ b/gnxraytracer_amd/csrc/api_common.hip.h
@@ -68,6 +68,8 @@
 #undef GX_ONCE
     static int volmedia_step_cap() { return env_set("GNXR_VOLMEDIA_STEP_CAP") ? std::max(0, env_int("GNXR_VOLMEDIA_STEP_CAP", 0)) : 64; }
     static bool no_escape_queue() { return env_set("GNXR_NO_ESCAPE_QUEUE"); }
+    static bool no_material_queues() { return env_set("GNXR_NO_MATERIAL_QUEUES"); }
+    static bool no_narrow_shade() { return env_set("GNXR_NO_NARROW_SHADE"); }
     static bool host_light_grid() { return env_set("GNXR_HOST_LIGHT_GRID"); }
     static bool binary_bvh() { return env_set("GNXR_BINARY_BVH"); }
 };
diff --git a/gnxraytracer_amd/csrc/api_render.hip.h b/gnxraytracer_amd/csrc/api_render.hip.h
--- a/gnxraytracer_amd/csrc/api_render.hip.h
+++ b/gnxraytracer_amd/csrc/api_render.hip.h
@@ -50,6 +50,8 @@
     int class_mask;
     bool area_only, area_env_only;
     bool escape_queue;
+    int queue_kernel[4];
+    unsigned kind_queue;
     bool caller_rays;
     int n_views;
     int local_rows, npix;
@@ -62,6 +64,31 @@
     int nsamples() const { return p.spp_end - p.spp_begin; }
     int size_passes(size_t slots_held, bool have_mem, size_t free_b);
 };
+
+enum ShadeQueueKernel { SHADE_Q_NONE = 0, SHADE_Q_DIFFUSE, SHADE_Q_GLOSSY, SHADE_Q_CONDUCTOR, SHADE_Q_ROUGH_DIELECTRIC, SHADE_Q_ALL, SHADE_Q_TEX, SHADE_Q_ESCAPE };
+
+static void plan_shade_queues(const CompiledScene &cs, RenderPlan *pl) {
+    int *qk = pl->queue_kernel;
+    qk[0] = SHADE_Q_DIFFUSE;
+    qk[1] = (pl->class_mask & 2) ? SHADE_Q_GLOSSY : SHADE_Q_NONE;
+    qk[2] = (pl->class_mask & 4) ? SHADE_Q_ALL : SHADE_Q_NONE;
+    qk[3] = (pl->class_mask & 8) ? SHADE_Q_TEX : (pl->escape_queue ? SHADE_Q_ESCAPE : SHADE_Q_NONE);
+    pl->kind_queue = 0x01010101u;
+    int kinds = 0, n_kinds = 0;
+    for (const DMaterial &m : cs.materials) if (m.shade_class == 1) kinds |= 1 << material_kind(m);
+    for (int k = 0; k < MATERIAL_KINDS; ++k) n_kinds += (kinds >> k) & 1;
+    const int n_free = 1 + (qk[2] == SHADE_Q_NONE ? 1 : 0) + (qk[3] == SHADE_Q_NONE ? 1 : 0);
+    if (!pl->path_int() || cs.n_spheres > 0 || (kinds & ~1) == 0 || n_kinds > n_free || Knobs::no_material_queues()) return;
+    const bool narrow = !Knobs::no_narrow_shade();
+    pl->kind_queue = 0;
+    for (int k = 0, q = 1; k < MATERIAL_KINDS; ++k) {
+        if (!((kinds >> k) & 1)) { pl->kind_queue |= 1u << (8 * k); continue; }
+        while (q < 3 && qk[q] != SHADE_Q_NONE && !(q == 1 && qk[1] == SHADE_Q_GLOSSY)) ++q;
+        qk[q] = !narrow ? SHADE_Q_GLOSSY : (k == MATERIAL_KIND_CONDUCTOR ? SHADE_Q_CONDUCTOR : (k == MATERIAL_KIND_ROUGH_DIELECTRIC ? SHADE_Q_ROUGH_DIELECTRIC : SHADE_Q_GLOSSY));
+        pl->kind_queue |= (unsigned)q << (8 * k);
+        ++q;
+    }
+}
 
 static const long long kSubPassPaths = 64ll << 20;
 static const unsigned long long kSlotBytesEstimate = 238;
@@ -118,6 +145,7 @@
         if (l.type != GNXR_LIGHT_AREA_TRI && l.type != GNXR_LIGHT_INFINITE) pl.area_env_only = false;
     }
     pl.escape_queue = pl.path_int() && !pl.textured_scene && !cs.infinite_lights.empty() && !Knobs::no_escape_queue();
+    plan_shade_queues(cs, &pl);
     pl.caller_rays = src != nullptr;
     pl.n_views = views ? views->n_views : 0;
     pl.local_rows = count_local_rows(&p);
@@ -288,7 +316,7 @@
 
     void launch_trace(TraceWork w, int n_sh, int n_mis, bool count_rays = true);
     void compact(int mode, const int *qin, int nin, const unsigned char *keys, int nout, int nscatter, unsigned int *totals, int *o0, int *o1, int *o2, int *o3 = nullptr, int split = 0,
-                 const unsigned *n_dev = nullptr);
+                 const unsigned *n_dev = nullptr, unsigned kind_queue = 0x01010101u);
     int shade_stage(const int *q_in, int n, int *q_out, const unsigned *n_dev);
     void raygen(const PathArrays &at, long long u0, int kk, unsigned char *medium_keys);
     void resolve(const PathArrays &at, long long u0, int kk);
@@ -328,7 +356,7 @@
 }
 
 void RenderRun::compact(int mode, const int *qin, int nin, const unsigned char *keys, int nout, int nscatter, unsigned int *totals, int *o0, int *o1, int *o2, int *o3, int split,
-                        const unsigned *n_dev) {
+                        const unsigned *n_dev, unsigned kind_queue) {
     const int tiles = (nin + kCompactTile - 1) / kCompactTile;
     const int g = std::max(1, std::min(tiles, g_num_cus * kCompactBlocksPerCu));
     if (st.compact_seq >= (1u << 30) - 1u) {
@@ -340,7 +368,7 @@
     const bool hitclass = mode == COMPACT_HITCLASS;
     const int *hit = hitclass ? (const int *)st.hit.p : nullptr;
     const unsigned char *cls = hitclass ? (const unsigned char *)s->tri_class.p : nullptr;
-#define GX_COMPACT(M, N, NS) hipLaunchKernelGGL((k_compact<M, N, NS>), dim3(g), dim3(kCompactBlock), 0, stream, qin, nin, keys, cs, totals, o0, o1, o2, o3, hit, cls, split, n_dev, dctr)
+#define GX_COMPACT(M, N, NS) hipLaunchKernelGGL((k_compact<M, N, NS>), dim3(g), dim3(kCompactBlock), 0, stream, qin, nin, keys, cs, totals, o0, o1, o2, o3, hit, cls, kind_queue, split, n_dev, dctr)
     if (mode == COMPACT_FLAGS) {
         if (nout == 5) { if (nscatter == 3) GX_COMPACT(COMPACT_FLAGS, 5, 3); else GX_COMPACT(COMPACT_FLAGS, 5, 2); }
         else { if (nscatter == 3) GX_COMPACT(COMPACT_FLAGS, 4, 3); else GX_COMPACT(COMPACT_FLAGS, 4, 2); }
@@ -358,10 +386,9 @@
 
 int RenderRun::shade_stage(const int *q_in, int n, int *q_out, const unsigned *n_dev) {
     if (timing) timer.begin(2, stream);
-    const int class_mask = pl.class_mask;
-    const bool escape_queue = pl.escape_queue;
-    const int n_classes = ((class_mask & 8) || escape_queue) ? 4 : 3;
-    compact(COMPACT_HITCLASS, q_in, n, st.pclass.p, n_classes, n_classes, &dctr->q_class[0], st.queue_c0.p, st.queue_c1.p, st.queue_c2.p, st.queue_c3.p, 0, n_dev);
+    const int *qk = pl.queue_kernel;
+    const int n_classes = qk[3] != SHADE_Q_NONE ? 4 : 3;
+    compact(COMPACT_HITCLASS, q_in, n, st.pclass.p, n_classes, n_classes, &dctr->q_class[0], st.queue_c0.p, st.queue_c1.p, st.queue_c2.p, st.queue_c3.p, 0, n_dev, pl.kind_queue);
     int *qc[4] = {st.queue_c0.p, st.queue_c1.p, st.queue_c2.p, st.queue_c3.p};
     dim3 g(grid_for(n, Knobs::shade_blocks_per_cu())), b(kBlock);
     const int sdims = std::min<int>(Knobs::shade_lds_dims(), (int)s->cs.prime_sums.size() - 1);
@@ -371,7 +398,8 @@
     const int llights = (shade_lds_tabs && n_lights > 0 && n_lights <= 16) ? n_lights : 0;
     const size_t slds = (sdims > 0 ? ((((size_t)snperm * 2 + 15) & ~(size_t)15) + (size_t)sdims * 32) : 0) + (size_t)lmats * sizeof(DMaterial) + (size_t)llights * sizeof(DLight);
     const int shade_streams = Knobs::shade_streams();
-    const int n_class_kernels = 1 + ((class_mask & 2) ? 1 : 0) + ((class_mask & 4) ? 1 : 0) + (((class_mask & 8) || escape_queue) ? 1 : 0);
+    int n_class_kernels = 0;
+    for (int q = 0; q < 4; ++q) n_class_kernels += qk[q] != SHADE_Q_NONE ? 1 : 0;
     const bool fork = (shade_streams < 0 ? n_class_kernels >= 3 : (shade_streams != 0 && n_class_kernels >= 2)) && s->aux_stream[0] && s->aux_stream[1];
     hipStream_t cst[4] = {stream, stream, stream, stream};
     if (fork) {
@@ -384,38 +412,42 @@
 #define GX_SHADE_K(K, C) hipLaunchKernelGGL(K, g, b, slds, cst[C], sc, r, pa, (const int *)qc[C], (const unsigned int *)&dctr->q_class[C], sdims, snperm, lmats, llights)
 #define GX_SHADE(LMV, LTV, C) do { if (spheres) GX_SHADE_K((k_shade<LMV, LTV, true>), C); else GX_SHADE_K((k_shade<LMV, LTV, false>), C); } while (0)
 #define GX_SHADE_TEX(LTV) do { if (spheres) GX_SHADE_K((k_shade<LM_ALL, LTV, true, true>), 3); else GX_SHADE_K((k_shade<LM_ALL, LTV, false, true>), 3); } while (0)
-    if (area_only) {
-        GX_SHADE(LM_DIFFUSE, LT_AREA, 0);
-        if (class_mask & 2) GX_SHADE(LM_GLOSSY, LT_AREA, 1);
-        if (class_mask & 4) GX_SHADE(LM_ALL, LT_AREA, 2);
-        if (class_mask & 8) GX_SHADE_TEX(LT_AREA);
-    } else if (area_env_only && !spheres && !(class_mask & 8)) {
-#define GX_SHADE_AE(LMV, C) GX_SHADE_K((k_shade<LMV, LT_AREA | LT_ENV, false>), C)
-        GX_SHADE_AE(LM_DIFFUSE, 0);
-        if (class_mask & 2) GX_SHADE_AE(LM_GLOSSY, 1);
-        if (class_mask & 4) GX_SHADE_AE(LM_ALL, 2);
-#undef GX_SHADE_AE
-    } else {
-        GX_SHADE(LM_DIFFUSE, LT_ALL, 0);
-        if (class_mask & 2) GX_SHADE(LM_GLOSSY, LT_ALL, 1);
-        if (class_mask & 4) GX_SHADE(LM_ALL, LT_ALL, 2);
-        if (class_mask & 8) GX_SHADE_TEX(LT_ALL);
-    }
+    const int light_set = area_only ? 0 : ((area_env_only && !spheres && !(pl.class_mask & 8)) ? 1 : 2);
+#define GX_SHADE_LM(LMV, C) do { \
+        if (light_set == 0) GX_SHADE(LMV, LT_AREA, C); \
+        else if (light_set == 1) GX_SHADE_K((k_shade<LMV, LT_AREA | LT_ENV, false>), C); \
+        else GX_SHADE(LMV, LT_ALL, C); } while (0)
+#define GX_SHADE_NARROW(LMV, C) do { \
+        if (light_set == 0) GX_SHADE_K((k_shade<LMV, LT_AREA, false>), C); \
+        else if (light_set == 1) GX_SHADE_K((k_shade<LMV, LT_AREA | LT_ENV, false>), C); \
+        else GX_SHADE_K((k_shade<LMV, LT_ALL, false>), C); } while (0)
+    for (int q = 0; q < 4; ++q) {
+        switch (qk[q]) {
+        case SHADE_Q_DIFFUSE: GX_SHADE_LM(LM_DIFFUSE, q); break;
+        case SHADE_Q_GLOSSY: GX_SHADE_LM(LM_GLOSSY, q); break;
+        case SHADE_Q_CONDUCTOR: GX_SHADE_NARROW(LM_CONDUCTOR, q); break;
+        case SHADE_Q_ROUGH_DIELECTRIC: GX_SHADE_NARROW(LM_ROUGH_DIELECTRIC, q); break;
+        case SHADE_Q_ALL: GX_SHADE_LM(LM_ALL, q); break;
+        case SHADE_Q_TEX: if (light_set == 0) GX_SHADE_TEX(LT_AREA); else GX_SHADE_TEX(LT_ALL); break;
+        case SHADE_Q_ESCAPE:
+            if (area_env_only) hipLaunchKernelGGL((k_shade_escape<LT_AREA | LT_ENV>), g, b, 0, cst[q], sc, pa, (const int *)qc[q], (const unsigned int *)&dctr->q_class[q]);
+            else hipLaunchKernelGGL((k_shade_escape<LT_ALL>), g, b, 0, cst[q], sc, pa, (const int *)qc[q], (const unsigned int *)&dctr->q_class[q]);
+            break;
+        default: continue;
+        }
+        ++launches;
+    }
+#undef GX_SHADE_NARROW
+#undef GX_SHADE_LM
 #undef GX_SHADE_TEX
 #undef GX_SHADE
 #undef GX_SHADE_K
-    if (escape_queue) {
-        if (area_env_only) hipLaunchKernelGGL((k_shade_escape<LT_AREA | LT_ENV>), g, b, 0, cst[3], sc, pa, (const int *)qc[3], (const unsigned int *)&dctr->q_class[3]);
-        else hipLaunchKernelGGL((k_shade_escape<LT_ALL>), g, b, 0, cst[3], sc, pa, (const int *)qc[3], (const unsigned int *)&dctr->q_class[3]);
-        ++launches;
-    }
     if (fork) {
         HIP_TRY(hipEventRecord(s->ev_join[0], s->aux_stream[0]));
         HIP_TRY(hipEventRecord(s->ev_join[1], s->aux_stream[1]));
         HIP_TRY(hipStreamWaitEvent(stream, s->ev_join[0], 0));
         HIP_TRY(hipStreamWaitEvent(stream, s->ev_join[1], 0));
     }
-    launches += 1 + ((class_mask & 2) ? 1 : 0) + ((class_mask & 4) ? 1 : 0) + ((class_mask & 8) ? 1 : 0);
     compact(COMPACT_FLAGS, q_in, n, st.pflags.p, 4, 2, &dctr->q_next, q_out, st.queue_nee.p, nullptr, nullptr, 0, n_dev);
     if (timing) timer.end(stream);
     return GNXR_OK;
diff --git a/gnxraytracer_amd/csrc/compact_kernel.hip.h b/gnxraytracer_amd/csrc/compact_kernel.hip.h
--- a/gnxraytracer_amd/csrc/compact_kernel.hip.h
+++ b/gnxraytracer_amd/csrc/compact_kernel.hip.h
@@ -1,5 +1,6 @@
 #pragma once
 #include "device_math.h"
+#include "gnxr_device_types.h"
 
 namespace gnxr {
 
@@ -8,6 +9,10 @@
 
 template <int MODE>
 GX_DEV bool compact_pred(unsigned key, int o) { return MODE == COMPACT_FLAGS ? ((key >> o) & 1u) != 0 : key == (unsigned)o; }
+GX_DEV unsigned compact_class_queue(unsigned key, unsigned kind_queue) {
+    const unsigned cls = key & (unsigned)kClassKeyClassMask;
+    return cls == 1u ? (kind_queue >> ((key >> kClassKeyKindShift) * 8u)) & 0xffu : cls;
+}
 
 constexpr int kCompactChunks = 32;
 constexpr int kCompactTile = kCompactBlock * kCompactChunks;
@@ -34,7 +39,7 @@
 template <int MODE, int NOUT, int NSCATTER>
 __global__ void __launch_bounds__(kCompactBlock) k_compact(const int *__restrict__ q_in, int n, const unsigned char *__restrict__ keys, CompactScratch cs,
                                                            unsigned int *totals, int *out0, int *out1, int *out2, int *out3, const int *__restrict__ hit,
-                                                           const unsigned char *__restrict__ tri_class, int split, const unsigned *n_dev, Counters *ctr) {
+                                                           const unsigned char *__restrict__ tri_class, unsigned kind_queue, int split, const unsigned *n_dev, Counters *ctr) {
     __shared__ unsigned int wtot[NOUT][kCompactWaves];
     __shared__ unsigned int s_excl[NOUT];
     __shared__ unsigned int s_ticket;
@@ -76,7 +81,7 @@
 #pragma unroll
                 for (int j = 0; j < kCompactGather; ++j) h[j] = path[c0 + j] >= 0 ? hit[path[c0 + j]] : -1;
 #pragma unroll
-                for (int j = 0; j < kCompactGather; ++j) key[j] = path[c0 + j] < 0 ? 0xffu : (h[j] >= 0 ? (unsigned)tri_class[h[j]] : (unsigned)keys[path[c0 + j]]);
+                for (int j = 0; j < kCompactGather; ++j) key[j] = path[c0 + j] < 0 ? 0xffu : (h[j] >= 0 ? compact_class_queue((unsigned)tri_class[h[j]], kind_queue) : (unsigned)keys[path[c0 + j]]);
             } else {
 #pragma unroll
                 for (int j = 0; j < kCompactGather; ++j) key[j] = path[c0 + j] >= 0 ? (unsigned)keys[path[c0 + j]] : 0xffu;
diff --git a/gnxraytracer_amd/csrc/device_bsdf.h b/gnxraytracer_amd/csrc/device_bsdf.h
--- a/gnxraytracer_amd/csrc/device_bsdf.h
+++ b/gnxraytracer_amd/csrc/device_bsdf.h
@@ -79,6 +79,10 @@
 constexpr uint32_t LM_GLOSSY = LM_DIFFUSE | lobe_bit(LOBE_SPEC_REFL) | lobe_bit(LOBE_SPEC_TRANS) | lobe_bit(LOBE_FRESNEL_SPEC) | lobe_bit(LOBE_MICRO_REFL) |
                                lobe_bit(LOBE_MICRO_TRANS) | fresnel_bit(FRESNEL_NOOP) | fresnel_bit(FRESNEL_DIELECTRIC) | fresnel_bit(FRESNEL_CONDUCTOR);
 constexpr uint32_t LM_ALL = 0xffffffffu;
+constexpr uint32_t LM_CONDUCTOR = lobe_bit(LOBE_MICRO_REFL) | fresnel_bit(FRESNEL_CONDUCTOR);
+constexpr uint32_t LM_ROUGH_DIELECTRIC = lobe_bit(LOBE_MICRO_REFL) | lobe_bit(LOBE_MICRO_TRANS) | fresnel_bit(FRESNEL_DIELECTRIC);
+constexpr bool lm_micro_only(uint32_t lm) { return (lm & 0xffffu & ~(lobe_bit(LOBE_MICRO_REFL) | lobe_bit(LOBE_MICRO_TRANS))) == 0; }
+#define GX_MICRO_IS_REFL(l) (!GX_HAS_LOBE(LOBE_MICRO_TRANS) || (l).kind == LOBE_MICRO_REFL)
 
 template <uint32_t LM>
 GX_DEV Spec fresnel_eval(const DLobe &l, float cosI) {
@@ -175,7 +179,7 @@
     }
     break;
     case LOBE_MICRO_REFL: case LOBE_MICRO_TRANS: if (GX_HAS_LOBE(LOBE_MICRO_REFL) || GX_HAS_LOBE(LOBE_MICRO_TRANS)) {
-        const bool refl = l.kind == LOBE_MICRO_REFL;
+        const bool refl = GX_MICRO_IS_REFL(l);
         float cosThetaO, cosThetaI, eta = 1, cosArg;
         V3 wh;
         if (refl) {
@@ -259,7 +263,7 @@
     case LOBE_SPEC_REFL: case LOBE_SPEC_TRANS: case LOBE_FRESNEL_SPEC: return 0.f;
     case LOBE_LAMBERT_TRANS: if (GX_HAS_LOBE(LOBE_LAMBERT_TRANS)) return !same_hemisphere(wo, wi) ? abs_cos_theta(wi) * GX_INV_PI : 0.f; break;
     case LOBE_MICRO_REFL: case LOBE_MICRO_TRANS: if (GX_HAS_LOBE(LOBE_MICRO_REFL) || GX_HAS_LOBE(LOBE_MICRO_TRANS)) {
-        const bool refl = l.kind == LOBE_MICRO_REFL;
+        const bool refl = GX_MICRO_IS_REFL(l);
         V3 wh;
         float scale;
         if (refl) {
@@ -290,6 +294,7 @@
     break;
     default: break;
     }
+    if (lm_micro_only(LM)) return 0.f;
     return same_hemisphere(wo, wi) ? abs_cos_theta(wi) * GX_INV_PI : 0.f;
 }
 
@@ -335,7 +340,7 @@
         if (wo.z == 0) return Spec(0.f);
         V3 wh = tr_sample_wh(l.alphax, l.alphay, wo, u0, u1);
         if (dot(wo, wh) < 0) return Spec(0.f);
-        if (l.kind == LOBE_MICRO_REFL) {
+        if (GX_MICRO_IS_REFL(l)) {
             *wi = reflect(wo, wh);
             if (!same_hemisphere(wo, *wi)) return Spec(0.f);
             *pdf = tr_pdf(l.alphax, l.alphay, wo, wh) / (4 * dot(wo, wh));
@@ -373,6 +378,7 @@
     break;
     default: break;
     }
+    if (lm_micro_only(LM)) return Spec(0.f);
     *wi = cosine_sample_hemisphere(u0, u1);
     if (wo.z < 0) wi->z *= -1;
     *pdf = lobe_pdf<LM>(l, wo, *wi);
@@ -393,8 +399,8 @@
         for (int i = 0; i < mat->n_lobes; ++i) if (matches(mat->lobes[i].type, flags)) ++n;
         return n;
     }
-    static constexpr bool kSingle = (LM == LM_DIFFUSE);
-    static constexpr int kSingleType = BSDF_REFLECTION | BSDF_DIFFUSE;
+    static constexpr bool kSingle = (LM == LM_DIFFUSE || LM == LM_CONDUCTOR);
+    static constexpr int kSingleType = BSDF_REFLECTION | (LM == LM_CONDUCTOR ? BSDF_GLOSSY : BSDF_DIFFUSE);
     GX_DEV Spec f(V3 woW, V3 wiW, int flags) const {
         V3 wi = to_local(wiW), wo = to_local(woW);
         if (wo.z == 0) return Spec(0.f);
diff --git a/gnxraytracer_amd/csrc/gnxr_device_types.h b/gnxraytracer_amd/csrc/gnxr_device_types.h
--- a/gnxraytracer_amd/csrc/gnxr_device_types.h
+++ b/gnxraytracer_amd/csrc/gnxr_device_types.h
@@ -68,6 +68,9 @@
     int32_t has_attr;
     DLobe lobes[8];
 };
+enum : int32_t { MATERIAL_KIND_OTHER = 0, MATERIAL_KIND_CONDUCTOR = 1, MATERIAL_KIND_ROUGH_DIELECTRIC = 2, MATERIAL_KINDS = 4 };
+constexpr int kClassKeyKindShift = 2;
+constexpr int kClassKeyClassMask = 3;
 
 struct DTexture {
     int32_t n_levels, w0, h0, wrap;
diff --git a/gnxraytracer_amd/csrc/host_scene.h b/gnxraytracer_amd/csrc/host_scene.h
--- a/gnxraytracer_amd/csrc/host_scene.h
+++ b/gnxraytracer_amd/csrc/host_scene.h
@@ -105,7 +105,8 @@
 };
 bool compile_materials(const gnxr_material *mats, int n_materials, int n_textures, const std::vector<int32_t> &sphere_material, const int32_t *tri_material,
                        const uint8_t *tri_own_attr, int n_triangles, const int32_t *visit, MaterialTables *mt);
-void triangle_material(const int32_t *mat_map, int32_t authored, uint8_t own_attr, int32_t *material, uint8_t *shade_class);
+void triangle_material(const int32_t *mat_map, int32_t authored, uint8_t own_attr, int32_t *material, uint8_t *class_key);
+int material_kind(const DMaterial &m);
 void refit_world_bound(CompiledScene *cs, const float root6[6]);
 bool compile_light(const gnxr_light &l, int index, const Vec3 corners[3], int tri_leaf, const Box3 &world_bound, DLight *out);
 DCamera make_camera(const gnxr_camera &c, int W, int H, int medium);
diff --git a/gnxraytracer_amd/csrc/inst_shade_kinds.hip b/gnxraytracer_amd/csrc/inst_shade_kinds.hip
--- /dev/null
+++ b/gnxraytracer_amd/csrc/inst_shade_kinds.hip
@@ -0,0 +1,5 @@
+#include "kernel_instances.h"
+using namespace gnxr;
+#define X(M, L) template GX_SHADE_KIND_SIGNATURE(M, L)
+GX_SHADE_KIND_INSTANCES(X)
+#undef X
diff --git a/gnxraytracer_amd/csrc/kernel_instances.h b/gnxraytracer_amd/csrc/kernel_instances.h
--- a/gnxraytracer_amd/csrc/kernel_instances.h
+++ b/gnxraytracer_amd/csrc/kernel_instances.h
@@ -15,6 +15,11 @@
 #define GX_VS_LT(X, M, T) GX_VS_ST(X, M, LT_AREA, T) GX_VS_ST(X, M, LT_ALL, T)
 #define GX_VOL_INSTANCES(X) GX_VS_LT(X, LM_DIFFUSE, false) GX_VS_LT(X, LM_GLOSSY, false) GX_VS_LT(X, LM_ALL, false) GX_VS_LT(X, LM_ALL, true)
 
+#define GX_SK_LT(X, M) X(M, LT_AREA) X(M, LT_AREA | LT_ENV) X(M, LT_ALL)
+#define GX_SHADE_KIND_INSTANCES(X) GX_SK_LT(X, LM_CONDUCTOR) GX_SK_LT(X, LM_ROUGH_DIELECTRIC)
+
+#define GX_SHADE_KIND_SIGNATURE(M, L) \
+    __global__ void gnxr::k_shade<M, L, false, false>(gnxr::DScene, gnxr::DRender, gnxr::PathArrays, const int *, const unsigned int *, int, int, int, int);
 #define GX_WHITTED_SIGNATURE(M, L, S, T) \
     __global__ void gnxr::k_whitted_step<M, L, S, T>(gnxr::DScene, gnxr::DRender, gnxr::PathArrays, gnxr::WhittedArrays, const int *, int, unsigned long long *);
 #define GX_VOL_SIGNATURE(M, L, ST, T) \
diff --git a/gnxraytracer_amd/csrc/kernels.hip.h b/gnxraytracer_amd/csrc/kernels.hip.h
--- a/gnxraytracer_amd/csrc/kernels.hip.h
+++ b/gnxraytracer_amd/csrc/kernels.hip.h
@@ -370,7 +370,9 @@
 #ifndef GX_SHADE_W_TEX
 #define GX_SHADE_W_TEX 3
 #endif
-template <uint32_t LM> constexpr int shade_min_waves() { return LM == LM_DIFFUSE ? GX_SHADE_W_DIFFUSE : (LM == LM_GLOSSY ? GX_SHADE_W_GLOSSY : GX_SHADE_W_ALL); }
+template <uint32_t LM> constexpr int shade_min_waves() {
+    return LM == LM_DIFFUSE ? GX_SHADE_W_DIFFUSE : ((LM == LM_GLOSSY || LM == LM_CONDUCTOR || LM == LM_ROUGH_DIELECTRIC) ? GX_SHADE_W_GLOSSY : GX_SHADE_W_ALL);
+}
 template <uint32_t LM, int LT, bool SPH, bool TEX = false>
 __global__ void __launch_bounds__(kBlock, (TEX ? GX_SHADE_W_TEX : shade_min_waves<LM>())) k_shade(DScene sc, DRender r, PathArrays pa, const int *__restrict__ queue, const unsigned int *n_dev, int lds_dims, int lds_nperm, int lds_mats, int lds_lights) {
     extern __shared__ int shade_smem[];
diff --git a/gnxraytracer_amd/csrc/material_kernel.hip.h b/gnxraytracer_amd/csrc/material_kernel.hip.h
--- a/gnxraytracer_amd/csrc/material_kernel.hip.h
+++ b/gnxraytracer_amd/csrc/material_kernel.hip.h
@@ -19,7 +19,7 @@
             const int4 e = mat_map[authored];
             const bool own = own_attr[prim] != 0;
             material = e.x < 0 ? -1 : (own ? e.y : e.x);
-            cls = e.x < 0 ? 0 : (own ? 3 : e.z);
+            cls = e.x < 0 ? 0 : (own ? 3 : (e.z | (e.w << kClassKeyKindShift)));
         }
         tris[li].material = material;
         tri_class[li] = (unsigned char)cls;
@@ -34,7 +34,7 @@
         if ((unsigned)prim >= (unsigned)n_tris) continue;
         const int m = tris[li].material;
         material_out[prim] = m >= 0 ? authored[m] : -1;
-        class_out[prim] = tri_class[li];
+        class_out[prim] = tri_class[li] & kClassKeyClassMask;
     }
 }
 
diff --git a/gnxraytracer_amd/csrc/scene_compile.cpp b/gnxraytracer_amd/csrc/scene_compile.cpp
--- a/gnxraytracer_amd/csrc/scene_compile.cpp
+++ b/gnxraytracer_amd/csrc/scene_compile.cpp
@@ -407,6 +407,18 @@
     if (out->shade_class == 0 && out->n_lobes > 1) out->shade_class = 1;
     if (textured) out->shade_class = 3;
     return true;
+}
+
+int material_kind(const DMaterial &m) {
+    if (m.shade_class != 1 || m.n_lobes < 1) return MATERIAL_KIND_OTHER;
+    bool conductor = m.n_lobes == 1, dielectric = true;
+    for (int i = 0; i < m.n_lobes; ++i) {
+        const DLobe &l = m.lobes[i];
+        if (l.disney_g) return MATERIAL_KIND_OTHER;
+        if (!(l.kind == LOBE_MICRO_REFL && l.fresnel == FRESNEL_CONDUCTOR)) conductor = false;
+        if (!((l.kind == LOBE_MICRO_REFL || l.kind == LOBE_MICRO_TRANS) && l.fresnel == FRESNEL_DIELECTRIC)) dielectric = false;
+    }
+    return conductor ? MATERIAL_KIND_CONDUCTOR : (dielectric ? MATERIAL_KIND_ROUGH_DIELECTRIC : MATERIAL_KIND_OTHER);
 }
 
 namespace {
@@ -891,6 +903,7 @@
         mt->mat_map[4 * (size_t)i] = mats[i].type == GNXR_MAT_NONE ? -1 : i;
         mt->mat_map[4 * (size_t)i + 1] = -1;
         mt->mat_map[4 * (size_t)i + 2] = mt->materials[i].shade_class;
+        mt->mat_map[4 * (size_t)i + 3] = material_kind(mt->materials[i]);
     }
     for (int k = 0; k < n_triangles; ++k) {
         const int prim = visit ? visit[k] : k, m = tri_material[prim];
@@ -915,13 +928,13 @@
     return true;
 }
 
-void triangle_material(const int32_t *mat_map, int32_t authored, uint8_t own_attr, int32_t *material, uint8_t *shade_class) {
-    *material = authored; *shade_class = 0;
+void triangle_material(const int32_t *mat_map, int32_t authored, uint8_t own_attr, int32_t *material, uint8_t *class_key) {
+    *material = authored; *class_key = 0;
     if (authored < 0) return;
     const int32_t *e = mat_map + 4 * (size_t)authored;
     if (e[0] < 0) { *material = -1; return; }
     *material = own_attr ? e[1] : e[0];
-    *shade_class = (uint8_t)(own_attr ? 3 : e[2]);
+    *class_key = (uint8_t)(own_attr ? 3 : (e[2] | (e[3] << kClassKeyKindShift)));
 }
 
 bool compile_scene(const gnxr_scene_desc *d, CompiledScene *cs, HlbvhBuildFn hlbvh_build) {
```

After: 5102 Mrays/s, median of 6. 1.2% higher.
